# nextpyp/cet_pick

Hardware: AMD Instinct MI355X
Metric: subtomograms/sec (MoCo-3D train) + voxels/sec (heatmap+NMS) at 1/2/4/8 GPU (higher is better)
Workload: dtype f32; 1 GPU; moco_main.py moco3d_18: 3D encoder, synthetic 512x512x128 tomogram, 32^3 subtomo crops, batch 64 per GPU, r=1024, dim=128, m=0.999, T=0.1, SGD lr 1e-3; global_batch=64, parallelism=dp1, hipgraph=True

## Files before the change

### cet_pick_amd/_lib.py

```python
import ctypes
import os

import torch

_HERE = os.path.dirname(os.path.abspath(__file__))
LIB_PATH = os.environ.get("CETPICK_HIP_LIB") or os.path.join(_HERE, "libcetpick_hip.so")

_c = ctypes
_P, _I, _F, _Z, _D, _L = _c.c_void_p, _c.c_int, _c.c_float, _c.c_size_t, _c.c_double, _c.c_long


class ConvGeom(ctypes.Structure):
    _fields_ = [(f, _I) for f in "N Di Hi Wi Ci Co kd kh kw stride pd ph pw dd dh dw".split()]


_G = _c.POINTER(ConvGeom)


class Aug2d3dRanges(ctypes.Structure):
    _fields_ = [(f, _F) for f in "flip_p angle_lo angle_hi erase_p scale_lo scale_hi ratio_lo ratio_hi".split()]


_R = _c.POINTER(Aug2d3dRanges)

SIGNATURES = {
    "mi_abi_version": (_I, []),
    "mi_graph_node_counts": (_I, [_P, _P]),
    "mi_debug_stamp": (_I, [_P, _P]),
    "mi_linear_stats_fwd_f32": (_I, [_P] * 5 + [_I] * 3 + [_P]),
    "mi_debug_last_conv_kernel": (_c.c_char_p, []),
    "mi_linear_bn_fwd_f32": (_I, [_P] * 5 + [_I] * 3 + [_P, _P, _F, _F] + [_P] * 4 + [_I, _P]),
    "mi_conv3d_stem_stats_workspace_bytes": (_Z, [_I] * 5),
    "mi_conv3d_stem_stats_f32": (_I, [_P, _P, _P] + [_I] * 5 + [_P, _P, _Z, _P]),
    "mi_build_arch": (_c.c_char_p, []),
    "mi_sigmoid_clamp": (_I, [_P, _P, _Z, _P]),
    "mi_nms3d": (_I, [_P, _P, _I, _I, _I, _I, _I, _P]),
    "mi_decode_workspace_bytes": (_Z, [_I, _I, _I, _I]),
    "mi_decode_workspace_init": (_I, [_P, _Z, _P]),
    "mi_sigmoid_nms_topk": (_I, [_P, _P, _I, _I, _I, _I, _I, _I, _I, _P, _P, _P, _Z, _P]),
    "mi_gauss3d_sep": (_I, [_P, _P, _P, _I, _I, _I, _F, _P]),
    "mi_dog_pick_workspace_bytes": (_Z, [_I, _I, _I, _I]),
    "mi_dog_pick": (_I, [_P, _I, _I, _I, _P, _I, _I, _I, _I, _P, _P, _P, _P, _I, _P, _P, _Z, _P]),
    "mi_greedy_nms3d_workspace_bytes": (_Z, [_I, _I, _I]),
    "mi_greedy_nms3d": (_I, [_P, _I, _I, _I, _F, _F, _F, _P, _P, _P, _I, _P, _Z, _P]),
    "mi_crop_normalize": (_I, [_P, _I, _I, _I, _P, _I, _I, _I, _I, _I, _I, _P, _P]),
    "mi_crop_normalize_table": (_I, [_P, _P, _P, _P, _P, _c.c_int64, _I, _I, _I, _I, _I, _I, _P, _P]),
    "mi_u8_roundtrip_normalize": (_I, [_P, _P, _Z, _F, _F, _P]),
    "mi_aug2d_params": (_I, [_P, _c.c_int64, _c.c_uint64, _I, _I, _I] + [_F] * 7 + [_P, _P]),
    "mi_aug2d_apply": (_I, [_P, _c.c_int64, _I, _P, _P, _c.c_int64, _I, _F, _F, _P, _P]),
    "mi_aug2d3d_params": (_I, [_P, _c.c_int64, _c.c_uint64, _I, _I, _R, _R, _P, _P]),
    "mi_aug2d3d_apply": (_I, [_P, _P, _c.c_int64, _I, _P, _P, _P, _P, _c.c_int64, _I, _F, _F, _F, _F, _P, _P]),
    "mi_tilt_patches": (_I, [_P, _I, _P, _P, _c.c_int64, _I, _I, _D, _D, _P, _P, _P]),
    "mi_semi_labels": (_I, [_P, _I, _I, _I, _P, _c.c_int64, _P, _I, _I, _P]),
    "mi_semi_pairs": (_I, [_P, _P, _I, _P, _P, _c.c_int64, _I, _I, _P, _P, _P, _P]),
    "mi_gauss2d_slices": (_I, [_P, _P, _P, _I, _I, _I, _F, _P]),
    "mi_rec_reorder": (_I, [_P, _I, _I, _I, _I, _I, _I, _P, _P]),
    "mi_vol_stats_workspace_bytes": (_Z, [_L, _L]),
    "mi_vol_stats": (_I, [_P, _L, _L, _P, _P, _Z, _P]),
    "mi_zscore": (_I, [_P, _P, _L, _L, _P, _P]),
    "mi_zscore_quantize_minmax": (_I, [_P, _P, _L, _L, _P, _D, _D, _I, _P]),
    "mi_conv_workspace_bytes": (_Z, [_G]),
    "mi_conv_fwd_f32": (_I, [_P, _P, _P, _P, _I, _I, _G, _P, _Z, _P]),
    "mi_conv_dgrad_f32": (_I, [_P, _P, _P, _P, _P, _G, _P, _Z, _P]),
    "mi_conv_wgrad_f32": (_I, [_P, _P, _P, _G, _P, _Z, _P, _P]),
    "mi_conv_wgrad_batch_f32": (_I, [_P, _P, _P, _P, _I, _G, _Z, _P, _P]),
    "mi_stem2d_fwd_bias_f32": (_I, [_P, _P, _P, _P, _I, _I, _I, _I, _P]),
    "mi_upconv_tail_fwd": (_I, [_P, _P, _P, _P, _P] + [_I] * 7 + [_P]),
    "mi_smallk_image_bytes": (_Z, [_I, _I]),
    "mi_smallk_prep": (_I, [_P, _P, _I, _I, _P]),
    "mi_smallk_fwd_f32": (_I, [_P, _P, _P, _P, _I, _L, _I, _I, _I, _L, _I, _P]),
    "mi_smallk_heads_fwd_f32": (_I, [_P, _P, _P, _P, _P, _I, _L, _I, _L, _I, _P]),
    "mi_splitk_reduce_batch": (_I, [_P, _P, _P, _P, _I, _P]),
    "mi_linear_fwd_f32": (_I, [_P, _P, _P, _P, _I, _I, _I, _P, _Z, _P]),
    "mi_conv3d_direct_wimg_bytes": (_Z, [_I]),
    "mi_conv3d_direct_workspace_bytes": (_Z, [_I, _I]),
    "mi_conv3d_direct_usable": (_I, [_I] * 9),
    "mi_conv3d_direct_prep": (_I, [_P, _P, _P, _P, _I, _P]),
    "mi_conv3d_direct_f32": (_I, [_P, _P, _P, _P, _P, _I, _I, _I, _I, _I, _I, _P, _Z, _P]),
    "mi_conv2d_p2d_usable": (_I, [_I] * 4),
    "mi_conv2d_p2d_wimg_bytes": (_Z, [_I]),
    "mi_conv2d_p2d_prep": (_I, [_P, _P, _P, _P, _I, _P]),
    "mi_conv2d_p2d_f32": (_I, [_P, _P, _P, _P, _P, _I, _I, _I, _I, _I, _P]),
    "mi_conv2d_p2d_wgrad_workspace_bytes": (_Z, [_I] * 4),
    "mi_conv2d_p2d_wgrad_f32": (_I, [_P, _P, _P, _I, _I, _I, _I, _P, _Z, _P]),
    "mi_conv2d_stem3_workspace_bytes": (_Z, [_I]),
    "mi_conv2d_stem3_fwd_f32": (_I, [_P, _P, _P, _I, _I, _I, _I, _P]),
    "mi_conv2d_stem3_wgrad_f32": (_I, [_P, _P, _P, _I, _I, _I, _I, _P, _Z, _P]),
    "mi_conv3d_cube2_workspace_bytes": (_Z, [_I, _I]),
    "mi_conv3d_cube2_usable": (_I, [_I] * 9),
    "mi_conv3d_cube2_f32": (_I, [_P, _P, _P, _P, _P, _I, _I, _I, _I, _P, _Z, _P]),
    "mi_conv_d32_kind": (_I, [_I] * 12),
    "mi_conv_d32_image_bytes": (_Z, [_I, _I]),
    "mi_conv_d64_image_bytes": (_Z, [_I, _I]),
    "mi_conv_d32_prep": (_I, [_P, _P, _I, _I, _P]),
    "mi_conv_d64_prep_co": (_I, [_P, _P, _I, _I, _I, _P]),
    "mi_conv_d32_1x1_fwd_f32": (_I, [_P, _P, _P, _P, _I, _I, _I, _I, _I, _I, _I, _P]),
    "mi_conv_d32_fwd_pool_f32": (_I, [_P, _P, _P, _P, _P] + [_I] * 7 + [_P]),
    "mi_conv_d32_fwd_pool_strided_f32": (_I, [_P, _P, _P, _P, _I, _P] + [_I] * 7 + [_P]),
    "mi_copy_channels_into": (_I, [_P, _I, _P, _I, _I, _L, _P]),
    "mi_conv_d32_upconv_fwd_f32": (_I, [_P, _P, _P, _P, _P] + [_I] * 8 + [_P]),
    "mi_conv_d64_fwd_f32": (_I, [_P, _P, _P, _P, _I, _I, _I, _I, _I, _I, _I, _P]),
    "mi_conv_d32_fwd_f32": (_I, [_P, _P, _P, _P, _I, _I, _I, _I, _I, _I, _I, _P]),
    "mi_maxpool2d_ceil_fwd": (_I, [_P, _P, _P, _I, _I, _I, _I, _I, _P]),
    "mi_maxpool2d_ceil_bwd": (_I, [_P, _P, _P, _I, _I, _I, _I, _I, _P]),
    "mi_shuffle2x2_fwd": (_I, [_P, _P, _P, _I, _I, _I, _I, _I, _I, _P]),
    "mi_shuffle2x2_bwd": (_I, [_P, _P, _I, _I, _I, _I, _I, _I, _P]),
    "mi_concat_channels": (_I, [_P, _I, _P, _I, _P, _L, _P]),
    "mi_split_channels": (_I, [_P, _P, _I, _P, _I, _L, _P]),
    "mi_zhead_fwd": (_I, [_P, _P, _P, _I, _I, _L, _I, _I, _P]),
    "mi_zhead_bwd_workspace_bytes": (_Z, [_I, _I, _L, _I, _I]),
    "mi_zhead_bwd": (_I, [_P, _P, _P, _P, _P, _I, _I, _L, _I, _I, _P, _Z, _P]),
    "mi_voxel_loss_workspace_bytes": (_Z, [_L]),
    "mi_pu_focal_loss_fwd": (_I, [_P, _P, _L, _D, _D, _P, _P, _P, _Z, _P]),
    "mi_pu_focal_loss_bwd": (_I, [_P, _P, _L, _D, _P, _P, _P, _P]),
    "mi_focal_loss_fwd": (_I, [_P, _P, _L, _P, _P, _P, _Z, _P]),
    "mi_focal_loss_bwd": (_I, [_P, _P, _L, _P, _P, _P, _P]),
    "mi_mse_loss_fwd": (_I, [_P, _P, _L, _P, _P, _P, _Z, _P]),
    "mi_mse_loss_bwd": (_I, [_P, _P, _L, _P, _P, _P, _P, _P]),
    "mi_ucl_rowsums_fwd": (_I, [_P, _P, _I, _I, _F, _P, _P, _P, _P, _P, _P]),
    "mi_ucl_rowsums_bwd_ranged": (_I, [_P, _P, _I, _I, _F, _P, _P, _P, _P, _P, _P, _P, _P]),
    "mi_colreduce_workspace_bytes": (_Z, [_L, _I]),
    "mi_bn_stats": (_I, [_P, _L, _I, _P, _P, _Z, _P]),
    "mi_bn_apply_fwd": (_I, [_P, _P, _L, _I, _P, _D, _P, _P, _F, _F, _P, _P, _P, _P, _P, _I, _P]),
    "mi_bn_relu_maxpool3d_fwd": (_I, [_P, _P, _P, _I, _I, _I, _I, _I, _I, _I, _I, _P, _D, _P, _P, _F, _F, _P, _P, _P, _P, _P]),
    "mi_bn_relu_bwd_reduce_x": (_I, [_P, _P, _L, _I, _P, _P, _P, _P, _P, _Z, _P]),
    "mi_bn_relu_bwd_apply_x": (_I, [_P, _P, _P, _L, _I, _P, _P, _P, _P, _D, _P, _P, _P]),
    "mi_bn_small_fwd": (_I, [_P, _P, _L, _I, _P, _P, _F, _F, _P, _P, _P, _P, _P, _I, _P]),
    "mi_bn_small_bwd": (_I, [_P, _P, _P, _P, _L, _I, _P, _P, _I, _P, _P, _P]),
    "mi_bn_small_pool_fwd": (_I, [_P, _P, _P, _L, _I, _I, _P, _P, _F, _F, _P, _P, _P, _P, _P]),
    "mi_bn_small_pool_bwd": (_I, [_P, _P, _P, _P, _L, _I, _I, _P, _P, _P, _P, _P]),
    "mi_bn_eval_fwd": (_I, [_P, _P, _L, _I, _P, _P, _P, _P, _F, _P, _P, _I, _P]),
    "mi_bn_bwd_reduce": (_I, [_P, _P, _P, _L, _I, _P, _I, _P, _P, _Z, _P]),
    "mi_bn_bwd_apply": (_I, [_P, _P, _P, _P, _L, _I, _P, _P, _P, _D, _I, _P, _P, _P]),
    "mi_bn_bwd_apply_res": (_I, [_P, _P, _P, _P, _P, _L, _I, _P, _P, _P, _D, _P, _P, _P]),
    "mi_bn_param_grads": (_I, [_P, _I, _P, _P, _P]),
    "mi_colsum": (_I, [_P, _L, _I, _P, _P, _P, _Z, _P]),
    "mi_maxpool3d_fwd": (_I, [_P, _P, _P] + [_I] * 8 + [_P]),
    "mi_maxpool3d_bwd": (_I, [_P, _P, _P] + [_I] * 8 + [_P]),
    "mi_avgpool_fwd": (_I, [_P, _P, _I, _I, _I, _P]),
    "mi_avgpool_bwd": (_I, [_P, _P, _I, _I, _I, _P]),
    "mi_bias_add": (_I, [_P, _P, _L, _I, _P]),
    "mi_copy_pair_f32": (_I, [_P, _P, _P, _P, _L, _P]),
    "mi_relu_mask": (_I, [_P, _P, _P, _P, _L, _P]),
    "mi_l2norm_fwd": (_I, [_P, _P, _P, _I, _I, _P]),
    "mi_l2norm_bwd": (_I, [_P, _P, _P, _P, _I, _I, _P]),
    "mi_moco_logits_fwd": (_I, [_P, _P, _P, _P, _I, _I, _I, _F, _P]),
    "mi_moco_logits_norm_fwd": (_I, [_P, _P, _P, _P, _P, _P, _P, _I, _I, _I, _F, _P]),
    "mi_moco_logits_bwd": (_I, [_P, _P, _P, _P, _I, _I, _I, _F, _P]),
# ... 123 lines not shown
```

### cet_pick_amd/csrc/common.h

```cpp
#pragma once
#include <hip/hip_runtime.h>
#include <stdint.h>
#include <math.h>
#include "../../include/cetpick_hip.h"

#define MI_RETURN_IF_LAUNCH_FAILED()                  \
    do {                                              \
        hipError_t e_ = hipGetLastError();            \
        if (e_ != hipSuccess) return (int)e_;         \
    } while (0)
#define MI_HIP(call)                                  \
    do {                                              \
        hipError_t e_ = (call);                       \
        if (e_ != hipSuccess) return (int)e_;         \
    } while (0)

static inline size_t mi_align_up(size_t x, size_t a) { return (x + a - 1) / a * a; }

struct MiSmallGemmBN {
    float* y;
    const float* gamma;
    const float* beta;
    float eps, momentum;
    float* running_mean;
    float* running_var;
    long long* num_batches_tracked;
    float* save;
    int relu;
    double* sums_only;
};
static inline int mi_cdiv(long a, long b) { return (int)((a + b - 1) / b); }

struct Cube2Final {
    unsigned* tickets;
    float* out;
    const float* res;
    const float* mask;
    int relu;
};
constexpr size_t MI_CUBE2_TICKET_BYTES = 16384;

__device__ __forceinline__ float wave_sum(float v) {
#pragma unroll
    for (int o = 32; o > 0; o >>= 1) v += __shfl_xor(v, o, 64);
    return v;
}
__device__ __forceinline__ double wave_sum(double v) {
#pragma unroll
    for (int o = 32; o > 0; o >>= 1) v += __shfl_xor(v, o, 64);
    return v;
}
__device__ __forceinline__ float wave_max(float v) {
#pragma unroll
    for (int o = 32; o > 0; o >>= 1) v = fmaxf(v, __shfl_xor(v, o, 64));
    return v;
}

__device__ __forceinline__ unsigned long long make_key(float score, unsigned tie) {
    return ((unsigned long long)__float_as_uint(score) << 32) | (unsigned long long)tie;
}

__device__ __forceinline__ void block_bitonic_sort_desc(unsigned long long* keys, int n_pow2,
                                                        int tid, int nthreads) {
    for (int k = 2; k <= n_pow2; k <<= 1) {
        for (int j = k >> 1; j > 0; j >>= 1) {
            __syncthreads();
            for (int t = tid; t < (n_pow2 >> 1); t += nthreads) {
                int i = ((t / j) * (j << 1)) + (t % j);
                int l = i + j;
                bool desc = ((i & k) == 0);
                unsigned long long a = keys[i], b = keys[l];
                bool swap = desc ? (a < b) : (a > b);
                if (swap) { keys[i] = b; keys[l] = a; }
            }
        }
    }
    __syncthreads();
}

template <bool GUARD>
__device__ __forceinline__ void bitonic_pairs4(unsigned long long* keys, int t0, int stride, int n_pairs, int base, int j,
                                               int lj, int k) {
    unsigned long long a[4], b[4];
    int ii[4];
#pragma unroll
    for (int u = 0; u < 4; ++u) {
        const int t = t0 + u * stride;
        ii[u] = base + ((t >> lj) << (lj + 1)) + (t & (j - 1));
        if (!GUARD || t < n_pairs) { a[u] = keys[ii[u]]; b[u] = keys[ii[u] + j]; }
    }
#pragma unroll
    for (int u = 0; u < 4; ++u) {
        const int t = t0 + u * stride;
        if (!GUARD || t < n_pairs) {
            const bool desc = ((ii[u] & k) == 0);
            const bool sw = desc ? (a[u] < b[u]) : (a[u] > b[u]);
            keys[ii[u]] = sw ? b[u] : a[u];
            keys[ii[u] + j] = sw ? a[u] : b[u];
        }
    }
}

__device__ __forceinline__ void block_sort_desc_fast(unsigned long long* keys, int n_pow2, int tid, int nthreads) {
    const int n_waves = nthreads >> 6;
    const int B = n_pow2 / n_waves;
    const int lane = tid & 63, wv = tid >> 6;
    const int half = n_pow2 >> 1;
    __syncthreads();
    for (int k = 2; k <= n_pow2; k <<= 1) {
        int j = k >> 1;
        for (; 2 * j > B; j >>= 1) {
            const int lj = 31 - __builtin_clz(j);
            if ((half & (4 * nthreads - 1)) == 0)
                for (int t0 = tid; t0 < half; t0 += 4 * nthreads) bitonic_pairs4<false>(keys, t0, nthreads, half, 0, j, lj, k);
            else
                for (int t0 = tid; t0 < half; t0 += 4 * nthreads) bitonic_pairs4<true>(keys, t0, nthreads, half, 0, j, lj, k);
            __syncthreads();
        }
        for (; j > 0; j >>= 1) {
            const int lj = 31 - __builtin_clz(j);
            if (((B >> 1) & 255) == 0)
// ... 10 lines not shown
```

### cet_pick_amd/csrc/conv_cube2.hip

```cpp
#include "common.h"
#include "bf16x3.h"
#include <type_traits>

namespace {

using namespace bf3;

constexpr int KQ = 4;

struct Cube2Params {
    const float* a;
    const float* w;
    float* slabs;
    int N, C;
    unsigned a_bytes, w_bytes;
    unsigned* tickets;
    float* out;
    const float* res;
    const float* mask;
    int relu;
};

__device__ __forceinline__ int pair_tap(int in_v, int out_v) {
    const int tz = ((in_v >> 2) & 1) - ((out_v >> 2) & 1) + 1, ty = ((in_v >> 1) & 1) - ((out_v >> 1) & 1) + 1,
// ... 65 lines not shown
#pragma unroll
    for (int s = 0; s < NS; ++s) {
        if (s + PD - 1 < NS) fetch_dyn(s + PD - 1);
        bf16x8 af[2][3], bf[3];
        float v[8];
#pragma unroll
        for (int rb = 0; rb < 2; ++rb) {
#pragma unroll
            for (int e = 0; e < 4; ++e) { v[e] = __uint_as_float(araw[s % PD][rb][0][e]); v[4 + e] = __uint_as_float(araw[s % PD][rb][1][e]); }
            cut8(v, af[rb]);
        }
#pragma unroll
        for (int e = 0; e < 8; ++e) v[e] = __uint_as_float(braw[s % PD][e]);
        cut8(v, bf);
#pragma unroll
        for (int pr = 0; pr < 6; ++pr) {
            acc[0] = __builtin_amdgcn_mfma_f32_32x32x16_bf16(af[0][PA[pr]], bf[PB[pr]], acc[0], 0, 0, 0);
            acc[1] = __builtin_amdgcn_mfma_f32_32x32x16_bf16(af[1][PA[pr]], bf[PB[pr]], acc[1], 0, 0, 0);
        }
    }

#pragma unroll
    for (int rb = 0; rb < 2; ++rb)
#pragma unroll
        for (int r = 0; r < 16; ++r) red[wave][rb * 16 + r][lane] = acc[rb][r];
    __syncthreads();
    const long slab = (long)p.N * 8 * C;
    float* out = p.slabs + (long)q * slab;
    float tv[8];
    long o[8];
#pragma unroll
    for (int j = 0; j < 8; ++j) {
        const int idx = wave * 8 + j, rb = idx >> 4, r = idx & 15;
        tv[j] = ((red[0][idx][lane] + red[1][idx][lane]) + red[2][idx][lane]) + red[3][idx][lane];
        const int n = n0 + rb * 32 + (r & 3) + 8 * (r >> 2) + 4 * h;
        o[j] = n < p.N ? ((long)n * 8 + cv) * C + cc0 + l32 : -1;
        if (!FINAL) { if (o[j] >= 0) out[o[j]] = tv[j]; }
        else if (o[j] >= 0) __hip_atomic_store(out + o[j], tv[j], __ATOMIC_RELAXED, __HIP_MEMORY_SCOPE_AGENT);
    }
    if (!FINAL) return;
    asm volatile("s_waitcnt vmcnt(0)" ::: "memory");
    __syncthreads();
    unsigned* ticket = p.tickets + (mt * gridDim.x + cbi);
    if (tid == 0) s_last = (__hip_atomic_fetch_add(ticket, 1u, __ATOMIC_RELAXED, __HIP_MEMORY_SCOPE_AGENT) == KQ - 1) ? 1u : 0u;
    __syncthreads();
    if (!s_last) return;
    if (tid == 0) __hip_atomic_store(ticket, 0u, __ATOMIC_RELAXED, __HIP_MEMORY_SCOPE_AGENT);
    float part[KQ][8];
#pragma unroll
    for (int z = 0; z < KQ; ++z)
#pragma unroll
        for (int j = 0; j < 8; ++j)
            part[z][j] = (z == q || o[j] < 0) ? tv[j] : __hip_atomic_load(p.slabs + (long)z * slab + o[j], __ATOMIC_RELAXED, __HIP_MEMORY_SCOPE_AGENT);
#pragma unroll
    for (int j = 0; j < 8; ++j) {
        if (o[j] < 0) continue;
        float t = ((part[0][j] + part[1][j]) + part[2][j]) + part[3][j];
        if (p.res) t += p.res[o[j]];
        if (p.relu) t = fmaxf(t, 0.f);
        if (p.mask) t = (p.mask[o[j]] > 0.f) ? t : 0.f;
        p.out[o[j]] = t;
    }
}

constexpr int PW_ROW = 64;
constexpr int PW_HALF = 64 * PW_ROW;
constexpr int PW_PLANE = 2 * PW_HALF;
constexpr int PW_OP = 3 * PW_PLANE;
constexpr int PW_MAXTAP = 27;

constexpr int PW_MAXPROB = 4;
struct PairWgradParams {
    const float* x[PW_MAXPROB];
    const float* dy[PW_MAXPROB];
    float* dw[PW_MAXPROB];
    int N, VI, VO, CI, CO, ntaps;
    unsigned x_bytes, dy_bytes;
    int Di, Do, stride, pad, ks;
    int S;
    long slab_stride;
    unsigned char order[PW_MAXTAP];
    unsigned short cnt[PW_MAXTAP];
    unsigned char lo[PW_MAXTAP][3], len[PW_MAXTAP][3];
};

__global__ __launch_bounds__(512, 2) void pair_wgrad_kernel(PairWgradParams p) {
    __shared__ __attribute__((aligned(16))) unsigned char lds[2 * PW_OP];
    const int tid = threadIdx.x, lane = tid & 63, wave = tid >> 6;
    const int h = lane >> 5, l32 = lane & 31, i16 = lane & 15, g16 = (lane >> 4) & 1;
    const int wm = (wave >> 1) & 1, wn = wave & 1, kh = wave >> 2;
    const int ncb = p.CO >> 6, nib = p.CI >> 6;
    const int tiles = nib * ncb;
    const int rem = blockIdx.x % tiles, ts = blockIdx.x / tiles;
    const int tap = p.order[ts / p.S];
    const int seg = ts % p.S;
    const int ib = rem / ncb, cb = rem % ncb;
    const int npairs = p.cnt[tap], nchunks = (p.N + 63) >> 6;
    const int all = npairs * nchunks, per = (all + p.S - 1) / p.S;
    const int it0 = seg * per, total = min(all, it0 + per);
    const int tz = tap / (p.ks * p.ks), ty = (tap / p.ks) % p.ks, tx = tap % p.ks;
    const int lz = p.lo[tap][0], ly = p.lo[tap][1], lx = p.lo[tap][2], ny = p.len[tap][1], nx = p.len[tap][2];

    const __amdgpu_buffer_rsrc_t xrs = rsrc(p.x[blockIdx.y], p.x_bytes), yrs = rsrc(p.dy[blockIdx.y], p.dy_bytes);
    const int srow = tid >> 3, cg = tid & 7;
    const int st_lds = (cg >> 2) * PW_HALF + srow * PW_ROW + (cg & 3) * 16;
    u32x4 ldx[3][2], ldy[3][2];
    int f_it = it0, f_chunk = it0 % nchunks, f_px, f_py, f_pz;
    { const int pr = it0 / nchunks; f_px = pr % nx; f_py = (pr / nx) % ny; f_pz = pr / (nx * ny); }
    auto fetch = [&](auto Sc, int) {
        constexpr int S = decltype(Sc)::value;
        const int n = f_chunk * 64 + srow;
        const bool ok = f_it < total && n < p.N;
        const int oz = lz + f_pz, oy = ly + f_py, ox = lx + f_px;
        const int vo = (oz * p.Do + oy) * p.Do + ox;
        const int vi = ((p.stride * oz + tz - p.pad) * p.Di + p.stride * oy + ty - p.pad) * p.Di + p.stride * ox + tx - p.pad;
        ++f_it;
        if (++f_chunk == nchunks) { f_chunk = 0; if (++f_px == nx) { f_px = 0; if (++f_py == ny) { f_py = 0; ++f_pz; } } }
        const unsigned xo = ok ? 4u * (unsigned)(((long)n * p.VI + vi) * p.CI + ib * 64 + cg * 8) : 0x80000000u;
        const unsigned yo = ok ? 4u * (unsigned)(((long)n * p.VO + vo) * p.CO + cb * 64 + cg * 8) : 0x80000000u;
#pragma unroll
        for (int q = 0; q < 2; ++q) {
            ldx[S][q] = __builtin_amdgcn_raw_buffer_load_b128(xrs, (int)(xo + 16u * q), 0, 0);
            ldy[S][q] = __builtin_amdgcn_raw_buffer_load_b128(yrs, (int)(yo + 16u * q), 0, 0);
        }
    };
    auto store = [&](auto Sc, int boff) {
        constexpr int S = decltype(Sc)::value;
#pragma unroll
        for (int op = 0; op < 2; ++op) {
            float v[8];
#pragma unroll
            for (int e = 0; e < 4; ++e) {
                v[e] = __uint_as_float(op ? ldy[S][0][e] : ldx[S][0][e]);
                v[4 + e] = __uint_as_float(op ? ldy[S][1][e] : ldx[S][1][e]);
            }
            bf16x8 o[3];
            cut8(v, o);
#pragma unroll
            for (int pl = 0; pl < 3; ++pl)
                *reinterpret_cast<u32x4*>(lds + boff + op * PW_OP + pl * PW_PLANE + st_lds) = __builtin_bit_cast(u32x4, o[pl]);
        }
    };
    const int q4 = i16 >> 2;
    const int coloff = (16 * g16 + 4 * (i16 & 3)) * 2;
    const int a_base = wm * PW_HALF + (8 * h + q4 + 32 * kh) * PW_ROW + coloff;
    const int b_base = PW_OP + wn * PW_HALF + (8 * h + q4 + 32 * kh) * PW_ROW + coloff;

    f32x16 acc;
#pragma unroll
    for (int r = 0; r < 16; ++r) acc[r] = 0.f;

    auto multiply = [&](int boff) {
#pragma unroll
        for (int ks = 0; ks < 2; ++ks) {
            bf16x8 af[3], bf[3];
#pragma unroll
            for (int pl = 0; pl < 3; ++pl) {
                const unsigned char* ap = lds + boff + a_base + pl * PW_PLANE + ks * 16 * PW_ROW;
                const unsigned char* bp = lds + boff + b_base + pl * PW_PLANE + ks * 16 * PW_ROW;
                const bf16x4 alo = __builtin_amdgcn_ds_read_tr16_b64_v4bf16((lds_bf16x4*)(ap));
                const bf16x4 ahi = __builtin_amdgcn_ds_read_tr16_b64_v4bf16((lds_bf16x4*)(ap + 4 * PW_ROW));
                const bf16x4 blo = __builtin_amdgcn_ds_read_tr16_b64_v4bf16((lds_bf16x4*)(bp));
                const bf16x4 bhi = __builtin_amdgcn_ds_read_tr16_b64_v4bf16((lds_bf16x4*)(bp + 4 * PW_ROW));
                af[pl] = __builtin_shufflevector(alo, ahi, 0, 1, 2, 3, 4, 5, 6, 7);
                bf[pl] = __builtin_shufflevector(blo, bhi, 0, 1, 2, 3, 4, 5, 6, 7);
            }
#pragma unroll
            for (int pr = 0; pr < 6; ++pr) acc = __builtin_amdgcn_mfma_f32_32x32x16_bf16(af[PA[pr]], bf[PB[pr]], acc, 0, 0, 0);
        }
    };
    auto body = [&](auto Sc, auto, int it) {
        store(Sc, 0);
        __syncthreads();
        fetch(Sc, it + 3);
        multiply(0);
        __syncthreads();
    };
    using I0 = std::integral_constant<int, 0>; using I1 = std::integral_constant<int, 1>; using I2 = std::integral_constant<int, 2>;
    fetch(I0{}, it0);
    fetch(I1{}, it0 + 1);
    fetch(I2{}, it0 + 2);
    int it = it0;
    for (; it + 3 <= total; it += 3) {
        body(I0{}, I1{}, it);
        body(I1{}, I2{}, it + 1);
        body(I2{}, I0{}, it + 2);
    }
    if (it < total) {
        body(I0{}, I1{}, it);
        if (it + 1 < total) body(I1{}, I2{}, it + 1);
    }
    float (*red)[16][64] = reinterpret_cast<float (*)[16][64]>(lds);
    if (kh == 1) {
#pragma unroll
        for (int r = 0; r < 16; ++r) red[wave & 3][r][lane] = acc[r];
    }
    __syncthreads();
    if (kh == 0) {
        float* out = p.dw[blockIdx.y] + seg * p.slab_stride + ((long)tap * p.CI + ib * 64 + 32 * wm) * p.CO + cb * 64 + 32 * wn + l32;
#pragma unroll
        for (int r = 0; r < 16; ++r) out[(long)((r & 3) + 8 * (r >> 2) + 4 * h) * p.CO] = acc[r] + red[wave][r][lane];
    }
}

struct SmallGemmParams {
    const float* a;
    const float* b;
    const float* bias;
    float* c;
    int M, N, K;
    long lda_m, lda_k, ldb_k, ldb_n;
    unsigned a_bytes, b_bytes;
    float* bn_y;
    const float* gamma;
    const float* beta;
    float eps, momentum;
    float* running_mean;
    float* running_var;
    long long* num_batches_tracked;
    float* save;
    int relu;
    double* sums_only;
};

template <bool A_KC, bool B_KC, int NS>
__global__ __launch_bounds__(256, 2) void small_gemm_kernel(SmallGemmParams p) {
    __shared__ float red[4][32][64];
    const int tid = threadIdx.x, lane = tid & 63, wave = tid >> 6;
    const int h = lane >> 5, l32 = lane & 31;
    const int n0 = blockIdx.x * 32, m0 = blockIdx.y * 64;
    const int KT = (p.K + 15) >> 4;
    const __amdgpu_buffer_rsrc_t ars = rsrc(p.a, p.a_bytes), brs = rsrc(p.b, p.b_bytes);
    constexpr int PD = NS < 4 ? NS : 4;
    unsigned araw[PD][2][8], braw[PD][8];
    const bool col_ok = n0 + l32 < p.N;
    auto fetch = [&](auto Uc) {
        constexpr int U = decltype(Uc)::value, SET = U % PD;
        if constexpr (U < NS) {
            const int ks = wave + 4 * U;
            const int k0 = ks * 16 + 8 * h;
            const bool live = ks < KT;
#pragma unroll
            for (int rb = 0; rb < 2; ++rb) {
                const int m = m0 + rb * 32 + l32;
                const bool ok = live && m < p.M;
                if (A_KC) {
                    const unsigned off = (ok && k0 + 8 <= p.K) ? 4u * (unsigned)(m * p.lda_m + k0) : 0x80000000u;
                    const u32x4 lo = __builtin_amdgcn_raw_buffer_load_b128(ars, (int)off, 0, 0);
                    const u32x4 hi = __builtin_amdgcn_raw_buffer_load_b128(ars, (int)(off + 16u), 0, 0);
#pragma unroll
                    for (int e = 0; e < 4; ++e) { araw[SET][rb][e] = lo[e]; araw[SET][rb][4 + e] = hi[e]; }
                } else {
#pragma unroll
                    for (int e = 0; e < 8; ++e) {
                        const unsigned off = (ok && k0 + e < p.K) ? 4u * (unsigned)(m * p.lda_m + (long)(k0 + e) * p.lda_k) : 0x80000000u;
                        araw[SET][rb][e] = __builtin_amdgcn_raw_buffer_load_b32(ars, (int)off, 0, 0);
                    }
                }
            }
            const bool okb = live && col_ok;
            if (B_KC) {
                const unsigned off = (okb && k0 + 8 <= p.K) ? 4u * (unsigned)((long)(n0 + l32) * p.ldb_n + k0) : 0x80000000u;
                const u32x4 lo = __builtin_amdgcn_raw_buffer_load_b128(brs, (int)off, 0, 0);
                const u32x4 hi = __builtin_amdgcn_raw_buffer_load_b128(brs, (int)(off + 16u), 0, 0);
#pragma unroll
                for (int e = 0; e < 4; ++e) { braw[SET][e] = lo[e]; braw[SET][4 + e] = hi[e]; }
            } else {
#pragma unroll
                for (int e = 0; e < 8; ++e) {
                    const unsigned off = (okb && k0 + e < p.K) ? 4u * (unsigned)((long)(k0 + e) * p.ldb_k + (long)(n0 + l32) * p.ldb_n) : 0x80000000u;
                    braw[SET][e] = __builtin_amdgcn_raw_buffer_load_b32(brs, (int)off, 0, 0);
                }
            }
        }
    };
    f32x16 acc[2];
#pragma unroll
    for (int r = 0; r < 16; ++r) { acc[0][r] = 0.f; acc[1][r] = 0.f; }
    auto step = [&](auto Uc) {
        constexpr int U = decltype(Uc)::value, SET = U % PD;
        if constexpr (U < NS) {
            fetch(std::integral_constant<int, U + PD - 1>{});
            if (wave + 4 * U < KT) {
                bf16x8 af[2][3], bf[3];
                float v[8];
// ... 69 lines not shown
            }
        }
        if (blockIdx.x == 0 && tid == 0 && p.num_batches_tracked) *p.num_batches_tracked += 1;
        const float g = (p.gamma && col_ok) ? p.gamma[col] : 1.f, b = (p.beta && col_ok) ? p.beta[col] : 0.f;
#pragma unroll
        for (int j = 0; j < 8; ++j) {
            const int idx = wave * 8 + j, rb = idx >> 4, r = idx & 15;
            const int m = m0 + rb * 32 + (r & 3) + 8 * (r >> 2) + 4 * h;
            float q = fmaf((tv[j] - mf) * iv, g, b);
            if (p.relu) q = fmaxf(q, 0.f);
            if (m < p.M && col_ok) p.bn_y[(long)m * p.N + col] = q;
        }
    }
}

}

bool mi_cube2_usable(int N, int Di, int Hi, int Wi, int Ci, int Co, int kd, int kh, int kw, int stride, int pd, int ph, int pw,
                     int dd, int dh, int dw) {
    const char* off = getenv("MI_CONV_NO_DIRECT");
    if (off && atoi(off) != 0) return false;
    if (kd != 3 || kh != 3 || kw != 3 || stride != 1 || pd != 1 || ph != 1 || pw != 1 || dd != 1 || dh != 1 || dw != 1) return false;
    if (Di != 2 || Hi != 2 || Wi != 2 || Ci != Co) return false;
    if (Ci != 128 && Ci != 256 && Ci != 512) return false;
    return N >= 1 && 4l * N * 8 * Ci < 0x7fff0000l;
}

namespace {
struct PairGeom { int ntaps, maxcnt; long pairs; };
PairGeom pair_geom(int Di, int k, int stride, PairWgradParams* p) {
    const int pad = k == 3 ? 1 : 0, Do = (Di + 2 * pad - k) / stride + 1;
    PairGeom r = {k * k * k, 0, 0};
    for (int t = 0; t < r.ntaps; ++t) {
        const int tt[3] = {t / (k * k), (t / k) % k, t % k};
        int c = 1;
        for (int a = 0; a < 3; ++a) {
            int lo = Do, hi = -1;
            for (int o = 0; o < Do; ++o) {
                const int i = stride * o + tt[a] - pad;
                if (i >= 0 && i < Di) { lo = std::min(lo, o); hi = std::max(hi, o); }
            }
            const int len = hi >= lo ? hi - lo + 1 : 0;
            if (p) { p->lo[t][a] = (unsigned char)(len ? lo : 0); p->len[t][a] = (unsigned char)std::max(len, 1); }
            c *= len;
        }
        if (p) p->cnt[t] = (unsigned short)c;
        r.maxcnt = std::max(r.maxcnt, c);
        r.pairs += c;
    }
    return r;
}
}

bool mi_pair_wgrad_usable(int N, int Di, int Hi, int Wi, int Ci, int Co, int kd, int kh, int kw, int stride, int pd, int ph, int pw,
                          int dd, int dh, int dw) {
    const char* off = getenv("MI_CONV_NO_DIRECT");
    if (off && atoi(off) != 0) return false;
    if (kd != kh || kd != kw || pd != ph || pd != pw || dd != 1 || dh != 1 || dw != 1) return false;
    if (!((kd == 3 && pd == 1) || (kd == 1 && pd == 0)) || (stride != 1 && stride != 2)) return false;
    if (Hi != Di || Wi != Di || Di < 2) return false;
    const int Do = (Di + 2 * pd - kd) / stride + 1;
    const char* wide = getenv("MI_PAIR_WGRAD_MAXOUT");
    if (Do < 1 || Do > (wide ? atoi(wide) : 2) || Do > 8) return false;
    if (Ci < 64 || Co < 64 || (Ci & 63) || (Co & 63)) return false;
    return N >= 1 && 4l * N * Di * Hi * Wi * Ci < 0x7fff0000l && 4l * N * Do * Do * Do * Co < 0x7fff0000l;
}

int mi_pair_wgrad_splits(int N, int Di, int Ci, int Co, int k, int stride) {
    const PairGeom g = pair_geom(Di, k, stride, nullptr);
    if (g.maxcnt <= 8) return 1;
    const char* e = getenv("MI_PAIR_WGRAD_SPLITS");
    if (e && atoi(e) > 0) return std::min(atoi(e), 64);
    const int iters = g.maxcnt * ((N + 63) / 64), tiles = (Ci / 64) * (Co / 64);
    int S = (iters + 7) / 8;
    if (g.ntaps * tiles * S < 256) S = (iters + 3) / 4;
    return std::max(1, std::min(S, 16));
}
size_t mi_pair_wgrad_slab_bytes(int N, int Di, int Ci, int Co, int k, int stride) {
    const int S = mi_pair_wgrad_splits(N, Di, Ci, Co, k, stride);
    return S > 1 ? sizeof(float) * (size_t)S * k * k * k * Ci * Co : 0;
}

int mi_pair_wgrad_batch_max() { return PW_MAXPROB; }
int mi_pair_wgrad_launch_batch(const float* const* xs, const float* const* dys, float* const* dws, float* const* slabs, int nb, int N,
                               int Di, int Ci, int Co, int k, int stride, hipStream_t s) {
    if (nb < 1 || nb > PW_MAXPROB) return MI_E_ARG;
    PairWgradParams p = {};
    const PairGeom g = pair_geom(Di, k, stride, &p);
    const int pad = k == 3 ? 1 : 0, Do = (Di + 2 * pad - k) / stride + 1;
    const int S = mi_pair_wgrad_splits(N, Di, Ci, Co, k, stride);
    for (int i = 0; i < nb; ++i) {
        if (S > 1 && !slabs[i]) return MI_E_ARG;
        p.x[i] = xs[i]; p.dy[i] = dys[i]; p.dw[i] = S > 1 ? slabs[i] : dws[i];
    }
    p.N = N; p.VI = Di * Di * Di; p.VO = Do * Do * Do; p.CI = Ci; p.CO = Co; p.ntaps = g.ntaps;
    p.x_bytes = (unsigned)(4l * N * p.VI * Ci); p.dy_bytes = (unsigned)(4l * N * p.VO * Co);
    p.Di = Di; p.Do = Do; p.stride = stride; p.pad = pad; p.ks = k; p.S = S; p.slab_stride = (long)g.ntaps * Ci * Co;
    int n = 0;
    for (int want = g.maxcnt; want >= 0; --want)
        for (int t = 0; t < g.ntaps; ++t)
            if (p.cnt[t] == want) p.order[n++] = (unsigned char)t;
    hipLaunchKernelGGL(pair_wgrad_kernel, dim3((unsigned)(g.ntaps * (Ci / 64) * (Co / 64) * S), (unsigned)nb), dim3(512), 0, s, p);
    MI_RETURN_IF_LAUNCH_FAILED();
    return MI_OK;
}
int mi_pair_wgrad_launch(const float* x, const float* dy, float* dwt, float* slabs, int N, int Di, int Ci, int Co, int k, int stride,
                         hipStream_t s) {
    const float* xs[1] = {x};
    const float* dys[1] = {dy};
    float* dws[1] = {dwt};
    float* sl[1] = {slabs};
    return mi_pair_wgrad_launch_batch(xs, dys, dws, sl, 1, N, Di, Ci, Co, k, stride, s);
}

size_t mi_cube2_slab_bytes(int N, int C) { return sizeof(float) * (size_t)KQ * N * 8 * C; }
int mi_cube2_splits() { return KQ; }

bool mi_cube2_final_usable(int N, int C) { return sizeof(unsigned) * (size_t)(8 * C / 32) * ((N + 63) / 64) <= MI_CUBE2_TICKET_BYTES; }
int mi_cube2_launch(int dgrad, const float* a, const float* w, float* slabs, int N, int C, hipStream_t s, const Cube2Final* fin) {
    Cube2Params p = {a, w, slabs, N, C, (unsigned)(4l * N * 8 * C), (unsigned)(4l * 27 * C * C), nullptr, nullptr, nullptr, nullptr, 0};
    if (fin) { p.tickets = fin->tickets; p.out = fin->out; p.res = fin->res; p.mask = fin->mask; p.relu = fin->relu; }
    const dim3 grid((unsigned)(8 * C / 32), KQ, (unsigned)((N + 63) / 64));
#define CUBE2_LAUNCH(D, NSV) do { if (fin) hipLaunchKernelGGL((cube2_kernel<D, NSV, true>), grid, dim3(256), 0, s, p); \
                                  else hipLaunchKernelGGL((cube2_kernel<D, NSV, false>), grid, dim3(256), 0, s, p); } while (0)
    if (C == 128) { if (dgrad) CUBE2_LAUNCH(true, 4); else CUBE2_LAUNCH(false, 4); }
    else if (C == 256) { if (dgrad) CUBE2_LAUNCH(true, 8); else CUBE2_LAUNCH(false, 8); }
    else if (C == 512) { if (dgrad) CUBE2_LAUNCH(true, 16); else CUBE2_LAUNCH(false, 16); }
    else return MI_E_UNSUPPORTED;
#undef CUBE2_LAUNCH
    MI_RETURN_IF_LAUNCH_FAILED();
    return MI_OK;
}

bool mi_small_gemm_usable(long M, long N, long K) {
    const char* off = getenv("MI_CONV_NO_DIRECT");
    if (off && atoi(off) != 0) return false;
    return M >= 1 && M <= 1024 && N >= 1 && N <= 4096 && K >= 1 && K <= 1024;
}
int mi_small_gemm_launch(const float* a, long lda_m, long lda_k, long a_elems, const float* b, long ldb_k, long ldb_n,
                         long b_elems, const float* bias, float* c, int M, int N, int K, hipStream_t s, const MiSmallGemmBN* bn) {
    if (4 * a_elems >= 0x7fff0000l || 4 * b_elems >= 0x7fff0000l) return MI_E_UNSUPPORTED;
    if (bn && M > 64) return MI_E_UNSUPPORTED;
    if (bn && !bn->sums_only && (!bn->y || !bn->save || (bn->running_mean == nullptr) != (bn->running_var == nullptr))) return MI_E_UNSUPPORTED;
    SmallGemmParams p = {a, b, bias, c, M, N, K, lda_m, lda_k, ldb_k, ldb_n, (unsigned)(4 * a_elems), (unsigned)(4 * b_elems)};
    p.bn_y = nullptr; p.sums_only = nullptr;
    if (bn && bn->sums_only) p.sums_only = bn->sums_only;
    else if (bn) {
        p.bn_y = bn->y; p.gamma = bn->gamma; p.beta = bn->beta; p.eps = bn->eps; p.momentum = bn->momentum;
        p.running_mean = bn->running_mean; p.running_var = bn->running_var; p.num_batches_tracked = bn->num_batches_tracked;
        p.save = bn->save; p.relu = bn->relu;
    }
    const dim3 grid((unsigned)((N + 31) / 32), (unsigned)((M + 63) / 64));
    const int kt = (K + 15) / 16, per = (kt + 3) / 4;
    const int ns = per <= 1 ? 1 : per <= 2 ? 2 : per <= 4 ? 4 : per <= 8 ? 8 : 16;
    const bool akc = lda_k == 1 && (lda_m % 4) == 0 && (K % 8) == 0, bkc = ldb_k == 1 && (ldb_n % 4) == 0 && (K % 8) == 0;
#define SG_LAUNCH(AK, BK, NSV) hipLaunchKernelGGL((small_gemm_kernel<AK, BK, NSV>), grid, dim3(256), 0, s, p)
#define SG_NS(AK, BK)                                                                                   \
    switch (ns) {                                                                                       \
        case 1: SG_LAUNCH(AK, BK, 1); break;                                                            \
        case 2: SG_LAUNCH(AK, BK, 2); break;                                                            \
        case 4: SG_LAUNCH(AK, BK, 4); break;                                                            \
        case 8: SG_LAUNCH(AK, BK, 8); break;                                                            \
        default: SG_LAUNCH(AK, BK, 16); break;                                                          \
    }
    if (akc && bkc) { SG_NS(true, true) }
    else if (akc) { SG_NS(true, false) }
    else if (bkc) { SG_NS(false, true) }
    else { SG_NS(false, false) }
#undef SG_NS
#undef SG_LAUNCH
    MI_RETURN_IF_LAUNCH_FAILED();
    return MI_OK;
}

void mi_note_conv_kernel(const char* name);
extern "C" size_t mi_conv3d_cube2_workspace_bytes(int N, int C) { return MI_CUBE2_TICKET_BYTES + mi_cube2_slab_bytes(N, C); }

extern "C" int mi_conv3d_cube2_usable(int N, int Di, int Hi, int Wi, int Ci, int Co, int k, int stride, int pad) {
    return mi_cube2_usable(N, Di, Hi, Wi, Ci, Co, k, k, k, stride, pad, pad, pad, 1, 1, 1) && mi_cube2_final_usable(N, Ci) ? 1 : 0;
}

extern "C" int mi_conv3d_cube2_f32(const float* a, const float* w, float* out, const float* res, const float* mask, int relu,
                                   int dgrad, int N, int C, void* ws, size_t ws_bytes, mi_stream_t stream) {
    if (!a || !w || !out) return MI_E_ARG;
    if (!mi_conv3d_cube2_usable(N, 2, 2, 2, C, C, 3, 1, 1)) return MI_E_UNSUPPORTED;
    if (!ws || ws_bytes < mi_conv3d_cube2_workspace_bytes(N, C)) return MI_E_WORKSPACE;
    Cube2Final fin = {(unsigned*)ws, out, res, mask, relu};
    mi_note_conv_kernel("cube2");
    return mi_cube2_launch(dgrad ? 1 : 0, a, w, (float*)((char*)ws + MI_CUBE2_TICKET_BYTES), N, C, (hipStream_t)stream, &fin);
}
```

### cet_pick_amd/csrc/conv_direct3.hip

```cpp
#include "common.h"
#include "bf16x3.h"
#include <type_traits>
#include <algorithm>

namespace {

using namespace bf3;

constexpr int C = 64;
constexpr int PLANE = 64;
constexpr int TZ = 2;
constexpr int PZ = TZ + 2;
constexpr int NV = PZ * PLANE;
constexpr int LEAD = 16;
constexpr int ZREC = 34;
constexpr int NREC = LEAD + NV + ZREC;
constexpr int ARR = NREC * 16;
constexpr int KS = C / 16;
constexpr int PL_BYTES = 2 * ARR;
constexpr int KS_BYTES = 3 * PL_BYTES;
constexpr int LDS_BYTES = KS * KS_BYTES;
constexpr int ZBASE = (LEAD + NV) * 16;
constexpr int WBLK = 1024;
constexpr int WSTEP = 2 * 3 * WBLK;
// ... 387 lines not shown
            __builtin_amdgcn_sched_barrier(0);
        }
    }

    const bool has_mask = p.mask != nullptr;
    const long zrow = ((long)n * p.D + z0 + tz) * p.H;
#pragma unroll
    for (int i = 0; i < 2; ++i) {
        float rr[16], mm[16];
        unsigned eo[16];
#pragma unroll
        for (int r = 0; r < 16; ++r) {
            const int m = (r & 3) + 8 * (r >> 2) + 4 * h, y = 4 * i + (m >> 3), x = m & 7;
            const bool in = y0 + y < p.H && x0 + x < p.W;
            eo[r] = in ? 4u * (unsigned)((((zrow + y0 + y) * p.W) + x0 + x) * C + col) : 0x80000000u;
            rr[r] = __uint_as_float(__builtin_amdgcn_raw_buffer_load_b32(rrs, (int)eo[r], 0, 0));
            mm[r] = __uint_as_float(__builtin_amdgcn_raw_buffer_load_b32(mrs, (int)eo[r], 0, 0));
        }
#pragma unroll
        for (int r = 0; r < 16; ++r) {
            float v = acc[i][r] + rr[r];
            if (p.relu) v = fmaxf(v, 0.f);
            if (has_mask) v = (mm[r] > 0.f) ? v : 0.f;
            if (eo[r] != 0x80000000u) p.out[eo[r] / 4] = v;
        }
    }
}

constexpr int PREP_MAX = 16;
struct PrepBatch {
    const float* w[PREP_MAX];
    unsigned char* img[PREP_MAX];
    int dgrad[PREP_MAX];
    int wide[PREP_MAX];
};
__device__ void direct3s_prep_body(const float* w, unsigned char* img, int dgrad, int idx);
__device__ void direct3s256_prep_body(const float* w, unsigned char* img, int dgrad, int idx);
constexpr int PREP_BLOCKS_256 = 8 * NTAP * 2 * 8 * 64 / 256;
constexpr int PREP_BLOCKS = NTAP * KS * 2 * 64 / 256;
constexpr int PREP_BLOCKS_WIDE = 4 * NTAP * 2 * 4 * 64 / 256;
template <int CT>
__device__ void direct3_prep_body(const float* w, unsigned char* img, int dgrad, int idx) {
    constexpr int KSn = CT / 16;
    const int lane = idx & 63, cw = (idx >> 6) & 1, rest = idx >> 7, ks = rest % KSn, tap = (rest / KSn) % NTAP, cb = rest / (KSn * NTAP);
    if (cb >= CT / 64) return;
    const int nn = cb * 64 + cw * 32 + (lane & 31), k0 = ks * 16 + 8 * (lane >> 5);
    float v[8];
    if (dgrad) {
        ld8(w + ((long)(NTAP - 1 - tap) * CT + nn) * CT + k0, v);
    } else {
#pragma unroll
        for (int e = 0; e < 8; ++e) v[e] = w[((long)tap * CT + k0 + e) * CT + nn];
    }
    u32x4 o[3];
    cut8(v, o);
    unsigned char* dst = img + (long)(((cb * KSn + ks) * NTAP + tap) * 2 + cw) * (3 * WBLK) + lane * 16;
    store_planes(dst, WBLK, o);
}
__global__ __launch_bounds__(256) void direct3_prep_kernel(PrepBatch b) {
    const int fmt = b.wide[blockIdx.y], idx = blockIdx.x * 256 + threadIdx.x;
    if (fmt == 1) { if (blockIdx.x < PREP_BLOCKS_WIDE) direct3s_prep_body(b.w[blockIdx.y], b.img[blockIdx.y], b.dgrad[blockIdx.y], idx); }
    else if (fmt == 2) { if (blockIdx.x < PREP_BLOCKS_WIDE) direct3_prep_body<128>(b.w[blockIdx.y], b.img[blockIdx.y], b.dgrad[blockIdx.y], idx); }
    else if (fmt == 3) direct3s256_prep_body(b.w[blockIdx.y], b.img[blockIdx.y], b.dgrad[blockIdx.y], idx);
    else if (blockIdx.x < PREP_BLOCKS) direct3_prep_body<C>(b.w[blockIdx.y], b.img[blockIdx.y], b.dgrad[blockIdx.y], idx);
}

constexpr int WG_SPLITS = 28;
constexpr int WROW = 64;
constexpr int WHALF = (PLANE + 1) * WROW;
constexpr int WPL = 2 * WHALF;
constexpr int WOP = 3 * WPL;
constexpr int WBUF = 2 * WOP;
constexpr int WZERO = PLANE * WROW;

constexpr int WG_MAXPROB = 4;
struct Direct3WgradParams {
    const float* x[WG_MAXPROB];
    const float* dy[WG_MAXPROB];
    float* slabs[WG_MAXPROB];
    int N, D;
    unsigned bytes;
    int nprob, splits;
    int H, W;
};

constexpr int W_HB = 3 * 2 * 8 * 128;
template <bool V4, int CT, bool TILED = false>
__global__ __launch_bounds__(512, 2) void direct3_wgrad_kernel(Direct3WgradParams p) {
    __shared__ __attribute__((aligned(16))) unsigned char lds[2 * WBUF + (TILED ? 2 * W_HB : 16)];
    unsigned char* const halo = lds + 2 * WBUF;
    static_assert(!TILED || (!V4 && CT == 64), "tiled planes: the 64-channel geometry");
    constexpr int NBLK = CT / 64;
    const int tid = threadIdx.x, lane = tid & 63;
    const int wave = __builtin_amdgcn_readfirstlane(tid >> 6);
    const int h = lane >> 5, l32 = lane & 31, i16 = lane & 15, g16 = (lane >> 4) & 1;
    const int kh = wave >> 2, wm = (wave >> 1) & 1, wn = wave & 1;
    const int per_grp = p.nprob * p.splits;
    const int grp = blockIdx.x / per_grp, rem = blockIdx.x % per_grp;
    const int pb = rem / p.splits, split = rem % p.splits, stride = p.splits;
    const int pair = grp % 9, chb = grp / 9;
    const int ci0 = (chb / NBLK) * 64, co0 = (chb % NBLK) * 64;
    const int dz = pair / 3, dy = pair % 3;
    const int tiles_x = TILED ? p.W >> 3 : 1, tiles = TILED ? (p.H >> 3) * tiles_x : 1;
    const int n_planes = p.N * p.D * tiles;

    const __amdgpu_buffer_rsrc_t xrs = rsrc(p.x[pb], p.bytes), yrs = rsrc(p.dy[pb], p.bytes);
    const int st_vox = tid >> 3, st_cg = tid & 7;
    const unsigned st_src = TILED ? 4u * (unsigned)(((st_vox >> 3) * p.W + (st_vox & 7)) * C + st_cg * 8)
                                  : 4u * (unsigned)(st_vox * CT + st_cg * 8);
    const int h_side = tid >> 8, h_row = (tid >> 5) & 7, h_c2 = tid & 31;
    const unsigned x_ch = 4u * (unsigned)ci0, y_ch = 4u * (unsigned)co0;
    const int zsh = V4 ? 0 : dz - 1;
    const int st_lds = (st_cg >> 2) * WHALF + st_vox * WROW + (st_cg & 3) * 16;
    auto next_plane = [&](int from) {
        if (V4) return from < n_planes ? from : -1;
        for (int pi = from; pi < n_planes; pi += stride) {
            const int zi = (pi / tiles) % p.D + dz - 1;
            if ((unsigned)zi < (unsigned)p.D) return pi;
        }
        return -1;
    };
    u32x4 ldx[2], ldy[2];
    u32x2 ldh = {0u, 0u};
    unsigned u_y, u_x, u_h;
    auto unit_offsets = [&](int pi) {
        if (pi < 0) { u_y = u_x = u_h = 0x80000000u; return; }
        if (!TILED) {
            u_y = 4u * (unsigned)((long)pi * PLANE * CT) + y_ch + st_src;
            u_x = 4u * (unsigned)((long)(pi + zsh) * PLANE * CT) + x_ch + st_src;
            u_h = 0x80000000u;
            return;
        }
        const int pl = pi / tiles, t = pi % tiles, y0 = (t / tiles_x) * 8, x0 = (t % tiles_x) * 8;
        u_y = 4u * (unsigned)((((long)pl * p.H + y0) * p.W + x0) * C) + st_src;
        const int xr = y0 + (st_vox >> 3) + dy - 1;
        u_x = (unsigned)xr < (unsigned)p.H
                  ? 4u * (unsigned)((((long)(pl + dz - 1) * p.H + xr) * p.W + x0 + (st_vox & 7)) * C + st_cg * 8) : 0x80000000u;
        const int hr = y0 + h_row + dy - 1, hc = h_side ? x0 + 8 : x0 - 1;
        u_h = ((unsigned)hr < (unsigned)p.H && (unsigned)hc < (unsigned)p.W)
                  ? 4u * (unsigned)((((long)(pl + dz - 1) * p.H + hr) * p.W + hc) * C + 2 * h_c2) : 0x80000000u;
    };
    auto stage_load = [&](int pi) {
        unit_offsets(pi);
        ldx[0] = __builtin_amdgcn_raw_buffer_load_b128(xrs, (int)u_x, 0, 0);
        ldx[1] = __builtin_amdgcn_raw_buffer_load_b128(xrs, (int)(u_x + 16u), 0, 0);
        ldy[0] = __builtin_amdgcn_raw_buffer_load_b128(yrs, (int)u_y, 0, 0);
        ldy[1] = __builtin_amdgcn_raw_buffer_load_b128(yrs, (int)(u_y + 16u), 0, 0);
        if (TILED) ldh = __builtin_amdgcn_raw_buffer_load_b64(xrs, (int)u_h, 0, 0);
    };
    unsigned hcu[3];
    auto halo_cut = [&]() {
        const unsigned a1 = rest(ldh[0]), b1 = rest(ldh[1]), a2 = rest(a1), b2 = rest(b1);
        hcu[0] = pack2(ldh[1], ldh[0]);
        hcu[1] = pack2(b1, a1);
        hcu[2] = pack2(b2, a2);
    };
    auto halo_store = [&](int buf) {
#pragma unroll
        for (int pl = 0; pl < 3; ++pl)
            *reinterpret_cast<unsigned*>(halo + buf * W_HB + ((pl * 2 + h_side) * 8 + h_row) * 128 + h_c2 * 4) = hcu[pl];
    };
    auto stage_store_unit = [&](int buf, int op) {
        float v[8];
#pragma unroll
        for (int e = 0; e < 4; ++e) {
            v[e] = __uint_as_float(op ? ldy[0][e] : ldx[0][e]);
            v[4 + e] = __uint_as_float(op ? ldy[1][e] : ldx[1][e]);
        }
        u32x4 o[3];
        cut8(v, o);
// ... 79 lines not shown
        const u32x4 c = __builtin_bit_cast(u32x4, af[set][1][pl]);
        u32x4 o;
        if (dxv == 0) {
            o[0] = c[0] << 16;
#pragma unroll
            for (int j = 1; j < 4; ++j) o[j] = __builtin_amdgcn_alignbit(c[j], c[j - 1], 16);
            if (V4) o[2] &= HI16;
            if (TILED) o[0] |= hl[set][0][pl];
        } else {
#pragma unroll
            for (int j = 0; j < 3; ++j) o[j] = __builtin_amdgcn_alignbit(c[j + 1], c[j], 16);
            o[3] = c[3] >> 16;
            if (V4) o[1] &= 0x0000ffffu;
            if (TILED) o[3] |= hl[set][1][pl] << 16;
        }
        af[set][dxv][pl] = __builtin_bit_cast(bf16x8, o);
    };
    unsigned cu[3][8];
    auto cut_a = [&](int op, int e) {
        cu[0][e] = op ? ldy[e >> 2][e & 3] : ldx[e >> 2][e & 3];
        cu[1][e] = rest(cu[0][e]);
    };
    auto cut_b = [&](int e) { cu[2][e] = rest(cu[1][e]); };
    auto store_piece = [&](int buf, int op, int pl) {
        u32x4 o;
#pragma unroll
        for (int d = 0; d < 4; ++d) o[d] = pack2(cu[pl][2 * d + 1], cu[pl][2 * d]);
        *reinterpret_cast<u32x4*>(lds + buf * WBUF + op * WOP + st_lds + pl * WPL) = o;
    };

    int buf = 0;
    if (cur >= 0) {
#pragma unroll
        for (int i = 0; i < 3; ++i) read_pair(0, 0, i);
    }
    constexpr int DXO[3] = {1, 0, 2};
    while (cur >= 0) {
        const int nn = nxt >= 0 ? next_plane(nxt + stride) : -1;
        unit_offsets(nn);
        __builtin_amdgcn_sched_barrier(0);
#pragma unroll
        for (int lk = 0; lk < 2; ++lk) {
            const int op = lk;
#pragma unroll
            for (int m = 0; m < 18; ++m) {
                const int dxm = DXO[m / 6];
                acc[dxm] = __builtin_amdgcn_mfma_f32_32x32x16_bf16(af[lk][dxm][PA[m % 6]], bfg[lk][PB[m % 6]], acc[dxm], 0, 0, 0);
                if (m < 3) derive(lk, 0, m);
                if (m >= 6 && m < 9) derive(lk, 2, m - 6);
                if (m >= 2 && m < 10) cut_a(op, m - 2);
                if (m >= 3 && m < 11) cut_b(m - 3);
                if (m >= 11 && m < 14) store_piece(buf ^ 1, op, m - 11);
                if (lk == 1 && m >= 14) {
                    const int i = m - 14, hf = i & 1;
                    if (i < 2) ldx[hf] = __builtin_amdgcn_raw_buffer_load_b128(xrs, (int)(u_x + 16u * hf), 0, 0);
                    else ldy[hf] = __builtin_amdgcn_raw_buffer_load_b128(yrs, (int)(u_y + 16u * hf), 0, 0);
                    if (TILED && i == 3) ldh = __builtin_amdgcn_raw_buffer_load_b64(xrs, (int)u_h, 0, 0);
                }
                if (TILED && lk == 0 && m == 14) halo_cut();
                if (TILED && lk == 0 && m == 15) halo_store(buf ^ 1);
                if (lk == 0) {
                    if (m < 3) read_pair(buf, 1, m);
                } else {
                    if (m == 13) __syncthreads();
                    if (m >= 14 && m < 17 && nxt >= 0) read_pair(buf ^ 1, 0, m - 14);
                }
                __builtin_amdgcn_sched_barrier(0);
            }
        }
        buf ^= 1;
        cur = nxt;
        nxt = nn;
    }

    __syncthreads();
    float* red = reinterpret_cast<float*>(lds);
    if (kh == 1) {
#pragma unroll
        for (int dx = 0; dx < 3; ++dx)
#pragma unroll
            for (int r = 0; r < 16; ++r) red[(((wave & 3) * 3 + dx) * 16 + r) * 64 + lane] = acc[dx][r];
    }
    __syncthreads();
    if (kh == 1) return;
    float* out = p.slabs[pb] + (long)split * (NTAP * CT * CT);
#pragma unroll
    for (int dx = 0; dx < 3; ++dx) {
        const int tap = (dz * 3 + dy) * 3 + dx;
#pragma unroll
        for (int r = 0; r < 16; ++r) {
            const int ci = ci0 + 32 * wm + (r & 3) + 8 * (r >> 2) + 4 * h;
            out[((long)tap * CT + ci) * CT + co0 + 32 * wn + l32] = acc[dx][r] + red[((wave * 3 + dx) * 16 + r) * 64 + lane];
        }
    }
}

constexpr int CS = 128;
constexpr int VS = 64;
constexpr int S_LEAD = 32;
constexpr int S_NV = VS;
constexpr int S_ZREC = 64;
constexpr int S_NREC = S_LEAD + S_NV + S_ZREC;
constexpr int S_ARR = S_NREC * 16;
constexpr int S_PL = 2 * S_ARR;
constexpr int S_KS = 3 * S_PL;
constexpr int S_CH = 2 * S_KS;
constexpr int S_ZBASE = (S_LEAD + S_NV) * 16;
constexpr int S_CHUNKS = 4;
constexpr int S_LDS = S_CHUNKS * S_CH;
constexpr int S_STEPS = 2 * NTAP;
constexpr int S_WSTEP = 4 * 3 * WBLK;
constexpr int S_WIMG_BYTES = S_CHUNKS * S_STEPS * S_WSTEP;
static_assert(S_STEPS % RB == 0, "ring slots");
static_assert(((S_LEAD + S_NV) & 15) == 0, "zero region must start at a record = 0 (mod 16)");
static_assert(S_LDS <= 160 * 1024 && 4 * 32 * 64 * 4 <= S_LDS, "patch (and the four partial tiles behind it) fit the LDS");

struct Direct3sParams {
    const float* a;
    const unsigned char* wimg;
    float* out;
    const float* res;
    const float* mask;
    int relu;
    int N;
    unsigned a_bytes;
};

template <int CT>
__global__ __launch_bounds__(256, 1) void direct3s_kernel(Direct3sParams p) {
    constexpr int NCB = CT / 32;
    constexpr int NPASS = NCB / S_CHUNKS;
    constexpr int WST = NCB * 3 * WBLK;
    __shared__ __attribute__((aligned(16))) unsigned char patch[S_LDS];
    const int tid = threadIdx.x, lane = tid & 63;
    const int cc = __builtin_amdgcn_readfirstlane(tid >> 6);
    const int h = lane >> 5, l32 = lane & 31;
    const int ct = blockIdx.x % NCB, n0 = blockIdx.x / NCB;

    const __amdgpu_buffer_rsrc_t wrs = rsrc(p.wimg, NCB * S_STEPS * WST);
    const int w_voff = ct * (3 * WBLK) + lane * 16;
    int w_soff = cc * (S_STEPS * WST);
    bf16x8 bfr[RB][3];
    auto wload = [&](int g, auto SLOTc) {
        constexpr int SLOT = decltype(SLOTc)::value;
        const int vo = g < S_STEPS ? w_voff : (int)0x80000000u;
        const int so = g < S_STEPS ? w_soff + g * WST : 0;
#pragma unroll
        for (int pl = 0; pl < 3; ++pl)
            bfr[SLOT][pl] = __builtin_bit_cast(bf16x8, __builtin_amdgcn_raw_buffer_load_b128(wrs, vo + pl * WBLK, so, 0));
    };
    auto wload_dyn = [&](int g) {
        switch (g % RB) {
            case 0: wload(g, std::integral_constant<int, 0>{}); break;
            case 1: wload(g, std::integral_constant<int, 1>{}); break;
            case 2: wload(g, std::integral_constant<int, 2>{}); break;
            case 3: wload(g, std::integral_constant<int, 3>{}); break;
            case 4: wload(g, std::integral_constant<int, 4>{}); break;
            default: wload(g, std::integral_constant<int, 5>{}); break;
        }
    };
    const __amdgpu_buffer_rsrc_t ars = rsrc(p.a, p.a_bytes);
    for (int i = tid; i < 12 * S_CHUNKS * S_ZREC; i += 256) {
        const int arr = i / S_ZREC, r = i % S_ZREC;
        *reinterpret_cast<u32x4*>(patch + arr * S_ARR + S_ZBASE + r * 16) = u32x4{0u, 0u, 0u, 0u};
    }
    auto stage = [&](int pass) {
        u32x4 ld[4][2];
#pragma unroll
        for (int u = 0; u < 4; ++u) {
            const int q = tid + 256 * u, vox = q >> 4, cg = q & 15;
            const unsigned off = 4u * (unsigned)(((long)n0 * VS + vox) * CT + pass * 128 + cg * 8);
            ld[u][0] = __builtin_amdgcn_raw_buffer_load_b128(ars, (int)off, 0, 0);
            ld[u][1] = __builtin_amdgcn_raw_buffer_load_b128(ars, (int)(off + 16u), 0, 0);
        }
#pragma unroll
        for (int u = 0; u < 4; ++u) {
// ... 148 lines not shown
}
bool mi_direct3_usable(int N, int Di, int Hi, int Wi, int Ci, int Co, int kd, int kh, int kw, int stride, int pd, int ph,
                       int pw, int dd, int dh, int dw) {
    return mi_direct3_kind(N, Di, Hi, Wi, Ci, Co, kd, kh, kw, stride, pd, ph, pw, dd, dh, dw) != 0;
}

size_t mi_direct3_wimg_bytes(int channels) {
    return channels == C ? (size_t)WIMG_BYTES : channels == CS ? (size_t)S_WIMG_BYTES : 0;
}
size_t mi_direct3_wimg_bytes_kind(int kind) {
    return (kind == 1 || kind == 5) ? (size_t)WIMG_BYTES : kind == 2 ? (size_t)S_WIMG_BYTES : kind == 3 ? (size_t)(2 * 8 * NTAP * WSTEP)
         : kind == 4 ? (size_t)8 * S_STEPS * (8 * 3 * WBLK) : 0;
}
size_t mi_direct3_slab_bytes(int, int) { return 0; }

int mi_direct3_prep_kind(const float* const* w, void* const* img, const int* dgrad, const int* kinds, int n, hipStream_t s) {
    for (int i0 = 0; i0 < n; i0 += PREP_MAX) {
        PrepBatch b = {};
        const int m = n - i0 < PREP_MAX ? n - i0 : PREP_MAX;
        int blocks = PREP_BLOCKS;
        for (int i = 0; i < m; ++i) {
            const int kd = kinds[i0 + i];
            if (kd < 1 || kd > 5 || !w[i0 + i] || !img[i0 + i]) return MI_E_ARG;
            b.w[i] = w[i0 + i]; b.img[i] = (unsigned char*)img[i0 + i]; b.dgrad[i] = dgrad[i0 + i];
            b.wide[i] = kd == 5 ? 0 : kd - 1;
            blocks = std::max(blocks, kd == 4 ? PREP_BLOCKS_256 : (kd == 2 || kd == 3) ? PREP_BLOCKS_WIDE : PREP_BLOCKS);
        }
        hipLaunchKernelGGL(direct3_prep_kernel, dim3(blocks, m), dim3(256), 0, s, b);
        MI_RETURN_IF_LAUNCH_FAILED();
    }
    return MI_OK;
}
int mi_direct3_prep(const float* const* w, void* const* img, const int* dgrad, const int* channels, int n, hipStream_t s) {
    if (n > 4096) return MI_E_ARG;
    int kinds[4096];
    for (int i = 0; i < n; ++i) {
        if (channels[i] != C && channels[i] != CS) return MI_E_ARG;
        kinds[i] = channels[i] == C ? 1 : 2;
    }
    return mi_direct3_prep_kind(w, img, dgrad, kinds, n, s);
}

int mi_direct3_launch(const float* a, const void* wimg, float* out, const float* res, const float* mask, int relu, int N,
                      int D, hipStream_t s) {
    Direct3Params p = {a, (const unsigned char*)wimg, out, res, mask, relu, N, D, (unsigned)(4l * N * D * PLANE * C)};
    if (getenv("MI_DIRECT3_FOUR_SLOTS")) hipLaunchKernelGGL(direct3_kernel<false>, dim3((unsigned)(N * (D / TZ))), dim3(256), 0, s, p);
    else hipLaunchKernelGGL(direct3_kernel<true>, dim3((unsigned)(N * (D / TZ))), dim3(256), 0, s, p);
    MI_RETURN_IF_LAUNCH_FAILED();
    return MI_OK;
}
int mi_direct3h_launch(const float* a, const void* wimg, float* out, const float* res, const float* mask, int relu, int N,
                       int D, int H, int W, hipStream_t s) {
    Direct3hParams p = {a, (const unsigned char*)wimg, out, res, mask, relu, N, D, H, W, (unsigned)(4l * N * D * H * W * C)};
    hipLaunchKernelGGL(direct3h_kernel, dim3((unsigned)((long)N * (D / TZ) * ((H + 7) / 8) * ((W + 7) / 8))), dim3(256), 0, s, p);
    MI_RETURN_IF_LAUNCH_FAILED();
    return MI_OK;
}
int mi_direct3_launch128(const float* a, const void* wimg, float* out, const float* res, const float* mask, int relu, int N,
                         int D, hipStream_t s) {
    Direct3Params p = {a, (const unsigned char*)wimg, out, res, mask, relu, N, D, (unsigned)(4l * N * D * PLANE * 128)};
    hipLaunchKernelGGL((direct3_kernel<true, 128>), dim3((unsigned)(N * (D / TZ)), 2), dim3(256), 0, s, p);
    MI_RETURN_IF_LAUNCH_FAILED();
    return MI_OK;
}

int mi_direct3s_launch(const float* a, const void* wimg, float* out, const float* res, const float* mask, int relu, int N,
                       hipStream_t s) {
    Direct3sParams p = {a, (const unsigned char*)wimg, out, res, mask, relu, N, (unsigned)(4l * N * VS * CS)};
    hipLaunchKernelGGL(direct3s_kernel<CS>, dim3((unsigned)(4 * N)), dim3(256), 0, s, p);
    MI_RETURN_IF_LAUNCH_FAILED();
    return MI_OK;
}
int mi_direct3s_launch256(const float* a, const void* wimg, float* out, const float* res, const float* mask, int relu, int N,
                          hipStream_t s) {
    Direct3sParams p = {a, (const unsigned char*)wimg, out, res, mask, relu, N, (unsigned)(4l * N * VS * 256)};
    hipLaunchKernelGGL(direct3s_kernel<256>, dim3((unsigned)(8 * N)), dim3(256), 0, s, p);
    MI_RETURN_IF_LAUNCH_FAILED();
    return MI_OK;
}

size_t mi_direct3_wgrad_slab_bytes() { return sizeof(float) * (size_t)WG_SPLITS * NTAP * C * C; }
int mi_direct3_wgrad_splits() { return WG_SPLITS; }

int mi_direct3_wgrad_launch(const float* x, const float* dy, float* slabs, int N, int D, hipStream_t s) {
    Direct3WgradParams p = {};
    p.x[0] = x; p.dy[0] = dy; p.slabs[0] = slabs; p.N = N; p.D = D; p.bytes = (unsigned)(4l * N * D * PLANE * C);
    p.nprob = 1; p.splits = WG_SPLITS;
    hipLaunchKernelGGL((direct3_wgrad_kernel<false, 64>), dim3(9 * WG_SPLITS), dim3(512), 0, s, p);
    MI_RETURN_IF_LAUNCH_FAILED();
    return MI_OK;
}
int mi_direct3_wgrad_batch_max() { return WG_MAXPROB; }
constexpr int WG_BATCH_SPLITS = 7;
int mi_direct3_wgrad_batch_splits(int nb) {
    if (nb < 1 || nb > WG_MAXPROB) return 0;
    if (const char* v = getenv("MI_D3W_BATCH_SPLITS")) { const int sv = atoi(v); if (sv >= 1 && sv <= WG_SPLITS) return sv; }
    return WG_BATCH_SPLITS;
}
int mi_direct3_wgrad_launch_batch(const float* const* xs, const float* const* dys, float* const* slabs, int nb, int N, int D,
                                  hipStream_t s) {
    if (nb < 1 || nb > WG_MAXPROB) return MI_E_ARG;
    Direct3WgradParams p = {};
    for (int i = 0; i < nb; ++i) { p.x[i] = xs[i]; p.dy[i] = dys[i]; p.slabs[i] = slabs[i]; }
    p.N = N; p.D = D; p.bytes = (unsigned)(4l * N * D * PLANE * C);
    p.nprob = nb; p.splits = mi_direct3_wgrad_batch_splits(nb);
    hipLaunchKernelGGL((direct3_wgrad_kernel<false, 64>), dim3(9 * nb * p.splits), dim3(512), 0, s, p);
    MI_RETURN_IF_LAUNCH_FAILED();
    return MI_OK;
}

constexpr int WS_SPLITS = 7, WS_BATCH_SPLITS = 2;
size_t mi_direct3s_wgrad_slab_bytes() { return sizeof(float) * (size_t)WS_SPLITS * NTAP * CS * CS; }
int mi_direct3s_wgrad_splits(int nb) {
    if (nb < 1 || nb > WG_MAXPROB) return 0;
    if (nb == 1) return WS_SPLITS;
    if (const char* v = getenv("MI_D3SW_BATCH_SPLITS")) { const int sv = atoi(v); if (sv >= 1 && sv <= WS_SPLITS) return sv; }
    return WS_BATCH_SPLITS;
}
int mi_direct3s_wgrad_launch_batch(const float* const* xs, const float* const* dys, float* const* slabs, int nb, int N, hipStream_t s) {
    if (nb < 1 || nb > WG_MAXPROB || N < 1) return MI_E_ARG;
    Direct3WgradParams p = {};
    for (int i = 0; i < nb; ++i) { p.x[i] = xs[i]; p.dy[i] = dys[i]; p.slabs[i] = slabs[i]; }
    p.N = N; p.D = 1; p.bytes = (unsigned)(4l * N * PLANE * CS);
    p.nprob = nb; p.splits = mi_direct3s_wgrad_splits(nb);
    hipLaunchKernelGGL((direct3_wgrad_kernel<true, 128>), dim3(36 * nb * p.splits), dim3(512), 0, s, p);
    MI_RETURN_IF_LAUNCH_FAILED();
    return MI_OK;
}

int mi_direct3t_wgrad_launch(const float* x, const float* dy, float* slabs, int N, int D, int H, int W, hipStream_t s) {
    if (H % 8 || W % 8 || H < 8 || W < 8) return MI_E_UNSUPPORTED;
    Direct3WgradParams p = {};
    p.x[0] = x; p.dy[0] = dy; p.slabs[0] = slabs; p.N = N; p.D = D; p.H = H; p.W = W;
    p.bytes = (unsigned)(4l * N * D * H * W * C);
    p.nprob = 1; p.splits = WG_SPLITS;
    hipLaunchKernelGGL((direct3_wgrad_kernel<false, 64, true>), dim3(9 * WG_SPLITS), dim3(512), 0, s, p);
    MI_RETURN_IF_LAUNCH_FAILED();
    return MI_OK;
}

int mi_direct3x_wgrad_splits(int kind) { return kind == 3 ? 7 : 0; }
size_t mi_direct3x_wgrad_slab_bytes(int kind) {
    const size_t ct = kind == 3 ? 128 : 0;
    return sizeof(float) * (size_t)mi_direct3x_wgrad_splits(kind) * NTAP * ct * ct;
}
int mi_direct3x_wgrad_launch(int kind, const float* x, const float* dy, float* slabs, int N, int D, hipStream_t s) {
    Direct3WgradParams p = {};
    p.x[0] = x; p.dy[0] = dy; p.slabs[0] = slabs; p.nprob = 1; p.splits = mi_direct3x_wgrad_splits(kind);
    if (kind == 3) {
        p.N = N; p.D = D; p.bytes = (unsigned)(4l * N * D * PLANE * 128);
        hipLaunchKernelGGL((direct3_wgrad_kernel<false, 128>), dim3(36 * p.splits), dim3(512), 0, s, p);
    } else return MI_E_UNSUPPORTED;
    MI_RETURN_IF_LAUNCH_FAILED();
    return MI_OK;
}

int mi_direct3_finish_slabs(const float* slabs, int n_slabs, long out_elems, float* out, const float* res, const float* mask,
                            int relu, hipStream_t s);

extern "C" size_t mi_conv3d_direct_wimg_bytes(int channels) { return mi_direct3_wimg_bytes(channels); }
extern "C" size_t mi_conv3d_direct_workspace_bytes(int N, int channels) { return mi_direct3_slab_bytes(N, channels); }

extern "C" int mi_conv3d_direct_usable(int N, int Di, int Hi, int Wi, int Ci, int Co, int k, int stride, int pad) {
    const int kind = mi_direct3_kind(N, Di, Hi, Wi, Ci, Co, k, k, k, stride, pad, pad, pad, 1, 1, 1);
    return kind <= 2 ? kind : 0;
}

extern "C" int mi_conv3d_direct_prep(const void* const* w, void* const* img, const int* dgrad, const int* channels, int n,
                                     mi_stream_t stream) {
    if (!w || !img || !dgrad || !channels || n < 0) return MI_E_ARG;
    if (n == 0) return MI_OK;
    return mi_direct3_prep(reinterpret_cast<const float* const*>(w), img, dgrad, channels, n, (hipStream_t)stream);
}

extern "C" int mi_conv3d_direct_f32(const float* a, const void* wimg, float* out, const float* res, const float* mask,
                                    int relu, int N, int Di, int Hi, int Wi, int channels, void* ws, size_t ws_bytes,
                                    mi_stream_t stream) {
    if (!a || !wimg || !out) return MI_E_ARG;
    const int kind = mi_direct3_kind(N, Di, Hi, Wi, channels, channels, 3, 3, 3, 1, 1, 1, 1, 1, 1, 1);
    if (kind == 1) return mi_direct3_launch(a, wimg, out, res, mask, relu, N, Di, (hipStream_t)stream);
    if (kind == 2) return mi_direct3s_launch(a, wimg, out, res, mask, relu, N, (hipStream_t)stream);
    return MI_E_UNSUPPORTED;
}
```

### cet_pick_amd/csrc/conv_igemm.hip

```cpp
#include "common.h"
#include "bf16x3.h"
#include <algorithm>
#include <cstdlib>
#include <type_traits>

int mi_stem7_fwd(const float* x, const float* w, float* y, const float* res, int relu, int N, int D, int H, int W,
                 int Co, int bf16x3, void* ws, size_t ws_bytes, hipStream_t s, double* sums = nullptr);
size_t mi_stem7_fwd_workspace_bytes();
size_t mi_stem7_fwd_stats_workspace_bytes(int N, int D, int H, int W);
size_t mi_stem7_wgrad_workspace_bytes(int N, int D, int H, int W, int Co);
int mi_stem7_wgrad(const float* x, const float* dy, float* dw, int N, int D, int H, int W, int Co, int bf16x3, void* ws,
                   size_t ws_bytes, hipStream_t s);

int mi_direct3_kind(int N, int Di, int Hi, int Wi, int Ci, int Co, int kd, int kh, int kw, int stride, int pd, int ph,
                    int pw, int dd, int dh, int dw);
size_t mi_direct3_wimg_bytes(int channels);
size_t mi_direct3_slab_bytes(int N, int channels);
int mi_direct3_prep(const float* const* w, void* const* img, const int* dgrad, const int* channels, int n, hipStream_t s);
int mi_direct3_launch(const float* a, const void* wimg, float* out, const float* res, const float* mask, int relu, int N,
                      int D, hipStream_t s);
size_t mi_direct3_wimg_bytes_kind(int kind);
int mi_direct3_prep_kind(const float* const* w, void* const* img, const int* dgrad, const int* kinds, int n, hipStream_t s);
int mi_direct3s_launch256(const float* a, const void* wimg, float* out, const float* res, const float* mask, int relu, int N,
                          hipStream_t s);
int mi_direct3h_launch(const float* a, const void* wimg, float* out, const float* res, const float* mask, int relu, int N,
                       int D, int H, int W, hipStream_t s);
int mi_direct3_launch128(const float* a, const void* wimg, float* out, const float* res, const float* mask, int relu, int N,
                         int D, hipStream_t s);
int mi_direct3s_launch(const float* a, const void* wimg, float* out, const float* res, const float* mask, int relu, int N,
                       hipStream_t s);
int mi_direct3_finish_slabs(const float* slabs, int n_slabs, long out_elems, float* out, const float* res, const float* mask,
                            int relu, hipStream_t s);
size_t mi_direct3_wgrad_slab_bytes();
int mi_direct3_wgrad_splits();
int mi_direct3_wgrad_launch(const float* x, const float* dy, float* slabs, int N, int D, hipStream_t s);
int mi_direct3_wgrad_batch_max();
int mi_direct3_wgrad_batch_splits(int nb);
int mi_direct3_wgrad_launch_batch(const float* const* xs, const float* const* dys, float* const* slabs, int nb, int N, int D, hipStream_t s);
size_t mi_direct3s_wgrad_slab_bytes();
int mi_direct3s_wgrad_splits(int nb);
int mi_direct3s_wgrad_launch_batch(const float* const* xs, const float* const* dys, float* const* slabs, int nb, int N, hipStream_t s);
int mi_direct3t_wgrad_launch(const float* x, const float* dy, float* slabs, int N, int D, int H, int W, hipStream_t s);
int mi_direct3x_wgrad_splits(int kind);
size_t mi_direct3x_wgrad_slab_bytes(int kind);
int mi_direct3x_wgrad_launch(int kind, const float* x, const float* dy, float* slabs, int N, int D, hipStream_t s);
int mi_pair_wgrad_batch_max();
int mi_pair_wgrad_launch_batch(const float* const* xs, const float* const* dys, float* const* dws, float* const* slabs, int nb, int N, int Di,
                               int Ci, int Co, int k, int stride, hipStream_t s);
bool mi_cube2_usable(int N, int Di, int Hi, int Wi, int Ci, int Co, int kd, int kh, int kw, int stride, int pd, int ph, int pw,
                     int dd, int dh, int dw);
size_t mi_cube2_slab_bytes(int N, int C);
int mi_cube2_splits();
int mi_cube2_launch(int dgrad, const float* a, const float* w, float* slabs, int N, int C, hipStream_t s, const Cube2Final* fin = nullptr);
bool mi_pair_wgrad_usable(int N, int Di, int Hi, int Wi, int Ci, int Co, int kd, int kh, int kw, int stride, int pd, int ph, int pw,
                          int dd, int dh, int dw);
int mi_pair_wgrad_splits(int N, int Di, int Ci, int Co, int k, int stride);
size_t mi_pair_wgrad_slab_bytes(int N, int Di, int Ci, int Co, int k, int stride);
int mi_pair_wgrad_launch(const float* x, const float* dy, float* dwt, float* slabs, int N, int Di, int Ci, int Co, int k, int stride,
                         hipStream_t s);
bool mi_small_gemm_usable(long M, long N, long K);
int mi_small_gemm_launch(const float* a, long lda_m, long lda_k, long a_elems, const float* b, long ldb_k, long ldb_n,
                         long b_elems, const float* bias, float* c, int M, int N, int K, hipStream_t s,
                         const MiSmallGemmBN* bn = nullptr);

namespace {

using namespace bf3;

enum { MODE_FWD = 0, MODE_DGRAD = 1, MODE_WGRAD = 2 };
constexpr int NTHREADS = 256;
constexpr int MAX_CLASSES = 27;

struct BorderClass { short pos0[3], cnt[3], tlo[3], tcnt[3]; };
constexpr int LUT_TAPS = 352;
constexpr int LUT_INVALID = 0x070707;

constexpr int MI_WGRAD_BATCH_MAX = 4;
struct ConvParams {
    const float* a_src;
    const float* b_src;
    float* out;
    const float* res;
    int res_bcast;
    const float* mask;
    int relu;
    int N, Dg, Hg, Wg, Cg;
    int Dr, Hr, Wr;
    unsigned mgW, mgH, mgD;
    int shW, shH, shD;
    int kd, kh, kw, stride, pd, ph, pw;
    int dd, dh, dw;
    int Ci, Co;
    long M;
    int Ncols;
    unsigned a_bytes, b_bytes;
    int splits;
    long slab_stride;
    long n_red_vox;
    int n_classes;
    int border;
    int cls_tile_start[MAX_CLASSES + 1];
    BorderClass bcls[MAX_CLASSES];
    int ny_tiles;
    int tiles_x;
    int fold;
    int wbox;
    int nbatch;
    const float* a_tab[MI_WGRAD_BATCH_MAX];
    const float* b_tab[MI_WGRAD_BATCH_MAX];
    float* out_tab[MI_WGRAD_BATCH_MAX];
};

constexpr unsigned OOR = 0x80000000u;
__device__ __forceinline__ float4 bld4(__amdgpu_buffer_rsrc_t r, unsigned off) {
    const u32x4 v = __builtin_amdgcn_raw_buffer_load_b128(r, (int)off, 0, 0);
    return make_float4(__uint_as_float(v.x), __uint_as_float(v.y), __uint_as_float(v.z), __uint_as_float(v.w));
}
__device__ __forceinline__ float bld1(__amdgpu_buffer_rsrc_t r, unsigned off) {
    return __uint_as_float(__builtin_amdgcn_raw_buffer_load_b32(r, (int)off, 0, 0));
}

__device__ __forceinline__ unsigned axis_mask(int base, int step, int count, int n) {
    unsigned m = 0;
    for (int t = 0; t < count; ++t)
        if ((unsigned)(base + step * t) < (unsigned)n) m |= 1u << t;
    return m;
}

struct GridDec {
    int D, H, W;
    unsigned mD, mH, mW;
    int sD, sH, sW;
    __device__ __forceinline__ static unsigned divm(unsigned n, unsigned m, int s) {
        return (unsigned)(((unsigned long long)n * m) >> s);
    }
    __device__ __forceinline__ void operator()(unsigned m, int& n, int& z, int& y, int& x) const {
        unsigned q = divm(m, mW, sW); x = (int)(m - q * (unsigned)W); m = q;
        q = divm(m, mH, sH); y = (int)(m - q * (unsigned)H); m = q;
        q = divm(m, mD, sD); z = (int)(m - q * (unsigned)D); n = (int)q;
    }
};
__host__ __device__ inline void magic31(int d, unsigned* m, int* s) {
    int L = 0;
    while ((1ll << L) < (long long)d) ++L;
    *s = 31 + L;
    *m = (unsigned)(((1ull << (31 + L)) / (unsigned long long)d) + 1ull);
}
__device__ __forceinline__ GridDec make_dec(int D, int H, int W) {
    GridDec g;
    g.D = D > 0 ? D : 1; g.H = H > 0 ? H : 1; g.W = W > 0 ? W : 1;
    magic31(g.D, &g.mD, &g.sD); magic31(g.H, &g.mH, &g.sH); magic31(g.W, &g.mW, &g.sW);
    return g;
}

struct Cursor {
    int c0, ia, ib, ic;
};

template <int MODE, int BM, int BN, int BK, bool STEM, bool BF3 = false>
__global__ __launch_bounds__(NTHREADS, BF3 ? ((BM == 128 && BN == 32) ? 2 : 3) : 1) void conv_igemm_kernel(ConvParams p) {
    static_assert(!BF3 || (!STEM && (BK == 16 || BK == 32)), "bf16x3 path: generic layers, 16- or 32-deep slices");
    static_assert(BK == 16 || BK == 32 || BK == 64, "slice depth");
    static_assert(BN == 32 || BN == 64 || BN == 128, "tile width");
    static_assert(BN != 32 || (BF3 && BM == 128 && BK == 32), "32-wide tiles: 128 rows, bf16x3, 32-deep slices");
    constexpr int WN = BN == 32 ? 1 : 2, WM = 4 / WN;
    constexpr int LDK = BK + 4;
    constexpr int KH = BK / 2;
    constexpr int KC = BK / 4;
    constexpr int WTM = BM / WM, WTN = BN / WN;
    constexpr int MT = WTM / 32, NT = WTN / 32;
    static_assert(MT >= 1 && NT >= 1, "wave tile");
    constexpr bool A_ROWK = (MODE != MODE_WGRAD);
    constexpr bool B_ROWK = (MODE == MODE_DGRAD);
    constexpr int A_ELEMS = A_ROWK ? BM * LDK : BK * BM;
    constexpr int B_ELEMS = B_ROWK ? BN * LDK : BK * BN;
    constexpr int STAGE = A_ELEMS + B_ELEMS;
    constexpr int A_CH = BM * KC / NTHREADS;
    constexpr int B_CH = BN * KC / NTHREADS;
    constexpr int TPV = NTHREADS / BK;
    static_assert(A_CH >= 1 && B_CH >= 1, "tile too small for 256 threads");
    constexpr int RS = 2 * BK;
    constexpr int KSUB = 64 * BK + 64;
    constexpr int A_PLANE = A_ROWK ? BM * RS : (BM / 32) * KSUB;
    constexpr int B_PLANE = B_ROWK ? BN * RS : (BN / 32) * KSUB;
    constexpr int STAGE_B = 3 * (A_PLANE + B_PLANE);
    constexpr int KS = BK / 16;

    auto rowk_swz = [](int r) { return BK == 32 ? (r >> 2) & 3 : (r >> 3) & 1; };
    __shared__ __attribute__((aligned(16))) float lds[BF3 ? STAGE_B / 2 : 2 * STAGE];
    unsigned char* const ldsb = reinterpret_cast<unsigned char*>(lds);
    __shared__ long rowmap[BM];
    __shared__ int2 taplut[STEM ? LUT_TAPS : 1];

    const int tid = threadIdx.x, lane = tid & 63, wave = tid >> 6;
    const int wm = wave / WN, wn = wave % WN;
    const int h = lane >> 5, l32 = lane & 31;
    int blk_x, blk_y, blk_z;
    {
        const int total = gridDim.x, L = blockIdx.x;
        int q = L;
        if (p.fold) {
            const int g = L >> 8, r = L & 255, m = g >> 1;
            q = (g & 1) ? total - 1 - (m * 256 + r) : m * 256 + r;
        }
        if (p.fold) {
            const int per = p.ny_tiles * p.splits;
            blk_x = q / per;
            const int rem = q - blk_x * per;
            blk_y = rem % p.ny_tiles;
            blk_z = rem / p.ny_tiles;
        } else {
            blk_x = q % p.tiles_x;
            const int rem = q / p.tiles_x;
            blk_y = rem % p.ny_tiles;
            blk_z = rem / p.ny_tiles;
        }
    }
    const int n0 = blk_y * BN;
    const int Kz = p.kd, Ky = p.kh, Kx = p.kw, S = p.stride, Pz = p.pd, Py = p.ph, Px = p.pw;
    const int taps = Kz * Ky * Kx;
    const int Lz = p.dd, Ly = p.dh, Lx = p.dw;

    int cls = 0;
    if (MODE != MODE_WGRAD && p.n_classes > 1) {
        while (cls + 1 < p.n_classes && blk_x >= p.cls_tile_start[cls + 1]) ++cls;
    }
    const long tile_in_cls = (long)blk_x - ((MODE != MODE_WGRAD) ? p.cls_tile_start[cls] : 0);
    const long m0 = tile_in_cls * BM;
    int cz = 0, cy = 0, cx = 0, zf = 0, yf = 0, xf = 0, Dz = p.Dr, Dy = p.Hr, Dx = p.Wr;
    int nz = Kz, ny = Ky, nx = Kx;
    int ta0 = 0, tb0 = 0, tc0 = 0, tstep = 1;
    int pz0 = 0, py0 = 0, px0 = 0;
    const bool border = (MODE != MODE_WGRAD) && p.border;
    if (border) {
        const BorderClass bc = p.bcls[cls];
        pz0 = bc.pos0[0]; py0 = bc.pos0[1]; px0 = bc.pos0[2];
        Dz = bc.cnt[0]; Dy = bc.cnt[1]; Dx = bc.cnt[2];
        ta0 = bc.tlo[0]; tb0 = bc.tlo[1]; tc0 = bc.tlo[2];
        nz = bc.tcnt[0]; ny = bc.tcnt[1]; nx = bc.tcnt[2];
    } else if (MODE == MODE_DGRAD) {
        cz = cls / (S * S); cy = (cls / S) % S; cx = cls % S;
        zf = ((cz - Pz) % S + S) % S; yf = ((cy - Py) % S + S) % S; xf = ((cx - Px) % S + S) % S;
        Dz = zf < p.Dr ? (p.Dr - zf + S - 1) / S : 0;
        Dy = yf < p.Hr ? (p.Hr - yf + S - 1) / S : 0;
// ... 349 lines not shown
        float af[MT][KH], bf[NT][KH];
#pragma unroll
        for (int i = 0; i < MT; ++i) {
            const int r = wm * WTM + i * 32 + l32;
            if (A_ROWK) {
#pragma unroll
                for (int u = 0; u < KH / 4; ++u) {
                    const float4 v = *reinterpret_cast<const float4*>(Ab + r * LDK + h * KH + 4 * u);
                    af[i][4 * u] = v.x; af[i][4 * u + 1] = v.y; af[i][4 * u + 2] = v.z; af[i][4 * u + 3] = v.w;
                }
            } else {
#pragma unroll
                for (int t = 0; t < KH; ++t) af[i][t] = Ab[(h * KH + t) * BM + r];
            }
        }
#pragma unroll
        for (int j = 0; j < NT; ++j) {
            const int c = wn * WTN + j * 32 + l32;
            if (B_ROWK) {
#pragma unroll
                for (int u = 0; u < KH / 4; ++u) {
                    const float4 v = *reinterpret_cast<const float4*>(Bb + c * LDK + h * KH + 4 * u);
                    bf[j][4 * u] = v.x; bf[j][4 * u + 1] = v.y; bf[j][4 * u + 2] = v.z; bf[j][4 * u + 3] = v.w;
                }
            } else {
#pragma unroll
                for (int t = 0; t < KH; ++t) bf[j][t] = Bb[(h * KH + t) * BN + c];
            }
        }
        __builtin_amdgcn_sched_barrier(0);
        constexpr int NMF = KH * MT * NT;
        static_assert(NPARTS <= NMF, "more gather pieces than MFMAs");
#pragma unroll
        for (int g = 0; g < NMF; ++g) {
            const int t = g / (MT * NT), i = (g / NT) % MT, j = g % NT;
            acc[i][j] = __builtin_amdgcn_mfma_f32_32x32x2f32(af[i][t], bf[j][t], acc[i][j], 0, 0, 0);
            if (g < NPARTS) {
                load_part(kt + 2, more2, g, SetCur{});
                asm volatile("" ::: "memory");
                __builtin_amdgcn_sched_barrier(0);
            }
        }
        __builtin_amdgcn_sched_barrier(0);
        store_tile(buf ^ 1, SetOther{});
        __syncthreads();
    };

    if (kt0 < kt1) {
        load_tile(kt0, true, Set0{});
        store_tile(0, Set0{});
        load_tile(kt0 + 1, kt0 + 1 < kt1, Set1{});
    }
    __syncthreads();

    int kt = kt0;
    for (; kt + 1 < kt1; kt += 2) {
        iteration(kt, 0, Set0{});
        iteration(kt + 1, 1, Set1{});
    }
    if (kt < kt1) iteration(kt, 0, Set0{});

    float* outp = (p.nbatch ? p.out_tab[blockIdx.y] : p.out) + (long)blk_z * p.slab_stride;
    const bool direct = (p.slab_stride == 0);
    const bool mapped = (MODE != MODE_WGRAD) && p.n_classes > 1;
#pragma unroll
    for (int i = 0; i < MT; ++i)
#pragma unroll
    for (int j = 0; j < NT; ++j) {
        const int col = n0 + wn * WTN + j * 32 + l32;
#pragma unroll
        for (int r = 0; r < 16; ++r) {
            const int trow = wm * WTM + i * 32 + (r & 3) + 8 * (r >> 2) + 4 * h;
            long row = m0 + trow;
            bool ok = row < M_here && col < p.Ncols;
            if (mapped) { row = rowmap[trow]; ok = ok && row >= 0; }
            if (ok) {
                const long o = row * p.Ncols + col;
                float v = acc[i][j][r];
                if (direct) {
                    if (p.res) v += p.res[p.res_bcast ? (long)col : o];
                    if (p.relu) v = fmaxf(v, 0.f);
                    if (p.mask) v = (p.mask[o] > 0.f) ? v : 0.f;
                }
                outp[o] = v;
            }
        }
    }
}

__global__ __launch_bounds__(256) void splitk_reduce_kernel(const float* slabs, int n_slabs,
                                                           long slab_stride, float* out,
                                                           const float* res, const float* mask,
                                                           int relu, long n4, int res_mod = 0) {
    for (long i = (long)blockIdx.x * 256 + threadIdx.x; i < n4; i += (long)gridDim.x * 256) {
        float4 s = ld4(slabs + 4 * i);
        for (int z = 1; z < n_slabs; ++z) {
            float4 v = ld4(slabs + (long)z * slab_stride + 4 * i);
            s.x += v.x; s.y += v.y; s.z += v.z; s.w += v.w;
        }
        if (res) { float4 v = ld4(res + (res_mod ? (4 * i) % res_mod : 4 * i)); s.x += v.x; s.y += v.y; s.z += v.z; s.w += v.w; }
        if (relu) { s.x = fmaxf(s.x, 0.f); s.y = fmaxf(s.y, 0.f); s.z = fmaxf(s.z, 0.f); s.w = fmaxf(s.w, 0.f); }
        if (mask) {
            float4 v = ld4(mask + 4 * i);
            s.x = v.x > 0.f ? s.x : 0.f; s.y = v.y > 0.f ? s.y : 0.f;
            s.z = v.z > 0.f ? s.z : 0.f; s.w = v.w > 0.f ? s.w : 0.f;
        }
        *reinterpret_cast<float4*>(out + 4 * i) = s;
    }
}

constexpr int MI_REDUCE_BATCH = 24;
struct SplitDesc { const float* slabs; float* out; long slab_stride; long n4; int n_slabs; int pad; };
struct SplitBatch { SplitDesc d[MI_REDUCE_BATCH]; };
__global__ __launch_bounds__(256) void splitk_reduce_batch_kernel(SplitBatch bt) {
    const SplitDesc& d = bt.d[blockIdx.y];
    for (long i = (long)blockIdx.x * 256 + threadIdx.x; i < d.n4; i += (long)gridDim.x * 256) {
        float4 s = ld4(d.slabs + 4 * i);
        for (int z = 1; z < d.n_slabs; ++z) {
            float4 v = ld4(d.slabs + (long)z * d.slab_stride + 4 * i);
            s.x += v.x; s.y += v.y; s.z += v.z; s.w += v.w;
        }
        *reinterpret_cast<float4*>(d.out + 4 * i) = s;
    }
}

struct Plan { int bm, bn, bk, splits; long tiles_x; };

int env_int(const char* name) {
    const char* v = getenv(name);
    return v ? atoi(v) : 0;
}

bool conv_arith_bf16x3() {
    const char* v = getenv("MI_CONV_ARITH");
    return !(v && v[0] == 'f');
}

template <class F>
Plan make_plan(int mode, bool stem, long M, int Ncols, long red_len, int red_ch, F tiles_x_of) {
    Plan pl;
    (void)mode; (void)stem;
    pl.bm = 64;
    pl.bk = (red_ch == 0 || red_ch % 32 == 0) ? 32 : 16;
    pl.bn = 64;
    if (int v = env_int("MI_CONV_BM")) pl.bm = (v == 128) ? 128 : 64;
    if (int v = env_int("MI_CONV_BN")) pl.bn = (v == 128 && Ncols % 128 == 0) ? 128 : 64;
    if (int v = env_int("MI_CONV_BK")) if ((v == 16 || v == 32 || v == 64) && (red_ch == 0 || red_ch % v == 0)) pl.bk = v;
    if (pl.bk != 32 || stem) pl.bn = 64;
    if (pl.bk == 64 && (stem || pl.bm != 128)) pl.bk = 32;
    {
        const char* nv = getenv("MI_CONV_NARROW");
        if (mode == MODE_FWD && !stem && Ncols <= 32 && pl.bk == 32 && pl.bm == 64 && pl.bn == 64 && conv_arith_bf16x3() &&
            !(nv && atoi(nv) == 0) && tiles_x_of(128) >= 512) { pl.bm = 128; pl.bn = 32; }
    }
    pl.tiles_x = tiles_x_of(pl.bm);
    const long tiles = pl.tiles_x * ((Ncols + pl.bn - 1) / pl.bn);
    const long nk = (red_len + pl.bk - 1) / pl.bk;
    int splits = 1;
    {
        const long min_slices = 128 / pl.bk;
        long max_splits = nk / min_slices > 0 ? nk / min_slices : 1;
        if (max_splits > 128) max_splits = 128;
        double best = 1e30;
        for (long sp = 1; sp <= max_splits; ++sp) {
            const long per = (nk + sp - 1) / sp;
            if ((sp - 1) * per >= nk) continue;
            const long blocks = tiles * sp;
            const long per_cu = (blocks + 255) / 256;
            const double rate = per_cu == 1 ? 1.4 : (double)per_cu;
            double cost = rate * (double)(per + 6);
            if (sp > 1) cost += 2.0 + 0.05 * (double)sp;
            if (cost < best - 1e-9) { best = cost; splits = (int)sp; }
        }
    }
    if (int v = env_int("MI_CONV_SPLITS")) splits = v;
    pl.splits = splits < 1 ? 1 : splits;
    return pl;
}

template <int MODE, bool STEM>
int launch_mode(const ConvParams& p, const Plan& pl, hipStream_t s) {
    dim3 grid((unsigned)(pl.tiles_x * ((p.Ncols + pl.bn - 1) / pl.bn) * pl.splits), (unsigned)std::max(1, p.nbatch));
    if constexpr (!STEM) {
        if constexpr (MODE == MODE_FWD) {
            if (conv_arith_bf16x3() && pl.bm == 128 && pl.bn == 32 && pl.bk == 32) {
                hipLaunchKernelGGL((conv_igemm_kernel<MODE, 128, 32, 32, false, true>), grid, dim3(NTHREADS), 0, s, p);
                MI_RETURN_IF_LAUNCH_FAILED();
                return MI_OK;
            }
        }
        if (conv_arith_bf16x3() && pl.bm == 64 && pl.bn == 64 && (pl.bk == 32 || pl.bk == 16)) {
            if (pl.bk == 32) hipLaunchKernelGGL((conv_igemm_kernel<MODE, 64, 64, 32, false, true>), grid, dim3(NTHREADS), 0, s, p);
            else hipLaunchKernelGGL((conv_igemm_kernel<MODE, 64, 64, 16, false, true>), grid, dim3(NTHREADS), 0, s, p);
            MI_RETURN_IF_LAUNCH_FAILED();
            return MI_OK;
        }
    }
#define MI_LAUNCH(BM_, BN_, BK_) \
    hipLaunchKernelGGL((conv_igemm_kernel<MODE, BM_, BN_, BK_, STEM>), grid, dim3(NTHREADS), 0, s, p)
    if (pl.bn == 128 && !STEM) {
        if (pl.bm == 128) MI_LAUNCH(128, 128, 32); else MI_LAUNCH(64, 128, 32);
    } else if (pl.bm == 128 && pl.bk == 64 && !STEM) MI_LAUNCH(128, 64, 64);
    else if (pl.bm == 128 && pl.bk == 32) MI_LAUNCH(128, 64, 32);
    else if (pl.bm == 128) MI_LAUNCH(128, 64, 16);
    else if (pl.bk == 32) MI_LAUNCH(64, 64, 32);
    else MI_LAUNCH(64, 64, 16);
#undef MI_LAUNCH
    MI_RETURN_IF_LAUNCH_FAILED();
    return MI_OK;
}

struct Geom {
    int N, Di, Hi, Wi, Ci, Do, Ho, Wo, Co, kd, kh, kw, stride, pd, ph, pw;
    int dd = 1, dh = 1, dw = 1;
};

bool geom_ok(const Geom& g) {
    if (g.N <= 0 || g.Di <= 0 || g.Hi <= 0 || g.Wi <= 0 || g.Ci <= 0 || g.Co <= 0) return false;
    if (g.kd <= 0 || g.kd > 7 || g.kh <= 0 || g.kh > 7 || g.kw <= 0 || g.kw > 7) return false;
    if (g.stride <= 0 || g.stride > 2 || g.pd < 0 || g.ph < 0 || g.pw < 0) return false;
    if ((g.Ci % 16 && g.Ci != 1) || g.Co % 16) return false;
    if ((long)g.N * g.Di * g.Hi * g.Wi >= (1l << 31)) return false;
    if (g.dd < 1 || g.dh < 1 || g.dw < 1 || g.dd > 36 || g.dh > 36 || g.dw > 36) return false;
    if ((g.dd > 1 || g.dh > 1 || g.dw > 1) && (g.stride != 1 || g.Ci == 1)) return false;
    return true;
}
Geom from_public(const mi_conv_geom& p) {
    Geom g{p.N, p.Di, p.Hi, p.Wi, p.Ci, 0, 0, 0, p.Co, p.kd, p.kh, p.kw, p.stride, p.pd, p.ph, p.pw, p.dd, p.dh, p.dw};
    const int s = p.stride > 0 ? p.stride : 1;
    g.Do = (p.Di + 2 * p.pd - p.dd * (p.kd - 1) - 1) / s + 1;
    g.Ho = (p.Hi + 2 * p.ph - p.dh * (p.kh - 1) - 1) / s + 1;
    g.Wo = (p.Wi + 2 * p.pw - p.dw * (p.kw - 1) - 1) / s + 1;
    return g;
}
Geom make_geom(int N, int Di, int Hi, int Wi, int Ci, int Co, int k, int stride, int pad) {
    return from_public(mi_conv_geom{N, Di, Hi, Wi, Ci, Co, k, k, k, stride, pad, pad, pad, 1, 1, 1});
}
bool public_geom(const mi_conv_geom* pg, Geom* g) {
    if (!pg) return false;
    *g = from_public(*pg);
    return geom_ok(*g) && g->Do > 0 && g->Ho > 0 && g->Wo > 0;
}

void dgrad_class(const Geom& g, int c, long* rows, int* ntaps) {
    const int S = g.stride;
    const int Ps[3] = {g.pd, g.ph, g.pw}, Ks[3] = {g.kd, g.kh, g.kw};
    const int cc[3] = {c / (S * S), (c / S) % S, c % S};
    const int dims[3] = {g.Di, g.Hi, g.Wi};
    long r = g.N;
    int t = 1;
    for (int a = 0; a < 3; ++a) {
        const int f = ((cc[a] - Ps[a]) % S + S) % S;
        r *= f < dims[a] ? (dims[a] - f + S - 1) / S : 0;
        t *= cc[a] < Ks[a] ? (Ks[a] - cc[a] + S - 1) / S : 0;
    }
    *rows = r; *ntaps = t;
}

struct AxisRun { int pos0, cnt, tlo, tcnt; };

int axis_runs(int mode, int n_pos, int n_src, int K, int S, int P, int L, AxisRun* runs, int max_runs) {
    int nr = 0;
    for (int o = 0; o < n_pos; ++o) {
        int lo = K, hi = -1;
        for (int t = 0; t < K; ++t) {
            const int src = (mode == MODE_FWD) ? o * S - P + t * L : o + P - t * L;
            if (src >= 0 && src < n_src) { lo = std::min(lo, t); hi = std::max(hi, t); }
        }
        const int tlo = hi < lo ? 0 : lo, tcnt = hi < lo ? 0 : hi - lo + 1;
        if (nr && runs[nr - 1].tlo == tlo && runs[nr - 1].tcnt == tcnt) { ++runs[nr - 1].cnt; continue; }
        if (nr == max_runs) return -1;
        runs[nr++] = AxisRun{o, 1, tlo, tcnt};
    }
    return nr;
}

bool build_border_classes(int mode, const Geom& g, ConvParams* p) {
    if (g.Ci == 1 || (mode == MODE_DGRAD && g.stride != 1) || mode == MODE_WGRAD) return false;
    if (env_int("MI_CONV_NO_BORDER")) return false;
    AxisRun rz[3], ry[3], rx[3];
    const bool f = (mode == MODE_FWD);
    const int nz = axis_runs(mode, f ? g.Do : g.Di, f ? g.Di : g.Do, g.kd, g.stride, g.pd, g.dd, rz, 3);
// ... 71 lines not shown
        }
    } else if (mode == MODE_DGRAD && build_border_classes(mode, g, &p)) {
        p.Dg = g.Do; p.Hg = g.Ho; p.Wg = g.Wo; p.Cg = g.Co;
        p.Dr = g.Di; p.Hr = g.Hi; p.Wr = g.Wi;
        p.M = Min; p.Ncols = g.Ci;
        plan_border(st, g.N, g.Co, mode, stem);
    } else if (mode == MODE_DGRAD) {
        if (stem) return MI_E_UNSUPPORTED;
        p.Dg = g.Do; p.Hg = g.Ho; p.Wg = g.Wo; p.Cg = g.Co;
        p.Dr = g.Di; p.Hr = g.Hi; p.Wr = g.Wi;
        p.M = Min; p.Ncols = g.Ci;
        const int nc = g.stride * g.stride * g.stride;
        p.n_classes = nc;
        long rows[MAX_CLASSES]; int nt[MAX_CLASSES]; int max_t = 0;
        for (int c = 0; c < nc; ++c) { dgrad_class(g, c, &rows[c], &nt[c]); max_t = std::max(max_t, nt[c]); }
        auto tiles_of = [&](int bm) { long t = 0; for (int c = 0; c < nc; ++c) t += (rows[c] + bm - 1) / bm; return t; };
        st->pl = make_plan(mode, stem, p.M, p.Ncols, (long)std::max(max_t, 1) * g.Co, g.Co, tiles_of);
        long acc = 0;
        for (int c = 0; c < nc; ++c) { p.cls_tile_start[c] = (int)acc; acc += (rows[c] + st->pl.bm - 1) / st->pl.bm; }
        p.cls_tile_start[nc] = (int)acc;
    } else {
        p.Dg = g.Di; p.Hg = g.Hi; p.Wg = g.Wi; p.Cg = g.Ci;
        p.Dr = g.Do; p.Hr = g.Ho; p.Wr = g.Wo;
        p.M = (long)taps * g.Ci; p.Ncols = g.Co; p.n_red_vox = Mout;
        const long M = p.M;
        st->pl = make_plan(mode, stem, p.M, p.Ncols, Mout, 0, [M](int bm) { return (M + bm - 1) / bm; });
    }
    magic31(p.Dr, &p.mgD, &p.shD); magic31(p.Hr, &p.mgH, &p.shH); magic31(p.Wr, &p.mgW, &p.shW);
    const long x_bytes = 4 * Min * g.Ci, y_bytes = 4 * Mout * g.Co, w_bytes = 4l * taps * g.Ci * g.Co;
    const long ab = (mode == MODE_DGRAD) ? y_bytes : x_bytes, bb = (mode == MODE_WGRAD) ? y_bytes : w_bytes;
    if (ab >= 0x7fff0000l || bb >= 0x7fff0000l) return MI_E_UNSUPPORTED;
    p.a_bytes = (unsigned)ab; p.b_bytes = (unsigned)bb;
    p.splits = st->pl.splits;
    p.ny_tiles = (p.Ncols + st->pl.bn - 1) / st->pl.bn;
    p.tiles_x = (int)st->pl.tiles_x;
    p.fold = (p.n_classes > 1 && !env_int("MI_CONV_NO_FOLD")) ? 1 : 0;
    p.wbox = (mode == MODE_WGRAD && !stem && !env_int("MI_CONV_NO_BORDER")) ? 1 : 0;
    if (p.wbox) {
        ConvParams tmp = ConvParams{};
        p.wbox = build_border_classes(MODE_FWD, g, &tmp) ? 1 : 0;
    }
    return MI_OK;
}

bool is_stem7(const Geom& g) {
    return g.Ci == 1 && g.kd == 7 && g.kh == 7 && g.kw == 7 && g.stride == 2 && g.pd == 3 && g.ph == 3 && g.pw == 3 &&
           g.dd == 1 && g.dh == 1 && g.dw == 1;
}

int direct3_kind(const Geom& g) {
    return mi_direct3_kind(g.N, g.Di, g.Hi, g.Wi, g.Ci, g.Co, g.kd, g.kh, g.kw, g.stride, g.pd, g.ph, g.pw, g.dd, g.dh, g.dw);
}
bool is_cube2(const Geom& g) {
    return mi_cube2_usable(g.N, g.Di, g.Hi, g.Wi, g.Ci, g.Co, g.kd, g.kh, g.kw, g.stride, g.pd, g.ph, g.pw, g.dd, g.dh, g.dw);
}
size_t direct3_ws_bytes(const Geom& g) {
    if (is_cube2(g)) return mi_cube2_slab_bytes(g.N, g.Ci);
    const int kind = direct3_kind(g);
    if (!kind) return 0;
    size_t b = mi_align_up(mi_direct3_wimg_bytes_kind(kind), 256);
    if (kind == 1 || kind == 5) b = std::max(b, mi_direct3_wgrad_slab_bytes());
    if (kind == 2) b = std::max(b, mi_direct3s_wgrad_slab_bytes());
    if (kind == 3 || kind == 4) b = std::max(b, mi_direct3x_wgrad_slab_bytes(kind));
    return b;
}

size_t conv_ws_bytes(const Geom& g) {
    size_t best = is_stem7(g) ? std::max(mi_stem7_wgrad_workspace_bytes(g.N, g.Di, g.Hi, g.Wi, g.Co), mi_stem7_fwd_workspace_bytes()) : 0;
    best = std::max(best, direct3_ws_bytes(g));
    if (mi_pair_wgrad_usable(g.N, g.Di, g.Hi, g.Wi, g.Ci, g.Co, g.kd, g.kh, g.kw, g.stride, g.pd, g.ph, g.pw, g.dd, g.dh, g.dw))
        best = std::max(best, mi_pair_wgrad_slab_bytes(g.N, g.Di, g.Ci, g.Co, g.kd, g.stride));
    for (int mode = 0; mode < 3; ++mode) {
        Setup st;
        if (setup_conv(mode, g, &st)) continue;
        if (st.pl.splits > 1) best = std::max(best, sizeof(float) * (size_t)st.p.M * st.p.Ncols * st.pl.splits);
    }
    return best + 256;
}

thread_local const char* g_last_conv_kernel = "none";

int run_conv(int mode, const Geom& g, const float* a_src, const float* b_src, float* out,
             const float* res, const float* mask, int relu, void* ws, size_t ws_bytes, hipStream_t s,
             int* defer_splits = nullptr, int res_bcast = 0) {
    if (defer_splits) *defer_splits = 1;
    if (mode != MODE_WGRAD && g.N > 1) {
        const long in_per = (long)g.Di * g.Hi * g.Wi * g.Ci, out_per = (long)g.Do * g.Ho * g.Wo * g.Co;
        const long a_per = (mode == MODE_FWD) ? in_per : out_per, o_per = (mode == MODE_FWD) ? out_per : in_per;
        if (4 * a_per * g.N >= 0x7fff0000l) {
            Geom lo = g, hi = g;
            lo.N = g.N / 2; hi.N = g.N - lo.N;
            int rc = run_conv(mode, lo, a_src, b_src, out, res, mask, relu, ws, ws_bytes, s, nullptr, res_bcast);
            if (rc) return rc;
            const long ao = a_per * lo.N, oo = o_per * lo.N;
            return run_conv(mode, hi, a_src + ao, b_src, out + oo, (res && !res_bcast) ? res + oo : res,
                            mask ? mask + oo : nullptr, relu, ws, ws_bytes, s, nullptr, res_bcast);
        }
    }
    if (is_stem7(g) && !env_int("MI_CONV_NO_STEM") && !res_bcast) {
        int rc = MI_E_UNSUPPORTED;
        if (mode == MODE_FWD)
            rc = mi_stem7_fwd(a_src, b_src, out, res, relu, g.N, g.Di, g.Hi, g.Wi, g.Co, conv_arith_bf16x3() ? 1 : 0, ws,
                              ws_bytes, s);
        else if (mode == MODE_WGRAD) rc = mi_stem7_wgrad(a_src, b_src, out, g.N, g.Di, g.Hi, g.Wi, g.Co,
                                                         (conv_arith_bf16x3() && !env_int("MI_STEM_WGRAD_F32")) ? 1 : 0, ws, ws_bytes, s);
        if (rc != MI_E_UNSUPPORTED) { g_last_conv_kernel = mode == MODE_FWD ? "stem_fwd" : "stem_wgrad"; return rc; }
    }
    if (conv_arith_bf16x3() && g.Di == 1 && g.Hi == 1 && g.Wi == 1 && g.kd == 1 && g.kh == 1 && g.kw == 1 && g.stride == 1 &&
        g.pd == 0 && g.ph == 0 && g.pw == 0 && !mask && !relu && (!res || res_bcast)) {
        const long xe = (long)g.N * g.Ci, ye = (long)g.N * g.Co, we = (long)g.Ci * g.Co;
        g_last_conv_kernel = "small_gemm";
        if (mode == MODE_FWD && mi_small_gemm_usable(g.N, g.Co, g.Ci))
            return mi_small_gemm_launch(a_src, g.Ci, 1, xe, b_src, g.Co, 1, we, res, out, g.N, g.Co, g.Ci, s);
        if (mode == MODE_DGRAD && !res && mi_small_gemm_usable(g.N, g.Ci, g.Co))
            return mi_small_gemm_launch(a_src, g.Co, 1, ye, b_src, 1, g.Co, we, nullptr, out, g.N, g.Ci, g.Co, s);
        if (mode == MODE_WGRAD && mi_small_gemm_usable(g.Ci, g.Co, g.N))
            return mi_small_gemm_launch(a_src, 1, g.Ci, xe, b_src, g.Co, 1, ye, nullptr, out, g.Ci, g.Co, g.N, s);
    }
    const int dkind = (conv_arith_bf16x3() && !res_bcast) ? direct3_kind(g) : 0;
    const size_t dimg = mi_align_up(mi_direct3_wimg_bytes_kind(dkind), 256);
    if (mode != MODE_WGRAD && dkind && ws && ws_bytes >= dimg) {
        const float* wl[1] = {b_src};
        void* il[1] = {ws};
        const int dg[1] = {mode == MODE_DGRAD ? 1 : 0}, kd[1] = {dkind};
        int rc = mi_direct3_prep_kind(wl, il, dg, kd, 1, s);
        if (rc) return rc;
        g_last_conv_kernel = dkind == 1 ? "direct3" : dkind == 2 ? "direct3s" : dkind == 3 ? "direct3 (128 channels)" : dkind == 4 ? "direct3s (256 channels)" : "direct3h (8 x 8 tiles)";
        if (dkind == 1) return mi_direct3_launch(a_src, ws, out, res, mask, relu, g.N, g.Di, s);
        if (dkind == 4) return mi_direct3s_launch256(a_src, ws, out, res, mask, relu, g.N, s);
        if (dkind == 5) return mi_direct3h_launch(a_src, ws, out, res, mask, relu, g.N, g.Di, g.Hi, g.Wi, s);
        if (dkind == 3) return mi_direct3_launch128(a_src, ws, out, res, mask, relu, g.N, g.Di, s);
        return mi_direct3s_launch(a_src, ws, out, res, mask, relu, g.N, s);
    }
    if (mode != MODE_WGRAD && conv_arith_bf16x3() && !res_bcast && is_cube2(g) && ws && ws_bytes >= mi_cube2_slab_bytes(g.N, g.Ci)) {
        g_last_conv_kernel = "cube2 + reduce";
        int rc = mi_cube2_launch(mode == MODE_DGRAD ? 1 : 0, a_src, b_src, (float*)ws, g.N, g.Ci, s);
        if (rc) return rc;
        return mi_direct3_finish_slabs((const float*)ws, mi_cube2_splits(), (long)g.N * 8 * g.Ci, out, res, mask, relu, s);
    }
    if (mode == MODE_WGRAD && conv_arith_bf16x3() &&
        mi_pair_wgrad_usable(g.N, g.Di, g.Hi, g.Wi, g.Ci, g.Co, g.kd, g.kh, g.kw, g.stride, g.pd, g.ph, g.pw, g.dd, g.dh, g.dw))
    {
        const int splits = mi_pair_wgrad_splits(g.N, g.Di, g.Ci, g.Co, g.kd, g.stride);
        if (splits == 1 || (ws && ws_bytes >= mi_pair_wgrad_slab_bytes(g.N, g.Di, g.Ci, g.Co, g.kd, g.stride))) {
            g_last_conv_kernel = splits > 1 ? "pair_wgrad + reduce" : "pair_wgrad";
            int rc = mi_pair_wgrad_launch(a_src, b_src, out, (float*)ws, g.N, g.Di, g.Ci, g.Co, g.kd, g.stride, s);
            if (rc || splits == 1) return rc;
            if (defer_splits) { *defer_splits = splits; return MI_OK; }
            return mi_direct3_finish_slabs((const float*)ws, splits, (long)g.kd * g.kh * g.kw * g.Ci * g.Co, out, nullptr, nullptr, 0, s);
        }
    }
    if (mode == MODE_WGRAD && dkind == 1 && ws && ws_bytes >= mi_direct3_wgrad_slab_bytes()) {
        g_last_conv_kernel = "direct3_wgrad + reduce";
        int rc = mi_direct3_wgrad_launch(a_src, b_src, (float*)ws, g.N, g.Di, s);
        if (rc) return rc;
        const int splits = mi_direct3_wgrad_splits();
        if (defer_splits) { *defer_splits = splits; return MI_OK; }
        const long out_elems = 27l * g.Ci * g.Co, n4 = out_elems / 4;
        hipLaunchKernelGGL(splitk_reduce_kernel, dim3((unsigned)std::min<long>((n4 + 255) / 256, 2048)), dim3(256), 0, s,
                           (const float*)ws, splits, out_elems, out, (const float*)nullptr, (const float*)nullptr, 0, n4);
        MI_RETURN_IF_LAUNCH_FAILED();
        return MI_OK;
    }
    if (mode == MODE_WGRAD && dkind == 2 && ws && ws_bytes >= mi_direct3s_wgrad_slab_bytes() && env_int("MI_D3S_WGRAD")) {
        g_last_conv_kernel = "direct3s_wgrad + reduce";
        const float* xs[1] = {a_src};
        const float* dys[1] = {b_src};
        float* sl[1] = {(float*)ws};
        int rc = mi_direct3s_wgrad_launch_batch(xs, dys, sl, 1, g.N, s);
        if (rc) return rc;
        const int splits = mi_direct3s_wgrad_splits(1);
        if (defer_splits) { *defer_splits = splits; return MI_OK; }
        return mi_direct3_finish_slabs((const float*)ws, splits, 27l * g.Ci * g.Co, out, nullptr, nullptr, 0, s);
    }
    if (mode == MODE_WGRAD && dkind == 5 && g.Hi % 8 == 0 && g.Wi % 8 == 0 && ws && ws_bytes >= mi_direct3_wgrad_slab_bytes() &&
        !env_int("MI_NO_D3T_WGRAD")) {
        g_last_conv_kernel = "direct3_wgrad (8 x 8 tiles) + reduce";
        int rc = mi_direct3t_wgrad_launch(a_src, b_src, (float*)ws, g.N, g.Di, g.Hi, g.Wi, s);
        if (rc) return rc;
        const int splits = mi_direct3_wgrad_splits();
        if (defer_splits) { *defer_splits = splits; return MI_OK; }
        return mi_direct3_finish_slabs((const float*)ws, splits, 27l * g.Ci * g.Co, out, nullptr, nullptr, 0, s);
    }
    if (mode == MODE_WGRAD && dkind == 3 && !env_int("MI_NO_D3X_WGRAD") && ws &&
        ws_bytes >= mi_direct3x_wgrad_slab_bytes(dkind)) {
        g_last_conv_kernel = "direct3_wgrad (128 channels) + reduce";
        int rc = mi_direct3x_wgrad_launch(dkind, a_src, b_src, (float*)ws, g.N, g.Di, s);
        if (rc) return rc;
        const int splits = mi_direct3x_wgrad_splits(dkind);
        if (defer_splits) { *defer_splits = splits; return MI_OK; }
        return mi_direct3_finish_slabs((const float*)ws, splits, 27l * g.Ci * g.Co, out, nullptr, nullptr, 0, s);
    }
    Setup st;
    int rc = setup_conv(mode, g, &st);
    if (rc) return rc;
    g_last_conv_kernel = st.pl.splits > 1 ? "implicit GEMM + reduce" : "implicit GEMM";
    ConvParams& p = st.p;
    Plan& pl = st.pl;
    p.a_src = a_src; p.b_src = b_src; p.res = res; p.mask = mask; p.relu = relu;
    p.res_bcast = res_bcast;
    const bool stem = (g.Ci == 1);
    const long out_elems = p.M * p.Ncols;
    if (pl.splits > 1) {
        size_t need = sizeof(float) * (size_t)out_elems * pl.splits;
        if (!ws || ws_bytes < need) pl.splits = 1;
    }
    p.splits = pl.splits;
    if (pl.splits > 1) { p.out = (float*)ws; p.slab_stride = out_elems; }
    else { p.out = out; p.slab_stride = 0; }
    if (mode == MODE_FWD) rc = stem ? launch_mode<MODE_FWD, true>(p, pl, s) : launch_mode<MODE_FWD, false>(p, pl, s);
    else if (mode == MODE_DGRAD) rc = launch_mode<MODE_DGRAD, false>(p, pl, s);
    else rc = stem ? launch_mode<MODE_WGRAD, true>(p, pl, s) : launch_mode<MODE_WGRAD, false>(p, pl, s);
    if (rc) return rc;
    if (pl.splits > 1 && defer_splits) { *defer_splits = pl.splits; return MI_OK; }
    if (pl.splits > 1) {
        long n4 = out_elems / 4;
        int blocks = (int)std::min<long>((n4 + 255) / 256, 2048);
        hipLaunchKernelGGL(splitk_reduce_kernel, dim3(blocks), dim3(256), 0, s, (const float*)ws,
                           pl.splits, out_elems, out, res, mask, relu, n4, res_bcast ? p.Ncols : 0);
        MI_RETURN_IF_LAUNCH_FAILED();
    }
    return MI_OK;
}

}

int mi_direct3_finish_slabs(const float* slabs, int n_slabs, long out_elems, float* out, const float* res, const float* mask,
                            int relu, hipStream_t s) {
    const long n4 = out_elems / 4;
    hipLaunchKernelGGL(splitk_reduce_kernel, dim3((unsigned)std::min<long>((n4 + 255) / 256, 2048)), dim3(256), 0, s, slabs,
                       n_slabs, out_elems, out, res, mask, relu, n4, 0);
    MI_RETURN_IF_LAUNCH_FAILED();
    return MI_OK;
}

extern "C" size_t mi_conv_workspace_bytes(const mi_conv_geom* pg) {
    Geom g;
    return public_geom(pg, &g) ? conv_ws_bytes(g) : 0;
}

extern "C" int mi_conv_fwd_f32(const float* x, const float* w, float* y, const float* res, int res_is_bias, int relu,
                               const mi_conv_geom* pg, void* ws, size_t ws_bytes, mi_stream_t stream) {
    Geom g;
    if (!x || !w || !y || (res_is_bias && !res) || !public_geom(pg, &g)) return MI_E_ARG;
    return run_conv(MODE_FWD, g, x, w, y, res, nullptr, relu, ws, ws_bytes, (hipStream_t)stream, nullptr, res_is_bias ? 1 : 0);
}

extern "C" int mi_conv_dgrad_f32(const float* dy, const float* w, float* dx, const float* res, const float* mask,
                                 const mi_conv_geom* pg, void* ws, size_t ws_bytes, mi_stream_t stream) {
    Geom g;
    if (!dy || !w || !dx || !public_geom(pg, &g)) return MI_E_ARG;
    return run_conv(MODE_DGRAD, g, dy, w, dx, res, mask, 0, ws, ws_bytes, (hipStream_t)stream);
}

extern "C" int mi_conv_wgrad_f32(const float* x, const float* dy, float* dw, const mi_conv_geom* pg, void* ws, size_t ws_bytes,
                                 int* splits_out, mi_stream_t stream) {
    Geom g;
    if (!x || !dy || !dw || !public_geom(pg, &g)) return MI_E_ARG;
    return run_conv(MODE_WGRAD, g, x, dy, dw, nullptr, nullptr, 0, ws, ws_bytes, (hipStream_t)stream, splits_out);
}

extern "C" const char* mi_debug_last_conv_kernel(void) { return g_last_conv_kernel; }
void mi_note_conv_kernel(const char* name) { g_last_conv_kernel = name; }

extern "C" int mi_linear_bn_fwd_f32(const float* x, const float* w, const float* bias, float* xlin, float* y, int M, int Ci,
                                    int Co, const float* gamma, const float* beta, float eps, float momentum,
                                    float* running_mean, float* running_var, long long* num_batches_tracked,
                                    float* save_mean_invstd, int relu, mi_stream_t stream) {
    if (!x || !w || !xlin || !y || !save_mean_invstd || M <= 0 || Ci <= 0 || Co <= 0) return MI_E_ARG;
    if ((running_mean == nullptr) != (running_var == nullptr)) return MI_E_ARG;
    if (M > 64 || !conv_arith_bf16x3() || !mi_small_gemm_usable(M, Co, Ci) || env_int("MI_NO_LINEAR_BN")) return MI_E_UNSUPPORTED;
    MiSmallGemmBN bn = {y, gamma, beta, eps, momentum, running_mean, running_var, num_batches_tracked, save_mean_invstd, relu,
                        nullptr};
    return mi_small_gemm_launch(x, Ci, 1, (long)M * Ci, w, Co, 1, (long)Ci * Co, bias, xlin, M, Co, Ci, (hipStream_t)stream, &bn);
}

extern "C" int mi_linear_stats_fwd_f32(const float* x, const float* w, const float* bias, float* xlin, double* sums, int M, int Ci,
                                       int Co, mi_stream_t stream) {
    if (!x || !w || !xlin || !sums || M <= 0 || Ci <= 0 || Co <= 0) return MI_E_ARG;
    if (M > 64 || !conv_arith_bf16x3() || !mi_small_gemm_usable(M, Co, Ci) || env_int("MI_NO_LINEAR_BN")) return MI_E_UNSUPPORTED;
    MiSmallGemmBN bn = {};
    bn.sums_only = sums;
    return mi_small_gemm_launch(x, Ci, 1, (long)M * Ci, w, Co, 1, (long)Ci * Co, bias, xlin, M, Co, Ci, (hipStream_t)stream, &bn);
}

extern "C" size_t mi_conv3d_stem_stats_workspace_bytes(int N, int Di, int Hi, int Wi, int Co) {
    Geom g = make_geom(N, Di, Hi, Wi, 1, Co, 7, 2, 3);
    if (!geom_ok(g) || !is_stem7(g) || Co != 64) return 0;
    return mi_stem7_fwd_stats_workspace_bytes(N, Di, Hi, Wi);
}

extern "C" int mi_conv3d_stem_stats_f32(const float* x, const float* w, float* y, int N, int Di, int Hi, int Wi, int Co,
                                        double* sums, void* ws, size_t ws_bytes, mi_stream_t stream) {
    Geom g = make_geom(N, Di, Hi, Wi, 1, Co, 7, 2, 3);
    if (!x || !w || !y || !sums || !geom_ok(g)) return MI_E_ARG;
    if (!is_stem7(g) || !conv_arith_bf16x3() || env_int("MI_CONV_NO_STEM") || env_int("MI_STEM_NO_STATS")) return MI_E_UNSUPPORTED;
    return mi_stem7_fwd(x, w, y, nullptr, 0, N, Di, Hi, Wi, Co, 1, ws, ws_bytes, (hipStream_t)stream, sums);
}

extern "C" int mi_linear_fwd_f32(const float* x, const float* w, const float* bias, float* y, int M, int Ci, int Co,
                                 void* ws, size_t ws_bytes, mi_stream_t stream) {
    Geom g = make_geom(M, 1, 1, 1, Ci, Co, 1, 1, 0);
    if (!x || !w || !y || !geom_ok(g)) return MI_E_ARG;
    return run_conv(MODE_FWD, g, x, w, y, bias, nullptr, 0, ws, ws_bytes, (hipStream_t)stream, nullptr, bias ? 1 : 0);
}

extern "C" int mi_conv_wgrad_batch_f32(const float* const* xs, const float* const* dys, float* const* dws, void* const* wss, int nb,
                                       const mi_conv_geom* pg, size_t ws_bytes, int* splits_out, mi_stream_t stream) {
    Geom g;
    if (!xs || !dys || !dws || !wss || !splits_out || nb < 1 || !public_geom(pg, &g)) return MI_E_ARG;
    for (int i = 0; i < nb; ++i) if (!xs[i] || !dys[i] || !dws[i]) return MI_E_ARG;
    if (nb < 2 || !conv_arith_bf16x3() || env_int("MI_NO_WGRAD_BATCH")) return MI_E_UNSUPPORTED;
    hipStream_t s = (hipStream_t)stream;
    float* slabs[MI_WGRAD_BATCH_MAX];
    if (nb > MI_WGRAD_BATCH_MAX) return MI_E_UNSUPPORTED;
    for (int i = 0; i < nb; ++i) slabs[i] = (float*)wss[i];
    if (is_stem7(g)) return MI_E_UNSUPPORTED;
    if (mi_pair_wgrad_usable(g.N, g.Di, g.Hi, g.Wi, g.Ci, g.Co, g.kd, g.kh, g.kw, g.stride, g.pd, g.ph, g.pw, g.dd, g.dh, g.dw)) {
        if (nb > mi_pair_wgrad_batch_max()) return MI_E_UNSUPPORTED;
        const int splits = mi_pair_wgrad_splits(g.N, g.Di, g.Ci, g.Co, g.kd, g.stride);
        if (splits > 1) {
            if (ws_bytes < mi_pair_wgrad_slab_bytes(g.N, g.Di, g.Ci, g.Co, g.kd, g.stride)) return MI_E_UNSUPPORTED;
            for (int i = 0; i < nb; ++i) if (!wss[i]) return MI_E_ARG;
        }
        g_last_conv_kernel = splits > 1 ? "pair_wgrad x nb + reduce" : "pair_wgrad x nb";
        *splits_out = splits;
        return mi_pair_wgrad_launch_batch(xs, dys, dws, slabs, nb, g.N, g.Di, g.Ci, g.Co, g.kd, g.stride, s);
    }
    if (direct3_kind(g) == 1) {
        if (nb > mi_direct3_wgrad_batch_max() || ws_bytes < mi_direct3_wgrad_slab_bytes()) return MI_E_UNSUPPORTED;
        for (int i = 0; i < nb; ++i) if (!wss[i]) return MI_E_ARG;
        g_last_conv_kernel = "direct3_wgrad x nb + reduce";
        *splits_out = mi_direct3_wgrad_batch_splits(nb);
        return mi_direct3_wgrad_launch_batch(xs, dys, slabs, nb, g.N, g.Di, s);
    }
    if (direct3_kind(g) == 2 && env_int("MI_D3S_WGRAD")) {
        if (nb > mi_direct3_wgrad_batch_max() || ws_bytes < mi_direct3s_wgrad_slab_bytes()) return MI_E_UNSUPPORTED;
        for (int i = 0; i < nb; ++i) if (!wss[i]) return MI_E_ARG;
        g_last_conv_kernel = "direct3s_wgrad x nb + reduce";
        *splits_out = mi_direct3s_wgrad_splits(nb);
        return mi_direct3s_wgrad_launch_batch(xs, dys, slabs, nb, g.N, s);
    }
    {
        const int dk = direct3_kind(g);
        if (dk == 3 && !env_int("MI_NO_D3X_WGRAD")) return MI_E_UNSUPPORTED;
        if (dk == 5 && g.Hi % 8 == 0 && g.Wi % 8 == 0 && !env_int("MI_NO_D3T_WGRAD")) return MI_E_UNSUPPORTED;
    }
    Setup st;
    int rc = setup_conv(MODE_WGRAD, g, &st);
    if (rc) return rc;
    if (g.Ci == 1) return MI_E_UNSUPPORTED;
    ConvParams& p = st.p;
    Plan& pl = st.pl;
    int splits = pl.splits;
    if (const char* v = getenv("MI_WGRAD_BATCH_SPLITS")) { const int sv = atoi(v); if (sv >= 1 && sv <= pl.splits) splits = sv; }
    const long out_elems = p.M * p.Ncols;
    if (splits > 1) {
        if (ws_bytes < sizeof(float) * (size_t)out_elems * splits) return MI_E_UNSUPPORTED;
        for (int i = 0; i < nb; ++i) if (!wss[i]) return MI_E_ARG;
    }
    pl.splits = splits;
    p.splits = splits;
    p.res = nullptr; p.mask = nullptr; p.relu = 0; p.res_bcast = 0;
    p.a_src = xs[0]; p.b_src = dys[0];
    p.nbatch = nb;
    for (int i = 0; i < nb; ++i) { p.a_tab[i] = xs[i]; p.b_tab[i] = dys[i]; p.out_tab[i] = splits > 1 ? slabs[i] : dws[i]; }
    p.out = p.out_tab[0];
    p.slab_stride = splits > 1 ? out_elems : 0;
    g_last_conv_kernel = splits > 1 ? "implicit GEMM x nb + reduce" : "implicit GEMM x nb";
    rc = launch_mode<MODE_WGRAD, false>(p, pl, s);
    if (rc) return rc;
    *splits_out = splits;
    return MI_OK;
}

extern "C" int mi_splitk_reduce_batch(const void* const* slabs, void* const* outs, const int* n_slabs, const long* out_elems,
                                      int n, mi_stream_t stream) {
    if (n <= 0) return MI_OK;
    if (!slabs || !outs || !n_slabs || !out_elems) return MI_E_ARG;
    for (int i0 = 0; i0 < n; i0 += MI_REDUCE_BATCH) {
        SplitBatch bt = {};
        const int m = std::min(MI_REDUCE_BATCH, n - i0);
        long max4 = 1;
        for (int i = 0; i < m; ++i) {
            if (!slabs[i0 + i] || !outs[i0 + i] || n_slabs[i0 + i] < 1 || (out_elems[i0 + i] & 3)) return MI_E_ARG;
            bt.d[i] = SplitDesc{(const float*)slabs[i0 + i], (float*)outs[i0 + i], out_elems[i0 + i], out_elems[i0 + i] / 4,
                                n_slabs[i0 + i], 0};
            max4 = std::max(max4, bt.d[i].n4);
        }
        const int bx = (int)std::min<long>((max4 + 255) / 256, 256);
        hipLaunchKernelGGL(splitk_reduce_batch_kernel, dim3(bx, m), dim3(256), 0, (hipStream_t)stream, bt);
        MI_RETURN_IF_LAUNCH_FAILED();
    }
    return MI_OK;
}
```

### cet_pick_amd/hipops.py

```python
import ctypes
import os
import torch
import torch.nn as nn

from . import _lib as L


PROFILE = None
PROFILE_REPEAT = 8


def _prof_run(tag, flops, fn):
    fn()
    if PROFILE is not None:
        e0 = torch.cuda.Event(enable_timing=True)
        e1 = torch.cuda.Event(enable_timing=True)
        e0.record()
        for _ in range(PROFILE_REPEAT):
            fn()
        e1.record()
        PROFILE.append((tag, flops, e0, e1, PROFILE_REPEAT))


STAMPS = None
# ... 605 lines not shown
    n, d, h, wd, ci = shape5
    co = w.shape[0]
    if not nd5 and dy.is_cuda and p2d_usable(tuple(in_shape), ci, co, k3, stride, p3, dil):
        if res is not None:
            _f32c(res, "res")
        if mask is not None:
            _f32c(mask, "mask")
        return _p2d_call(dy, w, True, res, mask, False, "dgrad")
    dx = torch.empty(tuple(in_shape), dtype=torch.float32, device=dy.device)
    lib = L.lib()
    d3 = _k3(dil, nd5) if dil is not None else (1, 1, 1)
    g = _Geom(shape5, co, k3, stride, p3, d3)
    flops = 2.0 * dy.numel() * ci * g.taps
    img = _cached_image(w, True, n, d, h, wd, k3, stride, p3) if (nd5 and dil is None) else None
    if img is not None:
        ws = _ws(lib.mi_conv3d_direct_workspace_bytes(n, ci), dy.device, "conv")
        L.check(lib.mi_conv3d_direct_f32(L.ptr(dy), L.ptr(img), L.ptr(dx), L.ptr(res), L.ptr(mask), 0, n, d, h, wd, ci,
                                         L.ptr(ws), ws.numel(), L.stream()), "mi_conv3d_direct_f32")
        return dx
    if nd5 and dil is None and _cube2_final(lib, n, d, h, wd, ci, co, k3, stride, p3):
        ws = _cube2_ws(lib, n, ci, dy.device)
        def call():
            return _cube2_call(lib, dy, w, dx, res, mask, 0, 1, n, ci, ws)
        _prof_run("dgrad", flops, call)
        return dx
    ws = g.workspace(dy.device)
    def call():
        return L.check(lib.mi_conv_dgrad_f32(L.ptr(dy), L.ptr(w), L.ptr(dx), L.ptr(res), L.ptr(mask), g.ref, L.ptr(ws), ws.numel(),
                                             L.stream()), "mi_conv_dgrad_f32")
    _prof_run("dgrad", flops, call)
    return dx


def conv_fwd_s2_block(x, w, w_ds):
    if x.dim() != 5 or w_ds is None:
        return None
    n, g, g2, g3, ci = x.shape
    co = w.shape[0]
    lib = L.lib()
    if not x.is_cuda or g != g2 or g != g3 or not lib.mi_conv3d_s2_fwd_usable(n, g, ci, co) or not (_phys_ok(w) and _phys_ok(w_ds)):
        return None
    _f32c(x, "x")
    hmid = torch.empty((n, g // 2, g // 2, g // 2, co), dtype=torch.float32, device=x.device)
    r = torch.empty_like(hmid)
    img = ACTIVE_IMAGES.get_s2(w, False) if (ACTIVE_IMAGES is not None and PROFILE is None) else None
    if img is not None:
        L.check(lib.mi_conv3d_s2_fwd_img_f32(L.ptr(x), L.ptr(img), L.ptr(hmid), L.ptr(r), n, g, ci, co, L.stream()),
                "mi_conv3d_s2_fwd_img_f32")
        return hmid, r
    ws = _ws(lib.mi_conv3d_s2_fwd_workspace_bytes(ci, co), x.device, "conv_s2f")
    def call():
        return L.check(lib.mi_conv3d_s2_fwd_f32(L.ptr(x), L.ptr(w), L.ptr(w_ds), L.ptr(hmid), L.ptr(r), n, g, ci, co, L.ptr(ws),
                                                ws.numel(), L.stream()), "mi_conv3d_s2_fwd_f32")
    _prof_run("fwd", 2.0 * hmid.numel() * ci * 28, call)
    return hmid, r


def conv_dgrad_s2_block(dh, d2, w, w_ds, in_shape, res=None, mask=None):
    n, g, _, _, ci = in_shape
    co = w.shape[0]
    lib = L.lib()
    if not dh.is_cuda or not lib.mi_conv3d_s2_dgrad_usable(n, g, ci, co):
        return None
    if in_shape[1] != in_shape[2] or in_shape[2] != in_shape[3] or not (_phys_ok(w) and (w_ds is None or _phys_ok(w_ds))):
        return None
    _f32c(dh, "dh")
    if d2 is not None:
        _f32c(d2, "d2")
    dx = torch.empty(tuple(in_shape), dtype=torch.float32, device=dh.device)
    img = ACTIVE_IMAGES.get_s2(w, True) if (ACTIVE_IMAGES is not None and PROFILE is None and d2 is not None) else None
    if img is not None:
        L.check(lib.mi_conv3d_s2_dgrad_img_f32(L.ptr(dh), L.ptr(d2), L.ptr(img), L.ptr(dx), L.ptr(res), L.ptr(mask), n, g, ci, co,
                                               L.stream()), "mi_conv3d_s2_dgrad_img_f32")
        return dx
    ws = _ws(lib.mi_conv3d_s2_dgrad_workspace_bytes(ci, co), dh.device, "conv_s2")
    def call():
        return L.check(lib.mi_conv3d_s2_dgrad_f32(L.ptr(dh), L.ptr(d2), L.ptr(w), L.ptr(w_ds), L.ptr(dx), L.ptr(res), L.ptr(mask), n, g,
                                                  ci, co, L.ptr(ws), ws.numel(), L.stream()), "mi_conv3d_s2_dgrad_f32")
    _prof_run("dgrad", 2.0 * dh.numel() * ci * (27 + (1 if d2 is not None else 0)), call)
    return dx


DEFERRED_WGRADS = None


def flush_wgrad_reduces():
    global DEFERRED_WGRADS
    items = DEFERRED_WGRADS
    if not items:
        return
    L.check(L.lib().mi_splitk_reduce_batch(L.host_array([it[0].data_ptr() for it in items]), L.host_array([it[1].data_ptr() for it in items]),
                                           L.host_array([it[2] for it in items], ctypes.c_int),
                                           L.host_array([it[3] for it in items], ctypes.c_long), len(items), L.stream()),
            "mi_splitk_reduce_batch")
    del items[:]


SIDE_WGRADS = None
SIDE_ROWS_MAX = int(os.environ.get("CETPICK_SIDE_ROWS", "32768"))


def _side_or_now(fn, rows):
    if SIDE_WGRADS is not None and rows <= SIDE_ROWS_MAX and (PROFILE is None or isinstance(fn, _WgradJob)):
        SIDE_WGRADS.append(fn)
        return True
    fn()
    return False


class _WgradJob:
    __slots__ = ("x", "dy", "tgt", "slab", "geom", "param", "flops")

    def __init__(self, x, dy, tgt, slab, geom, param=None, flops=0.0):
        self.x, self.dy, self.tgt, self.slab, self.geom, self.param, self.flops = x, dy, tgt, slab, geom, param, flops

    def __call__(self):
        splits = ctypes.c_int(0)
        L.check(L.lib().mi_conv_wgrad_f32(L.ptr(self.x), L.ptr(self.dy), L.ptr(self.tgt), self.geom.ref, L.ptr(self.slab),
                                          self.slab.numel(), ctypes.addressof(splits), L.stream()), "mi_conv_wgrad_f32")
        if splits.value > 1:
            DEFERRED_WGRADS.append((self.slab, self.tgt, int(splits.value), self.tgt.numel()))


WGRAD_BATCH = os.environ.get("CETPICK_WGRAD_BATCH", "1") != "0"
WGRAD_BATCH_MAX = 4

_BACKWARD_END = None
_BACKWARD_END_TASK = -1


def _defer_to_backward_end(job):
    global _BACKWARD_END, _BACKWARD_END_TASK
    try:
        torch.autograd.Variable._execution_engine.queue_callback(_flush_backward_end)
    except RuntimeError:
        return False
    task = torch._C._current_graph_task_id()
    if _BACKWARD_END is not None and task != _BACKWARD_END_TASK:
        for stale in _BACKWARD_END:
            if stale.param is not None:
                stale.param._mi_wgrad_pending = False
        _BACKWARD_END = None
    if _BACKWARD_END is None:
        _BACKWARD_END = []
        _BACKWARD_END_TASK = task
    _BACKWARD_END.append(job)
    if job.param is not None:
        job.param._mi_wgrad_pending = True
    return True


def _flush_backward_end():
    global _BACKWARD_END, DEFERRED_WGRADS
    items, _BACKWARD_END = _BACKWARD_END, None
    if not items:
        return
    saved, DEFERRED_WGRADS = DEFERRED_WGRADS, []
    try:
        run_wgrad_jobs(items)
        flush_wgrad_reduces()
    finally:
        DEFERRED_WGRADS = saved


def _launch_wgrad_group(jobs):
    rc = -3
    if len(jobs) > 1:
        splits = ctypes.c_int(0)
        rc = L.lib().mi_conv_wgrad_batch_f32(L.host_array([j.x.data_ptr() for j in jobs]), L.host_array([j.dy.data_ptr() for j in jobs]),
                                             L.host_array([j.tgt.data_ptr() for j in jobs]), L.host_array([j.slab.data_ptr() for j in jobs]),
                                             len(jobs), jobs[0].geom.ref, jobs[0].slab.numel(), ctypes.addressof(splits), L.stream())
        if rc == 0 and splits.value > 1:
            for j in jobs:
                DEFERRED_WGRADS.append((j.slab, j.tgt, int(splits.value), j.tgt.numel()))
    if rc == -3:
        for j in jobs:
            j()
    else:
        L.check(rc, "mi_conv_wgrad_batch_f32")


def run_wgrad_jobs(items):
    groups, order = {}, []
    for it in items:
        if isinstance(it, _WgradJob) and it.param is not None:
            it.param._mi_wgrad_pending = False
        if isinstance(it, _WgradJob) and WGRAD_BATCH and DEFERRED_WGRADS is not None:
            key = it.geom.key + (it.slab.numel(),)
            if key not in groups:
                groups[key] = []
                order.append(groups[key])
            groups[key].append(it)
        else:
            order.append(it)
    if PROFILE is not None:
        _run_wgrad_jobs_profiled(order)
        return
    for it in order:
        if not isinstance(it, list):
            it()
            continue
        for i0 in range(0, len(it), WGRAD_BATCH_MAX):
            _launch_wgrad_group(it[i0:i0 + WGRAD_BATCH_MAX])


def _run_wgrad_jobs_profiled(order):
    for it in order:
        if not isinstance(it, list):
            if isinstance(it, _WgradJob):
                it = [it]
            else:
                it()
                continue
        for i0 in range(0, len(it), WGRAD_BATCH_MAX):
            jobs = it[i0:i0 + WGRAD_BATCH_MAX]

            def call(jobs=jobs):
                global DEFERRED_WGRADS
                saved, DEFERRED_WGRADS = DEFERRED_WGRADS, []
                try:
                    _launch_wgrad_group(jobs)
                    flush_wgrad_reduces()
                finally:
                    DEFERRED_WGRADS = saved
            _prof_run("wgrad", sum(j.flops for j in jobs), call)


def conv_wgrad_into(x, dy, param, k, stride, pad, dil=None):
    nd5 = x.dim() == 5
    k3, p3 = _k3(k, nd5), _p3(pad, nd5)
    n, d, h, wd, ci = _as5d(x).shape
    co = dy.shape[-1]
    lib = L.lib()
    if getattr(param, "_mi_wgrad_pending", False):
        if DEFERRED_WGRADS is not None:
            raise L.HipExtensionError("MocoStepEngine: a convolution applied twice in one backward pass (its first weight gradient is "
                                      "still queued for the side stream) - run this model without the step engine")
        _flush_backward_end()
    dest = _GradInto(param)
    tgt = dest.tgt
    flops = 2.0 * dy.numel() * ci * k3[0] * k3[1] * k3[2]
    if (not nd5 and x.is_cuda and ci == 1 and tuple(k3) == (1, 3, 3) and stride == 1 and tuple(p3) == (0, 1, 1) and dil is None
            and _stem3_ok(int(co)) and _phys_ok(param)):
        _f32c(x, "x"), _f32c(dy, "dy")
        ws = _ws(lib.mi_conv2d_stem3_workspace_bytes(int(co)), x.device, "stem3")
        def call():
            return L.check(lib.mi_conv2d_stem3_wgrad_f32(L.ptr(x), L.ptr(dy), L.ptr(tgt), n, h, wd, int(co), L.ptr(ws), ws.numel(),
                                                         L.stream()), "mi_conv2d_stem3_wgrad_f32")
        with dest:
            _prof_run("wgrad", flops, call)
        return
    p2d_ws = (int(lib.mi_conv2d_p2d_wgrad_workspace_bytes(n, h, wd, ci))
              if (not nd5 and x.is_cuda and p2d_usable(tuple(x.shape), ci, int(co), k3, stride, p3, dil) and _phys_ok(param)
                  and not os.environ.get("MI_NO_P2D_WGRAD")) else 0)
    if p2d_ws:
        _f32c(x, "x"), _f32c(dy, "dy")
        ws = _ws(p2d_ws, x.device, "p2d_wgrad")
        def call():
            return L.check(lib.mi_conv2d_p2d_wgrad_f32(L.ptr(x), L.ptr(dy), L.ptr(tgt), n, h, wd, ci, L.ptr(ws), ws.numel(), L.stream()),
                           "mi_conv2d_p2d_wgrad_f32")
        with dest:
            _prof_run("wgrad", flops, call)
# ... 1431 lines not shown
```

### include/cetpick_hip.h

```cpp
#ifndef CETPICK_HIP_H
#define CETPICK_HIP_H

#include <stddef.h>
#include <stdint.h>

#ifdef __cplusplus
extern "C" {
#endif

typedef void* mi_stream_t;

#define MI_OK 0
#define MI_E_ARG (-1)
#define MI_E_WORKSPACE (-2)
#define MI_E_UNSUPPORTED (-3)

int mi_abi_version(void);
int mi_graph_node_counts(void* graph, int* counts);
int mi_debug_stamp(void* slot, mi_stream_t stream);
const char* mi_debug_last_conv_kernel(void);
const char* mi_build_arch(void);


int mi_sigmoid_clamp(float* x, float* y, size_t n, mi_stream_t stream);
// ... 15 lines not shown

enum { MI_ORDER_XYZ = 0, MI_ORDER_XZY = 1, MI_ORDER_YXZ = 2, MI_ORDER_ZXY = 3 };

int mi_rec_reorder(const void* src, int mrc_mode, int d0, int d1, int d2, int order, int compress,
                   float* dst, mi_stream_t stream);
size_t mi_vol_stats_workspace_bytes(long n_slices, long slice_elems);
int mi_vol_stats(const float* x, long n_slices, long slice_elems, double* stats, void* ws, size_t ws_bytes,
                 mi_stream_t stream);
int mi_zscore(const float* x, float* y, long n_slices, long slice_elems, const double* stats,
              mi_stream_t stream);
int mi_zscore_quantize_minmax(const float* x, float* y, long n_slices, long slice_elems, const double* stats,
                              double mi, double ma, int flat_zero, mi_stream_t stream);

size_t mi_dog_pick_workspace_bytes(int D, int H, int W, int n_sigmas);
int mi_dog_pick(const float* rec, int D, int H, int W, const float* sigmas_host, int n_sigmas,
                int k, int border_z, int nms_d, float* heat_out, float* scores, int32_t* coords,
                int32_t* n_out, int max_out, float* cutoff_out, void* workspace,
                size_t workspace_bytes, mi_stream_t stream);

size_t mi_greedy_nms3d_workspace_bytes(int D, int H, int W);
int mi_greedy_nms3d(const float* vol, int D, int H, int W, float d, float scale, float threshold,
                    float* scores, int32_t* coords, int32_t* n_out, int max_out, void* workspace,
                    size_t workspace_bytes, mi_stream_t stream);


int mi_crop_normalize(const float* vol, int D, int H, int W, const int32_t* centres_xyz, int n,
                      int cz, int cy, int cx, int mode, int flip_x, float* out, mi_stream_t stream);

typedef struct mi_vol_desc {
    const float* vol;
    int32_t D, H, W, reserved;
} mi_vol_desc;
int mi_crop_normalize_table(const mi_vol_desc* vols, const int32_t* owner, const int32_t* centres_xyz,
                            const int32_t* shift_xyz, const int64_t* order, int64_t first, int n, int cz, int cy,
                            int cx, int mode, int flip_x, float* out, mi_stream_t stream);
int mi_u8_roundtrip_normalize(const float* x, float* y, size_t n, float mean, float std, mi_stream_t stream);

int mi_aug2d_params(const int64_t* sample_ids, int64_t n, uint64_t seed, int epoch, int view, int bbox, float flip_p,
                    float bright_lo, float bright_hi, float contrast_lo, float contrast_hi, float area_lo, float area_hi,
                    int32_t* table, mi_stream_t stream);
int mi_aug2d_apply(const float* bank, int64_t n_samples, int n_banks, const int64_t* sample_ids, const int32_t* table,
                   int64_t n, int bbox, float mean, float std, float* out, mi_stream_t stream);

typedef struct mi_aug2d3d_ranges {
    float flip_p, angle_lo, angle_hi, erase_p, scale_lo, scale_hi, ratio_lo, ratio_hi;
} mi_aug2d3d_ranges;
int mi_aug2d3d_params(const int64_t* sample_ids, int64_t n, uint64_t seed, int epoch, int bbox,
                      const mi_aug2d3d_ranges* strong, const mi_aug2d3d_ranges* weak, int32_t* table, mi_stream_t stream);
int mi_aug2d3d_apply(const float* patches_2d, const float* patches_3d, int64_t n_samples, int n_variants,
                     const int64_t* sample_ids, const int64_t* variants, const int32_t* table_strong,
                     const int32_t* table_weak, int64_t n, int bbox, float mean_2d, float std_2d, float mean_3d, float std_3d,
                     float* out, mi_stream_t stream);

typedef struct mi_tilt_desc {
    const float* tilts;
    const double* cos_sin;
    int32_t T, H, W, Zfull;
} mi_tilt_desc;
int mi_tilt_patches(const mi_tilt_desc* stacks, int n_stacks, const int32_t* owner, const int32_t* centres_xyz, int64_t n,
                    int cy, int cx, double bx, double by, float* out, uint8_t* valid, mi_stream_t stream);

int mi_semi_labels(float* hm, int D, int H, int W, const int32_t* centres_xyz, int64_t n, const float* stencil, int r,
                   int fill_unlabeled, mi_stream_t stream);
int mi_semi_pairs(const mi_vol_desc* tomos, const mi_vol_desc* labels, int n_tomos, const int32_t* owner,
                  const int32_t* centres_xyz, int64_t first, int n, int flip_y, float* input, float* input_aug, float* hm,
                  mi_stream_t stream);


typedef struct mi_conv_geom {
    int N, Di, Hi, Wi, Ci, Co, kd, kh, kw, stride, pd, ph, pw, dd, dh, dw;
} mi_conv_geom;

size_t mi_conv_workspace_bytes(const mi_conv_geom* g);
int mi_conv_fwd_f32(const float* x, const float* w, float* y, const float* res, int res_is_bias, int relu,
                    const mi_conv_geom* g, void* ws, size_t ws_bytes, mi_stream_t stream);
int mi_conv_dgrad_f32(const float* dy, const float* w, float* dx, const float* res, const float* mask,
                      const mi_conv_geom* g, void* ws, size_t ws_bytes, mi_stream_t stream);
int mi_conv_wgrad_f32(const float* x, const float* dy, float* dw, const mi_conv_geom* g, void* ws, size_t ws_bytes,
                      int* splits_out, mi_stream_t stream);
int mi_splitk_reduce_batch(const void* const* slabs, void* const* outs, const int* n_slabs, const long* out_elems, int n,
                           mi_stream_t stream);
int mi_conv_wgrad_batch_f32(const float* const* xs, const float* const* dys, float* const* dws, void* const* wss, int nb,
                            const mi_conv_geom* g, size_t ws_bytes, int* splits_out, mi_stream_t stream);

int mi_linear_bn_fwd_f32(const float* x, const float* w, const float* bias, float* xlin, float* y, int M, int Ci, int Co,
                         const float* gamma, const float* beta, float eps, float momentum, float* running_mean,
                         float* running_var, long long* num_batches_tracked, float* save_mean_invstd, int relu,
                         mi_stream_t stream);

int mi_linear_stats_fwd_f32(const float* x, const float* w, const float* bias, float* xlin, double* sums, int M, int Ci, int Co,
                            mi_stream_t stream);

size_t mi_conv3d_stem_stats_workspace_bytes(int N, int Di, int Hi, int Wi, int Co);
int mi_conv3d_stem_stats_f32(const float* x, const float* w, float* y, int N, int Di, int Hi, int Wi, int Co,
                             double* sums, void* ws, size_t ws_bytes, mi_stream_t stream);

int mi_linear_fwd_f32(const float* x, const float* w, const float* bias, float* y, int M, int Ci, int Co, void* ws,
                      size_t ws_bytes, mi_stream_t stream);

int mi_stem2d_fwd_bias_f32(const float* x, const float* w, const float* bias, float* y, int relu, int N, int H, int W,
                           mi_stream_t stream);
size_t mi_smallk_image_bytes(int K, int Co);
int mi_smallk_prep(const float* w, void* img, int K, int Co, mi_stream_t stream);
int mi_smallk_fwd_f32(const float* x, const void* img, const float* bias, float* y, int relu, long M, int Ci, int Co,
                      int ntaps, long plane, int D, mi_stream_t stream);
int mi_smallk_heads_fwd_f32(const float* x, const void* img, float* y_proj, const float* w_hm, float* y_hm, int k_hm, long M, int Ci,
                            long plane, int D, mi_stream_t stream);
size_t mi_conv3d_direct_wimg_bytes(int channels);
size_t mi_conv3d_direct_workspace_bytes(int N, int channels);
int mi_conv3d_direct_usable(int N, int Di, int Hi, int Wi, int Ci, int Co, int k, int stride, int pad);
int mi_conv3d_direct_prep(const void* const* w, void* const* img, const int* dgrad, const int* channels, int n,
                          mi_stream_t stream);
int mi_conv3d_direct_f32(const float* a, const void* wimg, float* out, const float* res, const float* mask, int relu,
                         int N, int Di, int Hi, int Wi, int channels, void* ws, size_t ws_bytes, mi_stream_t stream);

int mi_conv2d_p2d_usable(int N, int H, int W, int C);
size_t mi_conv2d_p2d_wimg_bytes(int C);
int mi_conv2d_p2d_prep(const void* const* w, void* const* img, const int* dgrad, const int* channels, int n, mi_stream_t stream);
int mi_conv2d_p2d_f32(const float* a, const void* wimg, float* out, const float* res, const float* mask, int relu, int N, int H, int W,
                      int C, mi_stream_t stream);
size_t mi_conv2d_p2d_wgrad_workspace_bytes(int N, int H, int W, int C);
int mi_conv2d_p2d_wgrad_f32(const float* x, const float* dy, float* dw, int N, int H, int W, int C, void* ws, size_t ws_bytes,
                            mi_stream_t stream);

size_t mi_conv2d_stem3_workspace_bytes(int Co);
int mi_conv2d_stem3_fwd_f32(const float* x, const float* w, float* y, int N, int H, int W, int Co, mi_stream_t stream);
int mi_conv2d_stem3_wgrad_f32(const float* x, const float* dy, float* dw, int N, int H, int W, int Co, void* ws, size_t ws_bytes,
                              mi_stream_t stream);

size_t mi_conv3d_cube2_workspace_bytes(int N, int C);
int mi_conv3d_cube2_usable(int N, int Di, int Hi, int Wi, int Ci, int Co, int k, int stride, int pad);
int mi_conv3d_cube2_f32(const float* a, const float* w, float* out, const float* res, const float* mask, int relu, int dgrad,
                        int N, int C, void* ws, size_t ws_bytes, mi_stream_t stream);

int mi_conv_d32_kind(int N, int D, int H, int W, int Ci, int Co, int kd, int kh, int kw, int dd, int dh, int dw);
size_t mi_conv_d32_image_bytes(int Ci, int ntap);
int mi_conv_d32_prep(const float* w, void* img, int Ci, int ntap, mi_stream_t stream);
size_t mi_conv_d64_image_bytes(int Ci, int ntap);
int mi_conv_d64_prep_co(const float* w, void* img, int Ci, int Co, int ntap, mi_stream_t stream);
int mi_conv_d32_1x1_fwd_f32(const float* x, const void* wimg, const float* bias, float* y, int relu, int N, int D, int H, int W,
                            int Ci, int Co, mi_stream_t stream);
int mi_conv_d32_fwd_pool_f32(const float* x, const void* wimg, const float* bias, float* y, float* y_pool, int relu, int N, int D, int H,
                             int W, int Ci, int Co, mi_stream_t stream);
int mi_conv_d32_fwd_pool_strided_f32(const float* x, const void* wimg, const float* bias, float* y, int y_cstride, float* y_pool, int relu,
                                     int N, int D, int H, int W, int Ci, int Co, mi_stream_t stream);
int mi_copy_channels_into(const float* src, int Cs, float* dst, int Ct, int c0, long M, mi_stream_t stream);
int mi_conv_d32_upconv_fwd_f32(const float* x, const void* wimg, const float* scale, const float* shift, float* out, int N, int H,
                               int W, int Ci, int Co, int Ho, int Wo, int cstride, mi_stream_t stream);
int mi_conv_d64_fwd_f32(const float* x, const void* wimg, const float* bias, float* y, int relu, int N, int D, int H, int W, int Ci,
                        int Co, mi_stream_t stream);
int mi_conv_d32_fwd_f32(const float* x, const void* wimg, const float* bias, float* y, int relu, int N, int D, int H, int W,
                        int Ci, int kind, mi_stream_t stream);
int mi_maxpool2d_ceil_fwd(const float* x, float* y, uint8_t* argmax, int N, int Hi, int Wi, int C, int k,
                          mi_stream_t stream);
int mi_maxpool2d_ceil_bwd(const float* dy, const uint8_t* argmax, float* dx, int N, int Hi, int Wi, int C,
                          int k, mi_stream_t stream);
int mi_shuffle2x2_fwd(const float* t, const float* bias, float* y, int N, int H, int W, int Co, int Ho, int Wo,
                      mi_stream_t stream);
int mi_upconv_tail_fwd(const float* t, const float* scale, const float* shift, const float* enc, float* out, int N, int H,
                       int W, int Co, int Ce, int Ho, int Wo, mi_stream_t stream);
int mi_shuffle2x2_bwd(const float* dy, float* dt, int N, int H, int W, int Co, int Ho, int Wo,
                      mi_stream_t stream);
int mi_concat_channels(const float* a, int Ca, const float* b, int Cb, float* out, long M, mi_stream_t stream);
int mi_split_channels(const float* dout, float* da, int Ca, float* db, int Cb, long M, mi_stream_t stream);
int mi_zhead_fwd(const float* x, const float* w, float* y, int N, int D, long P, int C, int K,
                 mi_stream_t stream);
// ... 153 lines not shown
```

Baseline: 43090 subtomograms/sec.

## Fuse split-K wgrad reduction into kernels via last-block ticket counters

```diff
diff --git a/cet_pick_amd/_lib.py b/cet_pick_amd/_lib.py
--- a/cet_pick_amd/_lib.py
+++ b/cet_pick_amd/_lib.py
@@ -64,6 +64,10 @@
     "mi_conv_dgrad_f32": (_I, [_P, _P, _P, _P, _P, _G, _P, _Z, _P]),
     "mi_conv_wgrad_f32": (_I, [_P, _P, _P, _G, _P, _Z, _P, _P]),
     "mi_conv_wgrad_batch_f32": (_I, [_P, _P, _P, _P, _I, _G, _Z, _P, _P]),
+    "mi_wgrad_ticket_bytes": (_Z, [_G, _I]),
+    "mi_conv3d_pair_wgrad_splits": (_I, [_I, _I, _I, _I, _I, _I]),
+    "mi_conv_wgrad_final_f32": (_I, [_P, _P, _P, _G, _P, _Z, _P, _Z, _P, _P]),
+    "mi_conv_wgrad_batch_final_f32": (_I, [_P, _P, _P, _P, _I, _G, _Z, _P, _Z, _P, _P]),
     "mi_stem2d_fwd_bias_f32": (_I, [_P, _P, _P, _P, _I, _I, _I, _I, _P]),
     "mi_upconv_tail_fwd": (_I, [_P, _P, _P, _P, _P] + [_I] * 7 + [_P]),
     "mi_smallk_image_bytes": (_Z, [_I, _I]),
diff --git a/cet_pick_amd/csrc/common.h b/cet_pick_amd/csrc/common.h
--- a/cet_pick_amd/csrc/common.h
+++ b/cet_pick_amd/csrc/common.h
@@ -37,6 +37,10 @@
     const float* res;
     const float* mask;
     int relu;
+};
+struct WgradFinal {
+    unsigned* tickets;
+    float* const* outs;
 };
 constexpr size_t MI_CUBE2_TICKET_BYTES = 16384;
 
diff --git a/cet_pick_amd/csrc/conv_cube2.hip b/cet_pick_amd/csrc/conv_cube2.hip
--- a/cet_pick_amd/csrc/conv_cube2.hip
+++ b/cet_pick_amd/csrc/conv_cube2.hip
@@ -171,8 +171,12 @@
     unsigned char order[PW_MAXTAP];
     unsigned short cnt[PW_MAXTAP];
     unsigned char lo[PW_MAXTAP][3], len[PW_MAXTAP][3];
+    unsigned* tickets;
+    float* fin[PW_MAXPROB];
 };
 
+constexpr int PW_ZC = 4;
+template <bool FINAL>
 __global__ __launch_bounds__(512, 2) void pair_wgrad_kernel(PairWgradParams p) {
     __shared__ __attribute__((aligned(16))) unsigned char lds[2 * PW_OP];
     const int tid = threadIdx.x, lane = tid & 63, wave = tid >> 6;
@@ -285,11 +289,52 @@
         for (int r = 0; r < 16; ++r) red[wave & 3][r][lane] = acc[r];
     }
     __syncthreads();
+    const long o0 = ((long)tap * p.CI + ib * 64 + 32 * wm + 4 * h) * p.CO + cb * 64 + 32 * wn + l32;
+    auto orow = [&](int r) { return (long)((r & 3) + 8 * (r >> 2)) * p.CO; };
     if (kh == 0) {
-        float* out = p.dw[blockIdx.y] + seg * p.slab_stride + ((long)tap * p.CI + ib * 64 + 32 * wm) * p.CO + cb * 64 + 32 * wn + l32;
-#pragma unroll
-        for (int r = 0; r < 16; ++r) out[(long)((r & 3) + 8 * (r >> 2) + 4 * h) * p.CO] = acc[r] + red[wave][r][lane];
-    }
+        float* out = p.dw[blockIdx.y] + seg * p.slab_stride + o0;
+#pragma unroll
+        for (int r = 0; r < 16; ++r) {
+            const float v = acc[r] + red[wave][r][lane];
+            if (!FINAL) out[orow(r)] = v;
+            else __hip_atomic_store(out + orow(r), v, __ATOMIC_RELAXED, __HIP_MEMORY_SCOPE_AGENT);
+        }
+    }
+    if (!FINAL) return;
+    asm volatile("s_waitcnt vmcnt(0)" ::: "memory");
+    __syncthreads();
+    unsigned* const s_last = reinterpret_cast<unsigned*>(lds + 4 * 16 * 64 * 4);
+    unsigned* ticket = p.tickets + (((long)blockIdx.y * p.ntaps + ts / p.S) * tiles + rem);
+    if (tid == 0) *s_last = (__hip_atomic_fetch_add(ticket, 1u, __ATOMIC_RELAXED, __HIP_MEMORY_SCOPE_AGENT) == (unsigned)(p.S - 1)) ? 1u : 0u;
+    __syncthreads();
+    if (!*s_last || kh == 1) return;
+    if (tid == 0) __hip_atomic_store(ticket, 0u, __ATOMIC_RELAXED, __HIP_MEMORY_SCOPE_AGENT);
+    const float* sl = p.dw[blockIdx.y] + o0;
+    float sum[16] = {};
+    for (int z0 = 0; z0 < p.S; z0 += PW_ZC) {
+        float part[PW_ZC][16];
+#pragma unroll
+        for (int k = 0; k < PW_ZC; ++k) {
+            const int zl = min(z0 + k, p.S - 1);
+#pragma unroll
+            for (int r = 0; r < 16; ++r)
+                part[k][r] = __hip_atomic_load(sl + (long)zl * p.slab_stride + orow(r), __ATOMIC_RELAXED, __HIP_MEMORY_SCOPE_AGENT);
+        }
+#pragma unroll
+        for (int k = 0; k < PW_ZC; ++k) {
+            const int z = z0 + k;
+            if (z < p.S) {
+#pragma unroll
+                for (int r = 0; r < 16; ++r) {
+                    const float v = z == seg ? acc[r] + red[wave][r][lane] : part[k][r];
+                    sum[r] = z == 0 ? v : sum[r] + v;
+                }
+            }
+        }
+    }
+    float* fin = p.fin[blockIdx.y] + o0;
+#pragma unroll
+    for (int r = 0; r < 16; ++r) fin[orow(r)] = sum[r];
 }
 
 struct SmallGemmParams {
@@ -525,8 +570,9 @@
 }
 
 int mi_pair_wgrad_batch_max() { return PW_MAXPROB; }
+size_t mi_pair_wgrad_ticket_bytes(int Ci, int Co, int k) { return sizeof(unsigned) * (size_t)PW_MAXPROB * k * k * k * (Ci / 64) * (Co / 64); }
 int mi_pair_wgrad_launch_batch(const float* const* xs, const float* const* dys, float* const* dws, float* const* slabs, int nb, int N,
-                               int Di, int Ci, int Co, int k, int stride, hipStream_t s) {
+                               int Di, int Ci, int Co, int k, int stride, hipStream_t s, const WgradFinal* fin) {
     if (nb < 1 || nb > PW_MAXPROB) return MI_E_ARG;
     PairWgradParams p = {};
     const PairGeom g = pair_geom(Di, k, stride, &p);
@@ -543,17 +589,24 @@
     for (int want = g.maxcnt; want >= 0; --want)
         for (int t = 0; t < g.ntaps; ++t)
             if (p.cnt[t] == want) p.order[n++] = (unsigned char)t;
-    hipLaunchKernelGGL(pair_wgrad_kernel, dim3((unsigned)(g.ntaps * (Ci / 64) * (Co / 64) * S), (unsigned)nb), dim3(512), 0, s, p);
+    const dim3 grid((unsigned)(g.ntaps * (Ci / 64) * (Co / 64) * S), (unsigned)nb);
+    if (fin && S > 1) {
+        p.tickets = fin->tickets;
+        for (int i = 0; i < nb; ++i) p.fin[i] = fin->outs[i];
+        hipLaunchKernelGGL(pair_wgrad_kernel<true>, grid, dim3(512), 0, s, p);
+    } else {
+        hipLaunchKernelGGL(pair_wgrad_kernel<false>, grid, dim3(512), 0, s, p);
+    }
     MI_RETURN_IF_LAUNCH_FAILED();
     return MI_OK;
 }
 int mi_pair_wgrad_launch(const float* x, const float* dy, float* dwt, float* slabs, int N, int Di, int Ci, int Co, int k, int stride,
-                         hipStream_t s) {
+                         hipStream_t s, const WgradFinal* fin) {
     const float* xs[1] = {x};
     const float* dys[1] = {dy};
     float* dws[1] = {dwt};
     float* sl[1] = {slabs};
-    return mi_pair_wgrad_launch_batch(xs, dys, dws, sl, 1, N, Di, Ci, Co, k, stride, s);
+    return mi_pair_wgrad_launch_batch(xs, dys, dws, sl, 1, N, Di, Ci, Co, k, stride, s, fin);
 }
 
 size_t mi_cube2_slab_bytes(int N, int C) { return sizeof(float) * (size_t)KQ * N * 8 * C; }
diff --git a/cet_pick_amd/csrc/conv_direct3.hip b/cet_pick_amd/csrc/conv_direct3.hip
--- a/cet_pick_amd/csrc/conv_direct3.hip
+++ b/cet_pick_amd/csrc/conv_direct3.hip
@@ -493,10 +493,13 @@
     unsigned bytes;
     int nprob, splits;
     int H, W;
+    unsigned* tickets;
+    float* out[WG_MAXPROB];
 };
 
 constexpr int W_HB = 3 * 2 * 8 * 128;
-template <bool V4, int CT, bool TILED = false>
+constexpr int WG_ZC = 4;
+template <bool V4, int CT, bool TILED = false, bool FINAL = false>
 __global__ __launch_bounds__(512, 2) void direct3_wgrad_kernel(Direct3WgradParams p) {
     __shared__ __attribute__((aligned(16))) unsigned char lds[2 * WBUF + (TILED ? 2 * W_HB : 16)];
     unsigned char* const halo = lds + 2 * WBUF;
@@ -742,16 +745,61 @@
             for (int r = 0; r < 16; ++r) red[(((wave & 3) * 3 + dx) * 16 + r) * 64 + lane] = acc[dx][r];
     }
     __syncthreads();
-    if (kh == 1) return;
-    float* out = p.slabs[pb] + (long)split * (NTAP * CT * CT);
+    if (!FINAL && kh == 1) return;
+    constexpr long SLAB = (long)NTAP * CT * CT;
+    float* out = p.slabs[pb] + (long)split * SLAB;
+    const long o0 = ((long)((dz * 3 + dy) * 3) * CT + ci0 + 32 * wm + 4 * h) * CT + co0 + 32 * wn + l32;
+    auto orow = [](int r) { return (long)((r & 3) + 8 * (r >> 2)) * CT; };
+    if (kh == 0) {
+#pragma unroll
+        for (int dx = 0; dx < 3; ++dx) {
+#pragma unroll
+            for (int r = 0; r < 16; ++r) {
+                const float v = acc[dx][r] + red[((wave * 3 + dx) * 16 + r) * 64 + lane];
+                float* dst = out + o0 + (long)dx * CT * CT + orow(r);
+                if (!FINAL) *dst = v;
+                else __hip_atomic_store(dst, v, __ATOMIC_RELAXED, __HIP_MEMORY_SCOPE_AGENT);
+            }
+        }
+    }
+    if (!FINAL) return;
+    asm volatile("s_waitcnt vmcnt(0)" ::: "memory");
+    __syncthreads();
+    unsigned* const s_last = reinterpret_cast<unsigned*>(lds + 2 * WBUF);
+    unsigned* ticket = p.tickets + (grp * p.nprob + pb);
+    if (tid == 0) *s_last = (__hip_atomic_fetch_add(ticket, 1u, __ATOMIC_RELAXED, __HIP_MEMORY_SCOPE_AGENT) == (unsigned)(p.splits - 1)) ? 1u : 0u;
+    __syncthreads();
+    if (!*s_last || kh == 1) return;
+    if (tid == 0) __hip_atomic_store(ticket, 0u, __ATOMIC_RELAXED, __HIP_MEMORY_SCOPE_AGENT);
+    const float* sl = p.slabs[pb];
+    float* fin = p.out[pb];
 #pragma unroll
     for (int dx = 0; dx < 3; ++dx) {
-        const int tap = (dz * 3 + dy) * 3 + dx;
-#pragma unroll
-        for (int r = 0; r < 16; ++r) {
-            const int ci = ci0 + 32 * wm + (r & 3) + 8 * (r >> 2) + 4 * h;
-            out[((long)tap * CT + ci) * CT + co0 + 32 * wn + l32] = acc[dx][r] + red[((wave * 3 + dx) * 16 + r) * 64 + lane];
-        }
+        const long od = o0 + (long)dx * CT * CT;
+        float sum[16] = {};
+        for (int z0 = 0; z0 < p.splits; z0 += WG_ZC) {
+            float part[WG_ZC][16];
+#pragma unroll
+            for (int k = 0; k < WG_ZC; ++k) {
+                const int zl = min(z0 + k, p.splits - 1);
+#pragma unroll
+                for (int r = 0; r < 16; ++r)
+                    part[k][r] = __hip_atomic_load(sl + (long)zl * SLAB + od + orow(r), __ATOMIC_RELAXED, __HIP_MEMORY_SCOPE_AGENT);
+            }
+#pragma unroll
+            for (int k = 0; k < WG_ZC; ++k) {
+                const int z = z0 + k;
+                if (z < p.splits) {
+#pragma unroll
+                    for (int r = 0; r < 16; ++r) {
+                        const float v = z == split ? acc[dx][r] + red[((wave * 3 + dx) * 16 + r) * 64 + lane] : part[k][r];
+                        sum[r] = z == 0 ? v : sum[r] + v;
+                    }
+                }
+            }
+        }
+#pragma unroll
+        for (int r = 0; r < 16; ++r) fin[od + orow(r)] = sum[r];
     }
 }
 
@@ -1066,11 +1114,26 @@
 size_t mi_direct3_wgrad_slab_bytes() { return sizeof(float) * (size_t)WG_SPLITS * NTAP * C * C; }
 int mi_direct3_wgrad_splits() { return WG_SPLITS; }
 
-int mi_direct3_wgrad_launch(const float* x, const float* dy, float* slabs, int N, int D, hipStream_t s) {
+namespace {
+template <bool V4, int CT, bool TILED>
+void wgrad_launch(Direct3WgradParams& p, unsigned groups, const WgradFinal* fin, hipStream_t s) {
+    const dim3 grid(groups * (unsigned)(p.nprob * p.splits));
+    if (fin) {
+        p.tickets = fin->tickets;
+        for (int i = 0; i < p.nprob; ++i) p.out[i] = fin->outs[i];
+        hipLaunchKernelGGL((direct3_wgrad_kernel<V4, CT, TILED, true>), grid, dim3(512), 0, s, p);
+    } else {
+        hipLaunchKernelGGL((direct3_wgrad_kernel<V4, CT, TILED, false>), grid, dim3(512), 0, s, p);
+    }
+}
+}
+size_t mi_direct3_wgrad_ticket_bytes() { return sizeof(unsigned) * 36 * WG_MAXPROB; }
+
+int mi_direct3_wgrad_launch(const float* x, const float* dy, float* slabs, int N, int D, hipStream_t s, const WgradFinal* fin) {
     Direct3WgradParams p = {};
     p.x[0] = x; p.dy[0] = dy; p.slabs[0] = slabs; p.N = N; p.D = D; p.bytes = (unsigned)(4l * N * D * PLANE * C);
     p.nprob = 1; p.splits = WG_SPLITS;
-    hipLaunchKernelGGL((direct3_wgrad_kernel<false, 64>), dim3(9 * WG_SPLITS), dim3(512), 0, s, p);
+    wgrad_launch<false, 64, false>(p, 9, fin, s);
     MI_RETURN_IF_LAUNCH_FAILED();
     return MI_OK;
 }
@@ -1082,13 +1145,13 @@
     return WG_BATCH_SPLITS;
 }
 int mi_direct3_wgrad_launch_batch(const float* const* xs, const float* const* dys, float* const* slabs, int nb, int N, int D,
-                                  hipStream_t s) {
+                                  hipStream_t s, const WgradFinal* fin) {
     if (nb < 1 || nb > WG_MAXPROB) return MI_E_ARG;
     Direct3WgradParams p = {};
     for (int i = 0; i < nb; ++i) { p.x[i] = xs[i]; p.dy[i] = dys[i]; p.slabs[i] = slabs[i]; }
     p.N = N; p.D = D; p.bytes = (unsigned)(4l * N * D * PLANE * C);
     p.nprob = nb; p.splits = mi_direct3_wgrad_batch_splits(nb);
-    hipLaunchKernelGGL((direct3_wgrad_kernel<false, 64>), dim3(9 * nb * p.splits), dim3(512), 0, s, p);
+    wgrad_launch<false, 64, false>(p, 9, fin, s);
     MI_RETURN_IF_LAUNCH_FAILED();
     return MI_OK;
 }
@@ -1101,24 +1164,25 @@
     if (const char* v = getenv("MI_D3SW_BATCH_SPLITS")) { const int sv = atoi(v); if (sv >= 1 && sv <= WS_SPLITS) return sv; }
     return WS_BATCH_SPLITS;
 }
-int mi_direct3s_wgrad_launch_batch(const float* const* xs, const float* const* dys, float* const* slabs, int nb, int N, hipStream_t s) {
+int mi_direct3s_wgrad_launch_batch(const float* const* xs, const float* const* dys, float* const* slabs, int nb, int N, hipStream_t s,
+                                   const WgradFinal* fin) {
     if (nb < 1 || nb > WG_MAXPROB || N < 1) return MI_E_ARG;
     Direct3WgradParams p = {};
     for (int i = 0; i < nb; ++i) { p.x[i] = xs[i]; p.dy[i] = dys[i]; p.slabs[i] = slabs[i]; }
     p.N = N; p.D = 1; p.bytes = (unsigned)(4l * N * PLANE * CS);
     p.nprob = nb; p.splits = mi_direct3s_wgrad_splits(nb);
-    hipLaunchKernelGGL((direct3_wgrad_kernel<true, 128>), dim3(36 * nb * p.splits), dim3(512), 0, s, p);
+    wgrad_launch<true, 128, false>(p, 36, fin, s);
     MI_RETURN_IF_LAUNCH_FAILED();
     return MI_OK;
 }
 
-int mi_direct3t_wgrad_launch(const float* x, const float* dy, float* slabs, int N, int D, int H, int W, hipStream_t s) {
+int mi_direct3t_wgrad_launch(const float* x, const float* dy, float* slabs, int N, int D, int H, int W, hipStream_t s, const WgradFinal* fin) {
     if (H % 8 || W % 8 || H < 8 || W < 8) return MI_E_UNSUPPORTED;
     Direct3WgradParams p = {};
     p.x[0] = x; p.dy[0] = dy; p.slabs[0] = slabs; p.N = N; p.D = D; p.H = H; p.W = W;
     p.bytes = (unsigned)(4l * N * D * H * W * C);
     p.nprob = 1; p.splits = WG_SPLITS;
-    hipLaunchKernelGGL((direct3_wgrad_kernel<false, 64, true>), dim3(9 * WG_SPLITS), dim3(512), 0, s, p);
+    wgrad_launch<false, 64, true>(p, 9, fin, s);
     MI_RETURN_IF_LAUNCH_FAILED();
     return MI_OK;
 }
@@ -1128,12 +1192,12 @@
     const size_t ct = kind == 3 ? 128 : 0;
     return sizeof(float) * (size_t)mi_direct3x_wgrad_splits(kind) * NTAP * ct * ct;
 }
-int mi_direct3x_wgrad_launch(int kind, const float* x, const float* dy, float* slabs, int N, int D, hipStream_t s) {
+int mi_direct3x_wgrad_launch(int kind, const float* x, const float* dy, float* slabs, int N, int D, hipStream_t s, const WgradFinal* fin) {
     Direct3WgradParams p = {};
     p.x[0] = x; p.dy[0] = dy; p.slabs[0] = slabs; p.nprob = 1; p.splits = mi_direct3x_wgrad_splits(kind);
     if (kind == 3) {
         p.N = N; p.D = D; p.bytes = (unsigned)(4l * N * D * PLANE * 128);
-        hipLaunchKernelGGL((direct3_wgrad_kernel<false, 128>), dim3(36 * p.splits), dim3(512), 0, s, p);
+        wgrad_launch<false, 128, false>(p, 36, fin, s);
     } else return MI_E_UNSUPPORTED;
     MI_RETURN_IF_LAUNCH_FAILED();
     return MI_OK;
diff --git a/cet_pick_amd/csrc/conv_igemm.hip b/cet_pick_amd/csrc/conv_igemm.hip
--- a/cet_pick_amd/csrc/conv_igemm.hip
+++ b/cet_pick_amd/csrc/conv_igemm.hip
@@ -33,20 +33,26 @@
                             int relu, hipStream_t s);
 size_t mi_direct3_wgrad_slab_bytes();
 int mi_direct3_wgrad_splits();
-int mi_direct3_wgrad_launch(const float* x, const float* dy, float* slabs, int N, int D, hipStream_t s);
+int mi_direct3_wgrad_launch(const float* x, const float* dy, float* slabs, int N, int D, hipStream_t s, const WgradFinal* fin = nullptr);
+size_t mi_direct3_wgrad_ticket_bytes();
 int mi_direct3_wgrad_batch_max();
 int mi_direct3_wgrad_batch_splits(int nb);
-int mi_direct3_wgrad_launch_batch(const float* const* xs, const float* const* dys, float* const* slabs, int nb, int N, int D, hipStream_t s);
+int mi_direct3_wgrad_launch_batch(const float* const* xs, const float* const* dys, float* const* slabs, int nb, int N, int D, hipStream_t s,
+                                  const WgradFinal* fin = nullptr);
 size_t mi_direct3s_wgrad_slab_bytes();
 int mi_direct3s_wgrad_splits(int nb);
-int mi_direct3s_wgrad_launch_batch(const float* const* xs, const float* const* dys, float* const* slabs, int nb, int N, hipStream_t s);
-int mi_direct3t_wgrad_launch(const float* x, const float* dy, float* slabs, int N, int D, int H, int W, hipStream_t s);
+int mi_direct3s_wgrad_launch_batch(const float* const* xs, const float* const* dys, float* const* slabs, int nb, int N, hipStream_t s,
+                                   const WgradFinal* fin = nullptr);
+int mi_direct3t_wgrad_launch(const float* x, const float* dy, float* slabs, int N, int D, int H, int W, hipStream_t s,
+                             const WgradFinal* fin = nullptr);
 int mi_direct3x_wgrad_splits(int kind);
 size_t mi_direct3x_wgrad_slab_bytes(int kind);
-int mi_direct3x_wgrad_launch(int kind, const float* x, const float* dy, float* slabs, int N, int D, hipStream_t s);
+int mi_direct3x_wgrad_launch(int kind, const float* x, const float* dy, float* slabs, int N, int D, hipStream_t s,
+                             const WgradFinal* fin = nullptr);
 int mi_pair_wgrad_batch_max();
 int mi_pair_wgrad_launch_batch(const float* const* xs, const float* const* dys, float* const* dws, float* const* slabs, int nb, int N, int Di,
-                               int Ci, int Co, int k, int stride, hipStream_t s);
+                               int Ci, int Co, int k, int stride, hipStream_t s, const WgradFinal* fin = nullptr);
+size_t mi_pair_wgrad_ticket_bytes(int Ci, int Co, int k);
 bool mi_cube2_usable(int N, int Di, int Hi, int Wi, int Ci, int Co, int kd, int kh, int kw, int stride, int pd, int ph, int pw,
                      int dd, int dh, int dw);
 size_t mi_cube2_slab_bytes(int N, int C);
@@ -57,7 +63,7 @@
 int mi_pair_wgrad_splits(int N, int Di, int Ci, int Co, int k, int stride);
 size_t mi_pair_wgrad_slab_bytes(int N, int Di, int Ci, int Co, int k, int stride);
 int mi_pair_wgrad_launch(const float* x, const float* dy, float* dwt, float* slabs, int N, int Di, int Ci, int Co, int k, int stride,
-                         hipStream_t s);
+                         hipStream_t s, const WgradFinal* fin = nullptr);
 bool mi_small_gemm_usable(long M, long N, long K);
 int mi_small_gemm_launch(const float* a, long lda_m, long lda_k, long a_elems, const float* b, long ldb_k, long ldb_n,
                          long b_elems, const float* bias, float* c, int M, int N, int K, hipStream_t s,
@@ -109,7 +115,10 @@
     const float* a_tab[MI_WGRAD_BATCH_MAX];
     const float* b_tab[MI_WGRAD_BATCH_MAX];
     float* out_tab[MI_WGRAD_BATCH_MAX];
+    unsigned* tickets;
+    float* fin_tab[MI_WGRAD_BATCH_MAX];
 };
+constexpr int IG_ZC = 4;
 
 constexpr unsigned OOR = 0x80000000u;
 __device__ __forceinline__ float4 bld4(__amdgpu_buffer_rsrc_t r, unsigned off) {
@@ -157,9 +166,10 @@
     int c0, ia, ib, ic;
 };
 
-template <int MODE, int BM, int BN, int BK, bool STEM, bool BF3 = false>
+template <int MODE, int BM, int BN, int BK, bool STEM, bool BF3 = false, bool WFINAL = false>
 __global__ __launch_bounds__(NTHREADS, BF3 ? ((BM == 128 && BN == 32) ? 2 : 3) : 1) void conv_igemm_kernel(ConvParams p) {
     static_assert(!BF3 || (!STEM && (BK == 16 || BK == 32)), "bf16x3 path: generic layers, 16- or 32-deep slices");
+    static_assert(!WFINAL || (MODE == MODE_WGRAD && !STEM), "final form: weight gradients, not the stem");
     static_assert(BK == 16 || BK == 32 || BK == 64, "slice depth");
     static_assert(BN == 32 || BN == 64 || BN == 128, "tile width");
     static_assert(BN != 32 || (BF3 && BM == 128 && BK == 32), "32-wide tiles: 128 rows, bf16x3, 32-deep slices");
@@ -675,7 +685,59 @@
                     if (p.relu) v = fmaxf(v, 0.f);
                     if (p.mask) v = (p.mask[o] > 0.f) ? v : 0.f;
                 }
-                outp[o] = v;
+                if (WFINAL) __hip_atomic_store(outp + o, v, __ATOMIC_RELAXED, __HIP_MEMORY_SCOPE_AGENT);
+                else outp[o] = v;
+            }
+        }
+    }
+    if constexpr (WFINAL) {
+        __shared__ unsigned s_last;
+        asm volatile("s_waitcnt vmcnt(0)" ::: "memory");
+        __syncthreads();
+        unsigned* ticket = p.tickets + (((long)blockIdx.y * p.ny_tiles + blk_y) * p.tiles_x + blk_x);
+        if (tid == 0) s_last = (__hip_atomic_fetch_add(ticket, 1u, __ATOMIC_RELAXED, __HIP_MEMORY_SCOPE_AGENT) == (unsigned)(p.splits - 1)) ? 1u : 0u;
+        __syncthreads();
+        if (!s_last) return;
+        if (tid == 0) __hip_atomic_store(ticket, 0u, __ATOMIC_RELAXED, __HIP_MEMORY_SCOPE_AGENT);
+        const float* sl = p.nbatch ? p.out_tab[blockIdx.y] : p.out;
+        float* fin = p.fin_tab[blockIdx.y];
+#pragma unroll
+        for (int i = 0; i < MT; ++i)
+#pragma unroll
+        for (int j = 0; j < NT; ++j) {
+            const int col = n0 + wn * WTN + j * 32 + l32;
+            const long row0 = m0 + wm * WTM + i * 32 + 4 * h;
+            const bool colok = col < p.Ncols;
+            float sum[16] = {};
+            for (int z0 = 0; z0 < p.splits; z0 += IG_ZC) {
+                float part[IG_ZC][16];
+#pragma unroll
+                for (int k = 0; k < IG_ZC; ++k) {
+                    const int zl = min(z0 + k, p.splits - 1);
+#pragma unroll
+                    for (int r = 0; r < 16; ++r) {
+                        const long row = row0 + (r & 3) + 8 * (r >> 2);
+                        part[k][r] = (colok && row < M_here)
+                                         ? __hip_atomic_load(sl + (long)zl * p.slab_stride + row * p.Ncols + col, __ATOMIC_RELAXED, __HIP_MEMORY_SCOPE_AGENT)
+                                         : 0.f;
+                    }
+                }
+#pragma unroll
+                for (int k = 0; k < IG_ZC; ++k) {
+                    const int z = z0 + k;
+                    if (z < p.splits) {
+#pragma unroll
+                        for (int r = 0; r < 16; ++r) {
+                            const float v = z == blk_z ? acc[i][j][r] : part[k][r];
+                            sum[r] = z == 0 ? v : sum[r] + v;
+                        }
+                    }
+                }
+            }
+#pragma unroll
+            for (int r = 0; r < 16; ++r) {
+                const long row = row0 + (r & 3) + 8 * (r >> 2);
+                if (colok && row < M_here) fin[row * p.Ncols + col] = sum[r];
             }
         }
     }
@@ -771,7 +833,7 @@
     return pl;
 }
 
-template <int MODE, bool STEM>
+template <int MODE, bool STEM, bool WFINAL = false>
 int launch_mode(const ConvParams& p, const Plan& pl, hipStream_t s) {
     dim3 grid((unsigned)(pl.tiles_x * ((p.Ncols + pl.bn - 1) / pl.bn) * pl.splits), (unsigned)std::max(1, p.nbatch));
     if constexpr (!STEM) {
@@ -783,14 +845,14 @@
             }
         }
         if (conv_arith_bf16x3() && pl.bm == 64 && pl.bn == 64 && (pl.bk == 32 || pl.bk == 16)) {
-            if (pl.bk == 32) hipLaunchKernelGGL((conv_igemm_kernel<MODE, 64, 64, 32, false, true>), grid, dim3(NTHREADS), 0, s, p);
-            else hipLaunchKernelGGL((conv_igemm_kernel<MODE, 64, 64, 16, false, true>), grid, dim3(NTHREADS), 0, s, p);
+            if (pl.bk == 32) hipLaunchKernelGGL((conv_igemm_kernel<MODE, 64, 64, 32, false, true, WFINAL>), grid, dim3(NTHREADS), 0, s, p);
+            else hipLaunchKernelGGL((conv_igemm_kernel<MODE, 64, 64, 16, false, true, WFINAL>), grid, dim3(NTHREADS), 0, s, p);
             MI_RETURN_IF_LAUNCH_FAILED();
             return MI_OK;
         }
     }
 #define MI_LAUNCH(BM_, BN_, BK_) \
-    hipLaunchKernelGGL((conv_igemm_kernel<MODE, BM_, BN_, BK_, STEM>), grid, dim3(NTHREADS), 0, s, p)
+    hipLaunchKernelGGL((conv_igemm_kernel<MODE, BM_, BN_, BK_, STEM, false, WFINAL>), grid, dim3(NTHREADS), 0, s, p)
     if (pl.bn == 128 && !STEM) {
         if (pl.bm == 128) MI_LAUNCH(128, 128, 32); else MI_LAUNCH(64, 128, 32);
     } else if (pl.bm == 128 && pl.bk == 64 && !STEM) MI_LAUNCH(128, 64, 64);
@@ -1028,7 +1090,7 @@
 
 int run_conv(int mode, const Geom& g, const float* a_src, const float* b_src, float* out,
              const float* res, const float* mask, int relu, void* ws, size_t ws_bytes, hipStream_t s,
-             int* defer_splits = nullptr, int res_bcast = 0) {
+             int* defer_splits = nullptr, int res_bcast = 0, const WgradFinal* wfin = nullptr) {
     if (defer_splits) *defer_splits = 1;
     if (mode != MODE_WGRAD && g.N > 1) {
         const long in_per = (long)g.Di * g.Hi * g.Wi * g.Ci, out_per = (long)g.Do * g.Ho * g.Wo * g.Co;
@@ -1089,17 +1151,17 @@
     {
         const int splits = mi_pair_wgrad_splits(g.N, g.Di, g.Ci, g.Co, g.kd, g.stride);
         if (splits == 1 || (ws && ws_bytes >= mi_pair_wgrad_slab_bytes(g.N, g.Di, g.Ci, g.Co, g.kd, g.stride))) {
-            g_last_conv_kernel = splits > 1 ? "pair_wgrad + reduce" : "pair_wgrad";
-            int rc = mi_pair_wgrad_launch(a_src, b_src, out, (float*)ws, g.N, g.Di, g.Ci, g.Co, g.kd, g.stride, s);
-            if (rc || splits == 1) return rc;
+            g_last_conv_kernel = splits > 1 ? (wfin ? "pair_wgrad + reduce (in-kernel)" : "pair_wgrad + reduce") : "pair_wgrad";
+            int rc = mi_pair_wgrad_launch(a_src, b_src, out, (float*)ws, g.N, g.Di, g.Ci, g.Co, g.kd, g.stride, s, wfin);
+            if (rc || splits == 1 || wfin) return rc;
             if (defer_splits) { *defer_splits = splits; return MI_OK; }
             return mi_direct3_finish_slabs((const float*)ws, splits, (long)g.kd * g.kh * g.kw * g.Ci * g.Co, out, nullptr, nullptr, 0, s);
         }
     }
     if (mode == MODE_WGRAD && dkind == 1 && ws && ws_bytes >= mi_direct3_wgrad_slab_bytes()) {
-        g_last_conv_kernel = "direct3_wgrad + reduce";
-        int rc = mi_direct3_wgrad_launch(a_src, b_src, (float*)ws, g.N, g.Di, s);
-        if (rc) return rc;
+        g_last_conv_kernel = wfin ? "direct3_wgrad + reduce (in-kernel)" : "direct3_wgrad + reduce";
+        int rc = mi_direct3_wgrad_launch(a_src, b_src, (float*)ws, g.N, g.Di, s, wfin);
+        if (rc || wfin) return rc;
         const int splits = mi_direct3_wgrad_splits();
         if (defer_splits) { *defer_splits = splits; return MI_OK; }
         const long out_elems = 27l * g.Ci * g.Co, n4 = out_elems / 4;
@@ -1109,30 +1171,30 @@
         return MI_OK;
     }
     if (mode == MODE_WGRAD && dkind == 2 && ws && ws_bytes >= mi_direct3s_wgrad_slab_bytes() && env_int("MI_D3S_WGRAD")) {
-        g_last_conv_kernel = "direct3s_wgrad + reduce";
+        g_last_conv_kernel = wfin ? "direct3s_wgrad + reduce (in-kernel)" : "direct3s_wgrad + reduce";
         const float* xs[1] = {a_src};
         const float* dys[1] = {b_src};
         float* sl[1] = {(float*)ws};
-        int rc = mi_direct3s_wgrad_launch_batch(xs, dys, sl, 1, g.N, s);
-        if (rc) return rc;
+        int rc = mi_direct3s_wgrad_launch_batch(xs, dys, sl, 1, g.N, s, wfin);
+        if (rc || wfin) return rc;
         const int splits = mi_direct3s_wgrad_splits(1);
         if (defer_splits) { *defer_splits = splits; return MI_OK; }
         return mi_direct3_finish_slabs((const float*)ws, splits, 27l * g.Ci * g.Co, out, nullptr, nullptr, 0, s);
     }
     if (mode == MODE_WGRAD && dkind == 5 && g.Hi % 8 == 0 && g.Wi % 8 == 0 && ws && ws_bytes >= mi_direct3_wgrad_slab_bytes() &&
         !env_int("MI_NO_D3T_WGRAD")) {
-        g_last_conv_kernel = "direct3_wgrad (8 x 8 tiles) + reduce";
-        int rc = mi_direct3t_wgrad_launch(a_src, b_src, (float*)ws, g.N, g.Di, g.Hi, g.Wi, s);
-        if (rc) return rc;
+        g_last_conv_kernel = wfin ? "direct3_wgrad (8 x 8 tiles) + reduce (in-kernel)" : "direct3_wgrad (8 x 8 tiles) + reduce";
+        int rc = mi_direct3t_wgrad_launch(a_src, b_src, (float*)ws, g.N, g.Di, g.Hi, g.Wi, s, wfin);
+        if (rc || wfin) return rc;
         const int splits = mi_direct3_wgrad_splits();
         if (defer_splits) { *defer_splits = splits; return MI_OK; }
         return mi_direct3_finish_slabs((const float*)ws, splits, 27l * g.Ci * g.Co, out, nullptr, nullptr, 0, s);
     }
     if (mode == MODE_WGRAD && dkind == 3 && !env_int("MI_NO_D3X_WGRAD") && ws &&
         ws_bytes >= mi_direct3x_wgrad_slab_bytes(dkind)) {
-        g_last_conv_kernel = "direct3_wgrad (128 channels) + reduce";
-        int rc = mi_direct3x_wgrad_launch(dkind, a_src, b_src, (float*)ws, g.N, g.Di, s);
-        if (rc) return rc;
+        g_last_conv_kernel = wfin ? "direct3_wgrad (128 channels) + reduce (in-kernel)" : "direct3_wgrad (128 channels) + reduce";
+        int rc = mi_direct3x_wgrad_launch(dkind, a_src, b_src, (float*)ws, g.N, g.Di, s, wfin);
+        if (rc || wfin) return rc;
         const int splits = mi_direct3x_wgrad_splits(dkind);
         if (defer_splits) { *defer_splits = splits; return MI_OK; }
         return mi_direct3_finish_slabs((const float*)ws, splits, 27l * g.Ci * g.Co, out, nullptr, nullptr, 0, s);
@@ -1140,12 +1202,13 @@
     Setup st;
     int rc = setup_conv(mode, g, &st);
     if (rc) return rc;
-    g_last_conv_kernel = st.pl.splits > 1 ? "implicit GEMM + reduce" : "implicit GEMM";
     ConvParams& p = st.p;
     Plan& pl = st.pl;
     p.a_src = a_src; p.b_src = b_src; p.res = res; p.mask = mask; p.relu = relu;
     p.res_bcast = res_bcast;
     const bool stem = (g.Ci == 1);
+    const bool final_form = wfin && mode == MODE_WGRAD && !stem;
+    g_last_conv_kernel = st.pl.splits > 1 ? (final_form ? "implicit GEMM + reduce (in-kernel)" : "implicit GEMM + reduce") : "implicit GEMM";
     const long out_elems = p.M * p.Ncols;
     if (pl.splits > 1) {
         size_t need = sizeof(float) * (size_t)out_elems * pl.splits;
@@ -1154,10 +1217,12 @@
     p.splits = pl.splits;
     if (pl.splits > 1) { p.out = (float*)ws; p.slab_stride = out_elems; }
     else { p.out = out; p.slab_stride = 0; }
+    if (pl.splits > 1 && final_form) { p.tickets = wfin->tickets; p.fin_tab[0] = out; }
     if (mode == MODE_FWD) rc = stem ? launch_mode<MODE_FWD, true>(p, pl, s) : launch_mode<MODE_FWD, false>(p, pl, s);
     else if (mode == MODE_DGRAD) rc = launch_mode<MODE_DGRAD, false>(p, pl, s);
-    else rc = stem ? launch_mode<MODE_WGRAD, true>(p, pl, s) : launch_mode<MODE_WGRAD, false>(p, pl, s);
+    else rc = stem ? launch_mode<MODE_WGRAD, true>(p, pl, s) : p.tickets ? launch_mode<MODE_WGRAD, false, true>(p, pl, s) : launch_mode<MODE_WGRAD, false>(p, pl, s);
     if (rc) return rc;
+    if (pl.splits > 1 && final_form) return MI_OK;
     if (pl.splits > 1 && defer_splits) { *defer_splits = pl.splits; return MI_OK; }
     if (pl.splits > 1) {
         long n4 = out_elems / 4;
@@ -1204,6 +1269,43 @@
     Geom g;
     if (!x || !dy || !dw || !public_geom(pg, &g)) return MI_E_ARG;
     return run_conv(MODE_WGRAD, g, x, dy, dw, nullptr, nullptr, 0, ws, ws_bytes, (hipStream_t)stream, splits_out);
+}
+
+namespace {
+size_t wgrad_ticket_bytes(const Geom& g, int nb) {
+    nb = std::max(1, std::min(nb, MI_WGRAD_BATCH_MAX));
+    size_t b = mi_direct3_wgrad_ticket_bytes();
+    if (g.Ci >= 64 && g.Co >= 64 && g.kd <= 3) b = std::max(b, mi_pair_wgrad_ticket_bytes(g.Ci, g.Co, g.kd));
+    Setup st;
+    if (!setup_conv(MODE_WGRAD, g, &st)) b = std::max(b, sizeof(unsigned) * (size_t)nb * st.pl.tiles_x * st.p.ny_tiles);
+    return b;
+}
+bool wgrad_final_wanted() {
+    const char* v = getenv("MI_WGRAD_SLABS");
+    return v && v[0] == '0';
+}
+}
+extern "C" size_t mi_wgrad_ticket_bytes(const mi_conv_geom* pg, int nb) {
+    Geom g;
+    return public_geom(pg, &g) ? wgrad_ticket_bytes(g, nb) : 0;
+}
+
+extern "C" int mi_conv3d_pair_wgrad_splits(int N, int Di, int Ci, int Co, int k, int stride) {
+    const int pad = k == 3 ? 1 : 0;
+    if (!mi_pair_wgrad_usable(N, Di, Di, Di, Ci, Co, k, k, k, stride, pad, pad, pad, 1, 1, 1)) return 0;
+    return mi_pair_wgrad_splits(N, Di, Ci, Co, k, stride);
+}
+
+extern "C" int mi_conv_wgrad_final_f32(const float* x, const float* dy, float* dw, const mi_conv_geom* pg, void* ws, size_t ws_bytes,
+                                       void* tickets, size_t ticket_bytes, int* splits_out, mi_stream_t stream) {
+    Geom g;
+    if (!x || !dy || !dw || !public_geom(pg, &g)) return MI_E_ARG;
+    if (!tickets || !wgrad_final_wanted())
+        return run_conv(MODE_WGRAD, g, x, dy, dw, nullptr, nullptr, 0, ws, ws_bytes, (hipStream_t)stream, splits_out);
+    if (ticket_bytes < wgrad_ticket_bytes(g, 1)) return MI_E_WORKSPACE;
+    float* outs[1] = {dw};
+    const WgradFinal fin = {(unsigned*)tickets, outs};
+    return run_conv(MODE_WGRAD, g, x, dy, dw, nullptr, nullptr, 0, ws, ws_bytes, (hipStream_t)stream, splits_out, 0, &fin);
 }
 
 extern "C" const char* mi_debug_last_conv_kernel(void) { return g_last_conv_kernel; }
@@ -1251,8 +1353,22 @@
     return run_conv(MODE_FWD, g, x, w, y, bias, nullptr, 0, ws, ws_bytes, (hipStream_t)stream, nullptr, bias ? 1 : 0);
 }
 
+namespace {
+int wgrad_batch(const float* const* xs, const float* const* dys, float* const* dws, void* const* wss, int nb, const mi_conv_geom* pg,
+                size_t ws_bytes, void* tickets, size_t ticket_bytes, int* splits_out, mi_stream_t stream);
+}
 extern "C" int mi_conv_wgrad_batch_f32(const float* const* xs, const float* const* dys, float* const* dws, void* const* wss, int nb,
                                        const mi_conv_geom* pg, size_t ws_bytes, int* splits_out, mi_stream_t stream) {
+    return wgrad_batch(xs, dys, dws, wss, nb, pg, ws_bytes, nullptr, 0, splits_out, stream);
+}
+extern "C" int mi_conv_wgrad_batch_final_f32(const float* const* xs, const float* const* dys, float* const* dws, void* const* wss, int nb,
+                                             const mi_conv_geom* pg, size_t ws_bytes, void* tickets, size_t ticket_bytes,
+                                             int* splits_out, mi_stream_t stream) {
+    return wgrad_batch(xs, dys, dws, wss, nb, pg, ws_bytes, wgrad_final_wanted() ? tickets : nullptr, ticket_bytes, splits_out, stream);
+}
+namespace {
+int wgrad_batch(const float* const* xs, const float* const* dys, float* const* dws, void* const* wss, int nb, const mi_conv_geom* pg,
+                size_t ws_bytes, void* tickets, size_t ticket_bytes, int* splits_out, mi_stream_t stream) {
     Geom g;
     if (!xs || !dys || !dws || !wss || !splits_out || nb < 1 || !public_geom(pg, &g)) return MI_E_ARG;
     for (int i = 0; i < nb; ++i) if (!xs[i] || !dys[i] || !dws[i]) return MI_E_ARG;
@@ -1262,6 +1378,9 @@
     if (nb > MI_WGRAD_BATCH_MAX) return MI_E_UNSUPPORTED;
     for (int i = 0; i < nb; ++i) slabs[i] = (float*)wss[i];
     if (is_stem7(g)) return MI_E_UNSUPPORTED;
+    if (tickets && ticket_bytes < wgrad_ticket_bytes(g, nb)) return MI_E_WORKSPACE;
+    const WgradFinal fin = {(unsigned*)tickets, dws};
+    const WgradFinal* wfin = tickets ? &fin : nullptr;
     if (mi_pair_wgrad_usable(g.N, g.Di, g.Hi, g.Wi, g.Ci, g.Co, g.kd, g.kh, g.kw, g.stride, g.pd, g.ph, g.pw, g.dd, g.dh, g.dw)) {
         if (nb > mi_pair_wgrad_batch_max()) return MI_E_UNSUPPORTED;
         const int splits = mi_pair_wgrad_splits(g.N, g.Di, g.Ci, g.Co, g.kd, g.stride);
@@ -1269,23 +1388,23 @@
             if (ws_bytes < mi_pair_wgrad_slab_bytes(g.N, g.Di, g.Ci, g.Co, g.kd, g.stride)) return MI_E_UNSUPPORTED;
             for (int i = 0; i < nb; ++i) if (!wss[i]) return MI_E_ARG;
         }
-        g_last_conv_kernel = splits > 1 ? "pair_wgrad x nb + reduce" : "pair_wgrad x nb";
-        *splits_out = splits;
-        return mi_pair_wgrad_launch_batch(xs, dys, dws, slabs, nb, g.N, g.Di, g.Ci, g.Co, g.kd, g.stride, s);
+        g_last_conv_kernel = splits > 1 ? (wfin ? "pair_wgrad x nb + reduce (in-kernel)" : "pair_wgrad x nb + reduce") : "pair_wgrad x nb";
+        *splits_out = wfin ? 1 : splits;
+        return mi_pair_wgrad_launch_batch(xs, dys, dws, slabs, nb, g.N, g.Di, g.Ci, g.Co, g.kd, g.stride, s, wfin);
     }
     if (direct3_kind(g) == 1) {
         if (nb > mi_direct3_wgrad_batch_max() || ws_bytes < mi_direct3_wgrad_slab_bytes()) return MI_E_UNSUPPORTED;
         for (int i = 0; i < nb; ++i) if (!wss[i]) return MI_E_ARG;
-        g_last_conv_kernel = "direct3_wgrad x nb + reduce";
-        *splits_out = mi_direct3_wgrad_batch_splits(nb);
-        return mi_direct3_wgrad_launch_batch(xs, dys, slabs, nb, g.N, g.Di, s);
+        g_last_conv_kernel = wfin ? "direct3_wgrad x nb + reduce (in-kernel)" : "direct3_wgrad x nb + reduce";
+        *splits_out = wfin ? 1 : mi_direct3_wgrad_batch_splits(nb);
+        return mi_direct3_wgrad_launch_batch(xs, dys, slabs, nb, g.N, g.Di, s, wfin);
     }
     if (direct3_kind(g) == 2 && env_int("MI_D3S_WGRAD")) {
         if (nb > mi_direct3_wgrad_batch_max() || ws_bytes < mi_direct3s_wgrad_slab_bytes()) return MI_E_UNSUPPORTED;
         for (int i = 0; i < nb; ++i) if (!wss[i]) return MI_E_ARG;
-        g_last_conv_kernel = "direct3s_wgrad x nb + reduce";
-        *splits_out = mi_direct3s_wgrad_splits(nb);
-        return mi_direct3s_wgrad_launch_batch(xs, dys, slabs, nb, g.N, s);
+        g_last_conv_kernel = wfin ? "direct3s_wgrad x nb + reduce (in-kernel)" : "direct3s_wgrad x nb + reduce";
+        *splits_out = wfin ? 1 : mi_direct3s_wgrad_splits(nb);
+        return mi_direct3s_wgrad_launch_batch(xs, dys, slabs, nb, g.N, s, wfin);
     }
     {
         const int dk = direct3_kind(g);
@@ -1313,11 +1432,16 @@
     for (int i = 0; i < nb; ++i) { p.a_tab[i] = xs[i]; p.b_tab[i] = dys[i]; p.out_tab[i] = splits > 1 ? slabs[i] : dws[i]; }
     p.out = p.out_tab[0];
     p.slab_stride = splits > 1 ? out_elems : 0;
-    g_last_conv_kernel = splits > 1 ? "implicit GEMM x nb + reduce" : "implicit GEMM x nb";
-    rc = launch_mode<MODE_WGRAD, false>(p, pl, s);
+    if (splits > 1 && wfin) {
+        p.tickets = wfin->tickets;
+        for (int i = 0; i < nb; ++i) p.fin_tab[i] = dws[i];
+    }
+    g_last_conv_kernel = splits > 1 ? (wfin ? "implicit GEMM x nb + reduce (in-kernel)" : "implicit GEMM x nb + reduce") : "implicit GEMM x nb";
+    rc = p.tickets ? launch_mode<MODE_WGRAD, false, true>(p, pl, s) : launch_mode<MODE_WGRAD, false>(p, pl, s);
     if (rc) return rc;
-    *splits_out = splits;
+    *splits_out = wfin ? 1 : splits;
     return MI_OK;
+}
 }
 
 extern "C" int mi_splitk_reduce_batch(const void* const* slabs, void* const* outs, const int* n_slabs, const long* out_elems,
diff --git a/cet_pick_amd/hipops.py b/cet_pick_amd/hipops.py
--- a/cet_pick_amd/hipops.py
+++ b/cet_pick_amd/hipops.py
@@ -711,6 +711,12 @@
 
 
 DEFERRED_WGRADS = None
+WGRAD_TICKET_MIN = 1 << 16
+
+
+def _wgrad_tickets(geom, nb, device):
+    need = max(int(L.lib().mi_wgrad_ticket_bytes(geom.ref, nb)), WGRAD_TICKET_MIN)
+    return L.workspace(need, device, "wgrad_tickets", init=lambda b: b.zero_())
 
 
 def flush_wgrad_reduces():
@@ -745,8 +751,12 @@
 
     def __call__(self):
         splits = ctypes.c_int(0)
-        L.check(L.lib().mi_conv_wgrad_f32(L.ptr(self.x), L.ptr(self.dy), L.ptr(self.tgt), self.geom.ref, L.ptr(self.slab),
-                                          self.slab.numel(), ctypes.addressof(splits), L.stream()), "mi_conv_wgrad_f32")
+        tk = _wgrad_tickets(self.geom, 1, self.x.device)
+        rc = L.lib().mi_conv_wgrad_final_f32(L.ptr(self.x), L.ptr(self.dy), L.ptr(self.tgt), self.geom.ref, L.ptr(self.slab),
+                                             self.slab.numel(), L.ptr(tk), tk.numel(), ctypes.addressof(splits), L.stream())
+        if rc:
+            L.drop_workspace(self.x.device, "wgrad_tickets")
+        L.check(rc, "mi_conv_wgrad_final_f32")
         if splits.value > 1:
             DEFERRED_WGRADS.append((self.slab, self.tgt, int(splits.value), self.tgt.numel()))
 
@@ -796,9 +806,13 @@
     rc = -3
     if len(jobs) > 1:
         splits = ctypes.c_int(0)
-        rc = L.lib().mi_conv_wgrad_batch_f32(L.host_array([j.x.data_ptr() for j in jobs]), L.host_array([j.dy.data_ptr() for j in jobs]),
-                                             L.host_array([j.tgt.data_ptr() for j in jobs]), L.host_array([j.slab.data_ptr() for j in jobs]),
-                                             len(jobs), jobs[0].geom.ref, jobs[0].slab.numel(), ctypes.addressof(splits), L.stream())
+        tk = _wgrad_tickets(jobs[0].geom, len(jobs), jobs[0].x.device)
+        rc = L.lib().mi_conv_wgrad_batch_final_f32(L.host_array([j.x.data_ptr() for j in jobs]), L.host_array([j.dy.data_ptr() for j in jobs]),
+                                                   L.host_array([j.tgt.data_ptr() for j in jobs]),
+                                                   L.host_array([j.slab.data_ptr() for j in jobs]), len(jobs), jobs[0].geom.ref,
+                                                   jobs[0].slab.numel(), L.ptr(tk), tk.numel(), ctypes.addressof(splits), L.stream())
+        if rc not in (0, -3):
+            L.drop_workspace(jobs[0].x.device, "wgrad_tickets")
         if rc == 0 and splits.value > 1:
             for j in jobs:
                 DEFERRED_WGRADS.append((j.slab, j.tgt, int(splits.value), j.tgt.numel()))
@@ -806,7 +820,7 @@
         for j in jobs:
             j()
     else:
-        L.check(rc, "mi_conv_wgrad_batch_f32")
+        L.check(rc, "mi_conv_wgrad_batch_final_f32")
 
 
 def run_wgrad_jobs(items):
diff --git a/include/cetpick_hip.h b/include/cetpick_hip.h
--- a/include/cetpick_hip.h
+++ b/include/cetpick_hip.h
@@ -121,6 +121,13 @@
                            mi_stream_t stream);
 int mi_conv_wgrad_batch_f32(const float* const* xs, const float* const* dys, float* const* dws, void* const* wss, int nb,
                             const mi_conv_geom* g, size_t ws_bytes, int* splits_out, mi_stream_t stream);
+size_t mi_wgrad_ticket_bytes(const mi_conv_geom* g, int nb);
+int mi_conv3d_pair_wgrad_splits(int N, int Di, int Ci, int Co, int k, int stride);
+int mi_conv_wgrad_final_f32(const float* x, const float* dy, float* dw, const mi_conv_geom* g, void* ws, size_t ws_bytes,
+                            void* tickets, size_t ticket_bytes, int* splits_out, mi_stream_t stream);
+int mi_conv_wgrad_batch_final_f32(const float* const* xs, const float* const* dys, float* const* dws, void* const* wss, int nb,
+                                  const mi_conv_geom* g, size_t ws_bytes, void* tickets, size_t ticket_bytes, int* splits_out,
+                                  mi_stream_t stream);
 
 int mi_linear_bn_fwd_f32(const float* x, const float* w, const float* bias, float* xlin, float* y, int M, int Ci, int Co,
                          const float* gamma, const float* beta, float eps, float momentum, float* running_mean,
```

Measured after the change: 42580 subtomograms/sec. 0.988x the previous value.
